# bdaiinstitute/vlfm

Hardware: AMD Instinct MI355X
Metric: env-steps/s (VLM+value-map update), 640x480 RGB-D (higher is better)
Workload: dtype f16 ViT-g (f32 accumulate) + f32 Q-Former (split-f16, 22-bit); f32 confidence + f64 value maps; 1 GPU; configs[1] step x resident envs: BLIP-2 ITC + ValueMap+ObstacleMap+sort_waypoints; envs_per_gpu=256, global_envs=256, map=1000x1000 @ 20 px/m, parallelism=env-sharded x1, tuned_gemms=True, vit_gemm=hip:fc1, attention=hip

## Files before the change

### include/vlfm_amd.h

```cpp
#ifndef VLFM_AMD_H
#define VLFM_AMD_H

#include <stddef.h>
#include <stdint.h>

#ifdef __cplusplus
extern "C" {
#endif

typedef enum {
    VLFM_OK = 0,
    VLFM_ERR_INVALID = -1,
    VLFM_ERR_OUTSIDE_MAP = -2,
    VLFM_ERR_INDEX = -3,
    VLFM_ERR_HIP = -4,
    VLFM_ERR_CAPACITY = -5
} vlfm_status;

enum { VLFM_FUSE_DEFAULT = 0, VLFM_FUSE_REPLACE = 1, VLFM_FUSE_EQUAL_WEIGHTING = 2 };

const char* vlfm_last_error(void);
int vlfm_abi_version(void);

int vlfm_profile_enable(int on);
int vlfm_profile_read(const char* kernel_name, double* mean_ms, int* launches);

int vlfm_host_wait_mode(int blocking);

typedef struct {
    double inv_affine[6];
    int32_t row0, col0;
    int32_t env;
    int32_t reserved;
} vlfm_vm_pose;

int vlfm_value_map_pose_params(const double* h_tf, const double* h_yaw, const int32_t* h_env, int n, int map_size,
                               int pixels_per_meter, int template_size, vlfm_vm_pose* h_out, int* bad_index);

int vlfm_cone_template_host(double fov, double max_depth, int pixels_per_meter, double min_confidence,
                            float* h_conf, int conf_capacity, int64_t* h_poly_xy, int poly_capacity,
                            int* n_poly);

int vlfm_tan_table_host(double fov, int width, double* h_out);

int vlfm_cone_template_build(const float* d_conf, const int64_t* d_poly_xy, int n_poly, int template_size,
                             float* d_template, uint32_t* d_template_bits, void* stream);

typedef struct {
    double tf[12];
    float depth_scale;
    float depth_offset;
    float depth_max;
    float reserved0;
    double fx, fy;
    double min_height, max_height;
    int32_t env;
    int32_t scatter;
} vlfm_ingest_params;

typedef struct {
    uint32_t* d_cells;
    int32_t* d_count;
    int32_t capacity;
    int32_t reserved;
} vlfm_scatter_journal;

int vlfm_depth_ingest_batched(const float* d_depth, int n, int height, int width,
                              const vlfm_ingest_params* d_params,
                              uint32_t* d_colmax_keys ,
                              uint32_t* d_obstacle , int map_size, int pixels_per_meter,
                              int32_t* d_status ,
                              uint32_t* d_hole_bits ,
                              const uint32_t* d_filled_bits ,
                              const vlfm_scatter_journal* journal ,
                              void* stream);

int vlfm_selftest_div_exact(const double* d_numerators, int n, double divisor, int32_t* d_mismatches, void* stream);

size_t vlfm_hole_scratch_bytes(int n, int height, int width, int cap_pts, int cap_contours);
int vlfm_fill_small_holes_batched(const uint32_t* d_hole_bits, const int32_t* d_status, int n, int height, int width,
                                  double area_thresh, void* d_scratch, size_t scratch_bytes, int cap_pts,
                                  int cap_contours, uint32_t* d_filled_bits, int32_t* d_counts,
                                  const vlfm_ingest_params* d_params, uint32_t* d_obstacle, int map_size,
                                  const vlfm_scatter_journal* journal, void* stream);
int vlfm_depth_scatter_holes_batched(const vlfm_ingest_params* d_params, int n, int height, int width,
                                     const uint32_t* d_hole_bits, const uint32_t* d_filled_bits,
                                     const int32_t* d_hole_counts ,
                                     uint32_t* d_obstacle, int map_size, int pixels_per_meter, int32_t* d_status,
                                     const float* d_depth ,
                                     void* stream);

int vlfm_fill_small_holes_rig_batched(const uint32_t* d_hole_bits, const int32_t* d_status, int n, int height, int width,
                                      double area_thresh, void* d_scratch, size_t scratch_bytes, int cap_pts,
                                      int cap_contours, uint32_t* d_filled_bits, int32_t* d_counts,
                                      const vlfm_ingest_params* d_params, uint32_t* d_obstacle, int map_size,
                                      const vlfm_scatter_journal* journal, int32_t* d_slot_undone, int n_envs, void* stream);
int vlfm_depth_scatter_holes_rig_batched(const vlfm_ingest_params* d_params, int n, int height, int width,
                                         const uint32_t* d_hole_bits, const uint32_t* d_filled_bits,
                                         const int32_t* d_hole_counts, uint32_t* d_obstacle, int map_size,
                                         int pixels_per_meter, int32_t* d_status, const float* d_depth,
                                         const int32_t* d_slot_undone, void* stream);

int vlfm_value_map_update_fused_batched(uint32_t* d_colmax_keys, int width, const double* d_tan,
                                        const float* d_template, const uint32_t* d_template_bits, int template_size,
                                        const vlfm_vm_pose* d_pose, const double* d_values, int n,
                                        float* d_conf, double* d_value, int map_size, int channels, int pixels_per_meter,
                                        double min_depth, double max_depth, int use_max_confidence, int fusion_type,
                                        const uint32_t* d_explored_bits, uint32_t* d_written_bits, int32_t* d_counters,
                                        const float* d_conf_quadrant, void* stream);

typedef struct {
    const float* d_template;
    const uint32_t* d_template_bits;
    const float* d_conf_quadrant;
    const double* d_tan;
    float depth_scale;
    float depth_offset;
    int32_t template_size;
    int32_t reserved;
} vlfm_vm_optics;

int vlfm_value_map_update_rig_batched(uint32_t* d_colmax_keys, int width, const vlfm_vm_pose* d_pose,
                                      const vlfm_vm_optics* d_optics, const int32_t* d_slots, int n_slots, int n,
                                      int max_template_size, const double* d_values, float* d_conf, double* d_value,
                                      int map_size, int channels, int pixels_per_meter, int use_max_confidence,
                                      int fusion_type, const uint32_t* d_explored_bits, uint32_t* d_written_bits,
                                      int32_t* d_counters, void* stream);

int vlfm_disc_rows_host(int radius, int32_t* h_halfwidth );
int vlfm_value_map_sort_waypoints_batched(const double* d_value, int map_size, int channels,
                                          const int32_t* d_cells, int m, int radius, const int32_t* d_disc,
                                          int value_is_f32, double* d_out, void* stream);



int vlfm_resample_coeffs_host(int in_size, int out_size, int32_t* h_bounds, int32_t* h_kk, int kk_capacity,
                              int* ksize_out);

int vlfm_resample_coeffs_filter_host(int in_size, int out_size, int filter, int32_t* h_bounds, int32_t* h_kk,
                                     int kk_capacity, int* ksize_out);

int vlfm_preprocess_sam_batched(const uint8_t* d_rgb, int n, int height, int width, int out_h, int out_w,
                                const int32_t* d_hbounds, const int32_t* d_hk, int hksize,
                                const int32_t* d_vbounds, const int32_t* d_vk, int vksize,
                                const float* h_mean3, const float* h_std3, int pad_size, uint8_t* d_tmp, float* d_out,
                                void* stream);

int vlfm_preprocess_rgb_batched(const uint8_t* d_rgb, int n, int height, int width, int out_size,
                                const int32_t* d_hbounds, const int32_t* d_hk, int hksize,
                                const int32_t* d_vbounds, const int32_t* d_vk, int vksize,
                                const float* h_mean3, const float* h_std3, uint8_t* d_tmp, void* d_out,
                                int out_dtype, int patch_size, void* stream);

int vlfm_itc_head_batched(const float* d_proj, int batch, int n_query, int proj_dim,
                          const float* d_text, float* d_out, void* stream);

#define VLFM_ITC_MAX_PROMPTS 8
int vlfm_itc_head_multi(const float* d_proj, int batch, int n_query, int proj_dim, const float* d_text_table, int n_text,
                        const int32_t* d_text_index, int n_prompts, float* d_out, void* stream);

int vlfm_layernorm_bias_f16(const void* d_x, const float* d_channel_bias, const void* d_gamma, const void* d_beta,
                            void* d_y, int rows, int dim, float eps, void* stream);

int vlfm_vit_attention_f16(const void* d_qkv, void* d_out, int batch, int tokens, int heads, int head_dim, float scale,
                           void* stream);

int vlfm_gemm_f16_nt(const void* d_x, const void* d_w, const void* d_bias, void* d_c, int m, int n, int k, int epilogue,
                     void* stream);

int vlfm_gemm_f16_pair_f32_nt(const void* d_x, const void* d_w_pair, const void* d_bias_f32, void* d_out, int m, int n_out, int k,
                              void* stream);

int vlfm_qformer_cross_attention_f32(const void* d_q, const void* d_kv_blocks, void* d_out, int batch, int tokens, int queries,
                                     int heads, int k_block0, int v_block0, int m_total, float scale, void* stream);

int vlfm_gemm_f16_tile_order(int m, int n, int group_m, int* out, int capacity_pairs);
int vlfm_gemm_f16_work_items(int m, int n, int grid, int* out, int capacity_pairs);

int vlfm_split_f32_to_f16_pair(const float* d_src, void* d_hi, void* d_lo, long long count, int* d_overflow, void* stream);
int vlfm_gemm_f32_nt(const float* d_x, const float* d_w, const float* d_bias, const float* d_residual, float* d_c, int m, int n,
                     int k, int activation, int precision, const void* d_w_hi, const void* d_w_lo, int* d_overflow, void* stream);


int vlfm_layernorm_rows_f32(const float* d_x, const float* d_gamma, const float* d_beta, float* d_out, int batch, int height,
                            int width, int channels, int window, float eps, void* stream);
int vlfm_window_reverse_add_f32(float* d_x, const float* d_windows, int batch, int height, int width, int channels, int window,
                                void* stream);
int vlfm_dwconv3x3_nhwc_f32(const float* d_x, const float* d_w9c, const float* d_bias, float* d_out, int batch, int height, int width,
                            int channels, void* stream);
int vlfm_window_attention_f32(const float* d_qkv, const float* d_bias_t, float* d_out, long long windows, int tokens, int heads,
                              float scale, void* stream);
int vlfm_layernorm_rows_shifted_f32(const float* d_x, const float* d_gamma, const float* d_beta, float* d_out, int batch, int height,
                                    int width, int channels, int window, float eps, int shift, int pad_zero, void* stream);
int vlfm_window_reverse_add_shifted_f32(float* d_x, const float* d_windows, int batch, int height, int width, int channels, int window,
                                        int shift, void* stream);
int vlfm_window_attention_masked_f32(const float* d_qkv, const float* d_bias_t, const float* d_mask_t, int windows_per_image, float* d_out,
                                     long long windows, int tokens, int heads, float scale, void* stream);

int vlfm_maxpool2x2_nhwc_f16(const void* d_x, void* d_out, int batch, int height, int width, int channels, void* stream);
int vlfm_conv_nhwc_tile(int pixels, int cin, int cout, int ksize, int* tile_pixels, int* tile_channels);
int vlfm_conv_nhwc_f16(const void* d_x, const void* d_w, const void* d_bias, void* d_out, const void* d_zero, int batch,
                       int height, int width, int cin, int cout, int ksize, int stride, int x_pix_stride,
                       int out_pix_stride, int act, void* stream);

int vlfm_resize_area_tab_host(int ssize, int dsize, int32_t* h_first, int32_t* h_count, float* h_w, int ktaps_capacity);

int vlfm_resize_area_batched(const uint8_t* d_rgb, int n, int height, int width, int out_h, int out_w,
                             const int32_t* d_xfirst, const int32_t* d_xcount, const float* d_xw, int xktaps,
                             const int32_t* d_yfirst, const int32_t* d_ycount, const float* d_yw, int yktaps,
                             void* d_out, int out_dtype, void* stream);

int vlfm_to_tensor_normalize_batched(const uint8_t* d_rgb, int n, int height, int width, const float* h_mean3,
                                     const float* h_std3, float* d_out, void* stream);

size_t vlfm_nms_scratch_bytes(int n);
int vlfm_nms(const float* d_boxes_xyxy, const int32_t* d_order, int n, float iou_threshold, void* d_scratch,
             size_t scratch_bytes, int32_t* d_keep, int32_t* d_num_keep, int max_keep, void* stream);

int vlfm_ms_deform_attn(const float* d_value, const int32_t* d_spatial_shapes, const int32_t* d_level_start,
                        const float* d_sampling_loc, const float* d_attn_weight, int batch, int n_query, int n_heads,
                        int head_dim, int n_levels, int n_points, int total_len, float* d_out, void* stream);
int vlfm_ms_deform_attn_fused(const float* d_value, const int32_t* d_spatial_shapes, const int32_t* d_level_start,
                              const float* d_offsets_logits, const float* d_reference, int batch, int n_query, int n_heads,
                              int head_dim, int n_levels, int n_points, int ref_coords, int total_len, float* d_out, void* stream);

int vlfm_dwconv3x3_f32(const float* d_x, const float* d_w, const float* d_bias, float* d_y, int n, int channels, int height,
                       int width, int stride, int gelu, void* stream);

int vlfm_bias_act_nchw(void* d_y, const void* d_bias, int n, int channels, long long hw, int dtype, int act, void* stream);


size_t vlfm_object_cloud_scratch_bytes(int height, int width);
int vlfm_object_cloud_extract(const float* d_depth, const uint8_t* d_mask, int height, int width, int erosion_iterations,
                              double min_depth, double max_depth, double fx, double fy, void* d_scratch, double* d_cloud,
                              int capacity, int32_t* d_count, void* stream);

size_t vlfm_dbscan_scratch_bytes(int n);
int vlfm_dbscan_largest_cluster(const double* d_points, int n, double eps, int min_points, void* d_scratch,
                                size_t scratch_bytes, int32_t* d_labels, int32_t* d_keep, int32_t* d_num_keep, void* stream);

int vlfm_bits_pack(const uint8_t* d_src, uint32_t* d_dst, int planes, int rows, int cols, void* stream);
int vlfm_bits_unpack(const uint32_t* d_src, uint8_t* d_dst, int planes, int rows, int cols, void* stream);

int vlfm_bits_dilate(const uint32_t* d_src, uint32_t* d_dst, int planes, int rows, int cols, int kernel_w,
                     int kernel_h, void* stream);

int vlfm_find_contours_external(const uint32_t* d_img, int planes, int rows, int cols, int method,
                                uint32_t* d_scratch , int32_t* d_pts, int cap_pts,
                                int32_t* d_starts, int32_t* d_lens, int cap_contours, int32_t* d_counts, void* stream);

size_t vlfm_find_contours_wg_scratch_bytes(int planes, int rows, int cols, int cap_pts);
int vlfm_walk_path_counters(long long* h_out4, int reset);
int vlfm_find_contours_external_wg(const uint32_t* d_img, int planes, int rows, int cols, int method, void* d_scratch,
                                   size_t scratch_bytes, int32_t* d_pts, int cap_pts, int32_t* d_starts, int32_t* d_lens,
                                   int cap_contours, int32_t* d_counts, void* stream);

#define VLFM_FOG_MAX_POLY 80
typedef struct {
    int32_t env;
    int32_t ax, ay;
    int32_t radius;
    int32_t n_poly;
    int32_t reserved;
    double rot_c, rot_s;
    double line_len;
    long long poly[2 * VLFM_FOG_MAX_POLY];
} vlfm_fog_params;

int vlfm_fog_params_host(const int32_t* h_agent_px, const double* h_angle_cv2_deg, const double* h_rot_cs,
                         double fov_deg, double max_line_len, const int32_t* h_env, const int32_t* h_explore, int n,
                         vlfm_fog_params* h_out);

size_t vlfm_obstacle_scratch_bytes(int n_envs, int map_size, int cap_pts, int cap_contours);

int vlfm_obstacle_map_update_batched(const vlfm_fog_params* d_prm, int n, const uint32_t* d_obstacle,
                                     uint32_t* d_navigable, uint32_t* d_explored, int32_t* d_bbox, int n_envs,
                                     int map_size, int kernel_size, int fog_radius, double area_thresh_px,
                                     void* d_scratch, size_t scratch_bytes, int cap_pts, int cap_contours,
                                     double* d_frontiers, int cap_frontiers, int32_t* d_counts, int update_obstacles,
                                     int explore, const int32_t* d_windows, int window_blocks_navigable,
                                     int window_blocks_prepare, void* stream);

int vlfm_obstacle_status(const void* d_scratch, int n_envs, int map_size, int cap_pts, int cap_contours,
                         int32_t* h_out);

enum { VLFM_REDUCE_MAX = 0,
       VLFM_REDUCE_EXPLORE = 1,
       VLFM_REDUCE_PLANE = 2 };
enum { VLFM_PRIM_CIRCLE_FILL = 0,
       VLFM_PRIM_CIRCLE = 1,
       VLFM_PRIM_LINE = 2,
       VLFM_PRIM_POLYLINE = 3 };
#define VLFM_RENDER_FLIP_ROWS 1
#define VLFM_RENDER_UNDER_PATH 2
typedef struct {
    int32_t frame;
    int32_t kind;
    int32_t flags;
    int32_t thickness;
    int32_t x0, y0, x1, y1;
    int32_t vtx_off, n_vtx;
    uint8_t bgr[4];
    int32_t reserved;
} vlfm_render_prim;

size_t vlfm_value_render_scratch_bytes(int n, int map_size);

int vlfm_value_map_render(const double* d_value, int n_envs, int map_size, int channels, const int32_t* d_frames, int n,
                          int reduce_mode, double explore_thresh, const double* d_plane, const uint32_t* d_explored,
                          const uint32_t* d_path, const int32_t* d_prim_off, const vlfm_render_prim* d_prims,
                          const int64_t* d_vtx, int rgb, void* d_scratch, size_t scratch_bytes, uint8_t* d_out,
                          void* stream);

int vlfm_obstacle_map_render(const uint32_t* d_obstacle, const uint32_t* d_navigable, const uint32_t* d_explored,
                             int n_envs, int map_size, const int32_t* d_frames, int n, uint32_t pad_bgr,
                             const uint32_t* d_path, const int32_t* d_prim_off, const vlfm_render_prim* d_prims,
                             const int64_t* d_vtx, int rgb, uint8_t* d_out, void* stream);

int vlfm_traj_append(uint32_t* d_path, int n_envs, int map_size, const int32_t* d_segs, int m, int thickness,
                     void* stream);

int vlfm_circle_polygon_host(const int32_t* h_circles, int n, int64_t* h_xy, int32_t* h_off, int capacity);

int vlfm_jpeg_quant_tables_host(int quality, uint16_t* h_tables);
size_t vlfm_jpeg_scratch_bytes(int n, int H, int W);
int vlfm_jpeg_roundtrip_batched(const uint8_t* d_in, uint8_t* d_out, int n, int H, int W, const uint16_t* h_tables,
                                void* d_scratch, size_t scratch_bytes, void* stream);

int vlfm_jpeg_header_host(int quality, int H, int W, uint8_t* h_out, size_t cap, size_t* len);
size_t vlfm_jpeg_encode_bound(int H, int W);
size_t vlfm_jpeg_encode_scratch_bytes(int n, int H, int W);
int vlfm_jpeg_encode_batched(const uint8_t* d_in, int n, int H, int W, int rgb_order, const uint16_t* h_tables,
                             uint8_t* d_out, size_t capacity, uint32_t* d_lengths, void* d_scratch, size_t scratch_bytes,
                             void* stream);
// ... 46 lines not shown
```

### vlfm_amd/_lib.py

```python
from __future__ import annotations

import ctypes
import os
import subprocess
from typing import Optional

_HERE = os.path.dirname(os.path.abspath(__file__))
LIB_PATH = os.path.join(_HERE, "libvlfm_amd.so")
SOURCES = ["value_map.hip", "depth_ingest.hip", "depth_holes.hip", "obstacle_map.hip", "vlm_ops.hip", "vit_attention.hip", "qformer_attention.hip", "detect_ops.hip", "object_cloud.hip", "gemm_f16.hip", "gemm_f32.hip", "conv_nhwc.hip", "sam_ops.hip", "map_render.hip", "jpeg_codec.hip", "jpeg_entropy.hip", "jpeg_decode.hip", "world_render.hip", "host.cpp"]

VLFM_OK = 0
VLFM_ERR_INVALID = -1
VLFM_ERR_OUTSIDE_MAP = -2
VLFM_ERR_INDEX = -3
VLFM_ERR_HIP = -4
VLFM_ERR_CAPACITY = -5

FUSION_TYPES = {"default": 0, "replace": 1, "equal_weighting": 2}


class VmPose(ctypes.Structure):
    _fields_ = [("inv_affine", ctypes.c_double * 6), ("row0", ctypes.c_int32), ("col0", ctypes.c_int32),
                ("env", ctypes.c_int32), ("reserved", ctypes.c_int32)]


class IngestParams(ctypes.Structure):
    _fields_ = [("tf", ctypes.c_double * 12), ("depth_scale", ctypes.c_float), ("depth_offset", ctypes.c_float),
                ("depth_max", ctypes.c_float), ("reserved0", ctypes.c_float), ("fx", ctypes.c_double),
                ("fy", ctypes.c_double), ("min_height", ctypes.c_double), ("max_height", ctypes.c_double),
                ("env", ctypes.c_int32), ("scatter", ctypes.c_int32)]


FOG_MAX_POLY = 80


class FogParams(ctypes.Structure):
    _fields_ = [("env", ctypes.c_int32), ("ax", ctypes.c_int32), ("ay", ctypes.c_int32), ("radius", ctypes.c_int32),
                ("n_poly", ctypes.c_int32), ("reserved", ctypes.c_int32), ("rot_c", ctypes.c_double),
                ("rot_s", ctypes.c_double), ("line_len", ctypes.c_double), ("poly", ctypes.c_longlong * (2 * FOG_MAX_POLY))]


class ScatterJournal(ctypes.Structure):
    _fields_ = [("d_cells", ctypes.c_void_p), ("d_count", ctypes.c_void_p), ("capacity", ctypes.c_int32),
                ("reserved", ctypes.c_int32)]


class VmOptics(ctypes.Structure):
    _fields_ = [("d_template", ctypes.c_void_p), ("d_template_bits", ctypes.c_void_p), ("d_conf_quadrant", ctypes.c_void_p),
                ("d_tan", ctypes.c_void_p), ("depth_scale", ctypes.c_float), ("depth_offset", ctypes.c_float),
                ("template_size", ctypes.c_int32), ("reserved", ctypes.c_int32)]


assert ctypes.sizeof(ScatterJournal) == 24 and ctypes.sizeof(VmOptics) == 48
assert ctypes.sizeof(VmPose) == 64 and ctypes.sizeof(IngestParams) == 152 and ctypes.sizeof(FogParams) == 48 + 16 * FOG_MAX_POLY


def build(verbose: bool = False) -> str:
    from concurrent.futures import ThreadPoolExecutor

    csrc = os.path.join(_HERE, "csrc")
    srcs = [os.path.join(csrc, s) for s in SOURCES if os.path.exists(os.path.join(csrc, s))]
    hdrs = [os.path.join(csrc, h) for h in os.listdir(csrc) if h.endswith(".h")] + [
        os.path.join(_HERE, "..", "include", "vlfm_amd.h")]
    hdr_time = max(os.path.getmtime(h) for h in hdrs)
    objdir = os.path.join(csrc, "build")
    os.makedirs(objdir, exist_ok=True)
    flags = ["--offload-arch=gfx950", "-O3", "-std=c++17", "-fPIC", "-ffp-contract=off"]

    def compile_one(src: str) -> str:
        obj = os.path.join(objdir, os.path.basename(src) + ".o")
        if not os.path.exists(obj) or os.path.getmtime(obj) < max(os.path.getmtime(src), hdr_time):
            cmd = ["hipcc"] + flags + ["-c", src, "-o", obj]
            if verbose:
                print(" ".join(cmd), flush=True)
            subprocess.check_call(cmd)
        return obj

    with ThreadPoolExecutor(max_workers=min(8, len(srcs))) as pool:
        objs = list(pool.map(compile_one, srcs))
    if os.path.exists(LIB_PATH) and all(os.path.getmtime(LIB_PATH) >= os.path.getmtime(o) for o in objs):
        return LIB_PATH
    cmd = ["hipcc", "--offload-arch=gfx950", "-shared", "-fPIC", "-o", LIB_PATH] + objs
    if verbose:
        print(" ".join(cmd), flush=True)
    subprocess.check_call(cmd)
    return LIB_PATH


_lib: Optional[ctypes.CDLL] = None


def lib() -> ctypes.CDLL:
    global _lib
    if _lib is None:
        if not os.path.exists(LIB_PATH):
            raise ImportError(
                f"{LIB_PATH} is missing: build it with `python -c 'import __graft_entry__ as g; g.build()'` "
                "(hipcc --offload-arch=gfx950).  vlfm_amd has no CPU fallback.")
        L = ctypes.CDLL(LIB_PATH)
        vp, ci, cd = ctypes.c_void_p, ctypes.c_int, ctypes.c_double
        L.vlfm_last_error.restype = ctypes.c_char_p
        L.vlfm_abi_version.restype = ci
        L.vlfm_profile_enable.argtypes = [ci]
        L.vlfm_host_wait_mode.argtypes = [ci]
        L.vlfm_profile_read.argtypes = [ctypes.c_char_p, ctypes.POINTER(cd), ctypes.POINTER(ci)]
        L.vlfm_value_map_pose_params.argtypes = [vp, vp, vp, ci, ci, ci, ci, vp, ctypes.POINTER(ci)]
        L.vlfm_cone_template_host.argtypes = [cd, cd, ci, cd, vp, ci, vp, ci, ctypes.POINTER(ci)]
        L.vlfm_tan_table_host.argtypes = [cd, ci, vp]
        L.vlfm_disc_rows_host.argtypes = [ci, vp]
        L.vlfm_cone_template_build.argtypes = [vp, vp, ci, ci, vp, vp, vp]
        L.vlfm_depth_ingest_batched.argtypes = [vp, ci, ci, ci, vp, vp, vp, ci, ci, vp, vp, vp, vp, vp]
        L.vlfm_selftest_div_exact.argtypes = [vp, ci, cd, vp, vp]
        L.vlfm_hole_scratch_bytes.argtypes = [ci, ci, ci, ci, ci]
        L.vlfm_hole_scratch_bytes.restype = ctypes.c_size_t
        L.vlfm_fill_small_holes_batched.argtypes = [vp, vp, ci, ci, ci, cd, vp, ctypes.c_size_t, ci, ci, vp, vp, vp, vp,
                                                    ci, vp, vp]
        L.vlfm_depth_scatter_holes_batched.argtypes = [vp, ci, ci, ci, vp, vp, vp, vp, ci, ci, vp, vp, vp]
        L.vlfm_fill_small_holes_rig_batched.argtypes = [vp, vp, ci, ci, ci, cd, vp, ctypes.c_size_t, ci, ci, vp, vp, vp, vp,
                                                        ci, vp, vp, ci, vp]
        L.vlfm_depth_scatter_holes_rig_batched.argtypes = [vp, ci, ci, ci, vp, vp, vp, vp, ci, ci, vp, vp, vp, vp]
        L.vlfm_layernorm_bias_f16.argtypes = [vp, vp, vp, vp, vp, ci, ci, ctypes.c_float, vp]
        L.vlfm_vit_attention_f16.argtypes = [vp, vp, ci, ci, ci, ci, ctypes.c_float, vp]
        L.vlfm_gemm_f16_nt.argtypes = [vp, vp, vp, vp, ci, ci, ci, ci, vp]
        L.vlfm_gemm_f16_pair_f32_nt.argtypes = [vp, vp, vp, vp, ci, ci, ci, vp]
        L.vlfm_qformer_cross_attention_f32.argtypes = [vp, vp, vp, ci, ci, ci, ci, ci, ci, ci, ctypes.c_float, vp]
        L.vlfm_gemm_f32_nt.argtypes = [vp, vp, vp, vp, vp, ci, ci, ci, ci, ci, vp, vp, vp, vp]
        L.vlfm_split_f32_to_f16_pair.argtypes = [vp, vp, vp, ctypes.c_longlong, vp, vp]
        L.vlfm_layernorm_rows_f32.argtypes = [vp, vp, vp, vp, ci, ci, ci, ci, ci, ctypes.c_float, vp]
        L.vlfm_window_reverse_add_f32.argtypes = [vp, vp, ci, ci, ci, ci, ci, vp]
        L.vlfm_dwconv3x3_nhwc_f32.argtypes = [vp, vp, vp, vp, ci, ci, ci, ci, vp]
        L.vlfm_window_attention_f32.argtypes = [vp, vp, vp, ctypes.c_longlong, ci, ci, ctypes.c_float, vp]
        L.vlfm_layernorm_rows_shifted_f32.argtypes = [vp, vp, vp, vp, ci, ci, ci, ci, ci, ctypes.c_float, ci, ci, vp]
        L.vlfm_window_reverse_add_shifted_f32.argtypes = [vp, vp, ci, ci, ci, ci, ci, ci, vp]
        L.vlfm_window_attention_masked_f32.argtypes = [vp, vp, vp, ci, vp, ctypes.c_longlong, ci, ci, ctypes.c_float, vp]
        L.vlfm_maxpool2x2_nhwc_f16.argtypes = [vp, vp, ci, ci, ci, ci, vp]
        L.vlfm_conv_nhwc_tile.argtypes = [ci, ci, ci, ci, ctypes.POINTER(ci), ctypes.POINTER(ci)]
        L.vlfm_conv_nhwc_f16.argtypes = [vp, vp, vp, vp, vp, ci, ci, ci, ci, ci, ci, ci, ci, ci, ci, vp]
        L.vlfm_value_map_update_fused_batched.argtypes = [vp, ci, vp, vp, vp, ci, vp, vp, ci, vp, vp, ci, ci, ci, cd, cd,
                                                          ci, ci, vp, vp, vp, vp, vp]
        L.vlfm_value_map_update_rig_batched.argtypes = [vp, ci, vp, vp, vp, ci, ci, ci, vp, vp, vp, ci, ci, ci, ci, ci, vp, vp,
                                                        vp, vp]
        L.vlfm_value_map_sort_waypoints_batched.argtypes = [vp, ci, ci, vp, ci, ci, vp, ci, vp, vp]
        L.vlfm_resample_coeffs_host.argtypes = [ci, ci, vp, vp, ci, ctypes.POINTER(ci)]
        L.vlfm_resample_coeffs_filter_host.argtypes = [ci, ci, ci, vp, vp, ci, ctypes.POINTER(ci)]
        L.vlfm_preprocess_sam_batched.argtypes = [vp, ci, ci, ci, ci, ci, vp, vp, ci, vp, vp, ci, vp, vp, ci, vp, vp, vp]
        L.vlfm_preprocess_rgb_batched.argtypes = [vp, ci, ci, ci, ci, vp, vp, ci, vp, vp, ci, vp, vp, vp, vp, ci, ci, vp]
        L.vlfm_itc_head_batched.argtypes = [vp, ci, ci, ci, vp, vp, vp]
        L.vlfm_itc_head_multi.argtypes = [vp, ci, ci, ci, vp, ci, vp, ci, vp, vp]
        cf = ctypes.c_float
        L.vlfm_resize_area_tab_host.argtypes = [ci, ci, vp, vp, vp, ci]
        L.vlfm_resize_area_batched.argtypes = [vp, ci, ci, ci, ci, ci, vp, vp, vp, ci, vp, vp, vp, ci, vp, ci, vp]
        L.vlfm_to_tensor_normalize_batched.argtypes = [vp, ci, ci, ci, vp, vp, vp, vp]
        L.vlfm_nms_scratch_bytes.argtypes = [ci]
        L.vlfm_nms_scratch_bytes.restype = ctypes.c_size_t
        L.vlfm_nms.argtypes = [vp, vp, ci, cf, vp, ctypes.c_size_t, vp, vp, ci, vp]
        L.vlfm_ms_deform_attn.argtypes = [vp, vp, vp, vp, vp, ci, ci, ci, ci, ci, ci, ci, vp, vp]
        L.vlfm_ms_deform_attn_fused.argtypes = [vp, vp, vp, vp, vp, ci, ci, ci, ci, ci, ci, ci, ci, vp, vp]
        L.vlfm_object_cloud_scratch_bytes.argtypes = [ci, ci]
        L.vlfm_object_cloud_scratch_bytes.restype = ctypes.c_size_t
        L.vlfm_object_cloud_extract.argtypes = [vp, vp, ci, ci, ci, cd, cd, cd, cd, vp, vp, ci, vp, vp]
        L.vlfm_dbscan_scratch_bytes.argtypes = [ci]
        L.vlfm_dbscan_scratch_bytes.restype = ctypes.c_size_t
        L.vlfm_dbscan_largest_cluster.argtypes = [vp, ci, cd, ci, vp, ctypes.c_size_t, vp, vp, vp, vp]
        L.vlfm_bits_pack.argtypes = [vp, vp, ci, ci, ci, vp]
        L.vlfm_bits_unpack.argtypes = [vp, vp, ci, ci, ci, vp]
        L.vlfm_bits_dilate.argtypes = [vp, vp, ci, ci, ci, ci, ci, vp]
        L.vlfm_find_contours_external.argtypes = [vp, ci, ci, ci, ci, vp, vp, ci, vp, vp, ci, vp, vp]
        L.vlfm_dwconv3x3_f32.argtypes = [vp, vp, vp, vp, ci, ci, ci, ci, ci, ci, vp]
        L.vlfm_bias_act_nchw.argtypes = [vp, vp, ci, ci, ctypes.c_longlong, ci, ci, vp]
        L.vlfm_find_contours_wg_scratch_bytes.argtypes = [ci, ci, ci, ci]
        L.vlfm_find_contours_wg_scratch_bytes.restype = ctypes.c_size_t
        L.vlfm_find_contours_external_wg.argtypes = [vp, ci, ci, ci, ci, vp, ctypes.c_size_t, vp, ci, vp, vp, ci, vp, vp]
        L.vlfm_walk_path_counters.argtypes = [vp, ci]
        L.vlfm_fog_params_host.argtypes = [vp, vp, vp, cd, cd, vp, vp, ci, vp]
        L.vlfm_obstacle_scratch_bytes.argtypes = [ci, ci, ci, ci]
        L.vlfm_obstacle_scratch_bytes.restype = ctypes.c_size_t
        L.vlfm_obstacle_map_update_batched.argtypes = [vp, ci, vp, vp, vp, vp, ci, ci, ci, ci, cd, vp, ctypes.c_size_t,
                                                       ci, ci, vp, ci, vp, ci, ci, vp, ci, ci, vp]
        L.vlfm_obstacle_status.argtypes = [vp, ci, ci, ci, ci, vp]
        L.vlfm_value_render_scratch_bytes.argtypes = [ci, ci]
        L.vlfm_value_render_scratch_bytes.restype = ctypes.c_size_t
        L.vlfm_value_map_render.argtypes = [vp, ci, ci, ci, vp, ci, ci, cd, vp, vp, vp, vp, vp, vp, ci, vp,
                                            ctypes.c_size_t, vp, vp]
        L.vlfm_obstacle_map_render.argtypes = [vp, vp, vp, ci, ci, vp, ci, ctypes.c_uint32, vp, vp, vp, vp, ci, vp, vp]
        L.vlfm_traj_append.argtypes = [vp, ci, ci, vp, ci, ci, vp]
        L.vlfm_circle_polygon_host.argtypes = [vp, ci, vp, vp, ci]
        L.vlfm_jpeg_quant_tables_host.argtypes = [ci, vp]
        L.vlfm_jpeg_scratch_bytes.argtypes = [ci, ci, ci]
        L.vlfm_jpeg_scratch_bytes.restype = ctypes.c_size_t
        L.vlfm_jpeg_roundtrip_batched.argtypes = [vp, vp, ci, ci, ci, vp, vp, ctypes.c_size_t, vp]
        L.vlfm_jpeg_header_host.argtypes = [ci, ci, ci, vp, ctypes.c_size_t, ctypes.POINTER(ctypes.c_size_t)]
        L.vlfm_jpeg_encode_bound.argtypes = [ci, ci]
        L.vlfm_jpeg_encode_bound.restype = ctypes.c_size_t
        L.vlfm_jpeg_encode_scratch_bytes.argtypes = [ci, ci, ci]
        L.vlfm_jpeg_encode_scratch_bytes.restype = ctypes.c_size_t
        L.vlfm_jpeg_encode_batched.argtypes = [vp, ci, ci, ci, ci, vp, vp, ctypes.c_size_t, vp, vp, ctypes.c_size_t, vp]
        L.vlfm_jpeg_parse_host.argtypes = [vp, ctypes.c_size_t, vp, vp]
        L.vlfm_jpeg_parse_reason.argtypes = [ci]
        L.vlfm_jpeg_parse_reason.restype = ctypes.c_char_p
        L.vlfm_jpeg_decode_chunk_bytes.restype = ctypes.c_size_t
        L.vlfm_jpeg_decode_scratch_bytes.argtypes = [ci, ci, ci, ctypes.c_size_t]
        L.vlfm_jpeg_decode_scratch_bytes.restype = ctypes.c_size_t
        L.vlfm_jpeg_decode_batched.argtypes = [vp, ctypes.c_size_t, vp, ctypes.c_size_t, vp, ci, ci, ci, vp, vp, ci, vp, ci, ci,
                                               ctypes.c_size_t, ci, vp, vp, vp, ctypes.c_size_t, vp]
        L.vlfm_rooms_raycast.argtypes = [vp, ci, vp, ci, ci, ci, vp, vp]
        L.vlfm_rooms_raycast_objects.argtypes = [vp, ci, vp, ci, vp, vp, ci, ci, ci, vp, vp, vp, vp]
        _lib = L
    return _lib


def profile_read(kernel: str):
    ms, n = ctypes.c_double(0.0), ctypes.c_int(0)
    lib().vlfm_profile_read(kernel.encode(), ctypes.byref(ms), ctypes.byref(n))
    return ms.value, n.value


def last_error() -> str:
    return lib().vlfm_last_error().decode()


def host_wait_blocking(device=None, blocking: bool = True) -> None:
    import torch

    with torch.cuda.device(device if device is not None else torch.cuda.current_device()):
        check(lib().vlfm_host_wait_mode(int(bool(blocking))), "host_wait_mode")


def try_host_wait_blocking(device=None) -> bool:
    import os
    import warnings

    if os.environ.get("VLFM_HOST_WAIT", "blocking") == "spin":
        return False
    try:
        host_wait_blocking(device)
        return True
    except Exception as exc:
        warnings.warn(f"blocking host waits not enabled on {device}: {exc} (call vlfm_amd._lib.host_wait_blocking before the "
                      f"device's first allocation; waits will spin on a host core)")
        return False


def check(rc: int, what: str = "") -> int:
    if rc >= 0:
        return rc
    msg = last_error()
    if rc == VLFM_ERR_OUTSIDE_MAP:
        raise AssertionError(msg or "Pixel location is outside the image.")
    if rc == VLFM_ERR_INDEX:
        raise IndexError(msg or "index out of bounds for obstacle map")
    raise RuntimeError(f"libvlfm_amd {what} failed ({rc}): {msg}")
```

### vlfm_amd/csrc/gemm_f32.hip

```cpp
#include <hip/hip_runtime.h>
#include <stdint.h>
#include <stdlib.h>

#include "../../include/vlfm_amd.h"
#include "profile.h"
#include "status.h"

namespace vlfm {
namespace g32 {

typedef float floatx4 __attribute__((ext_vector_type(4)));
typedef float floatx16 __attribute__((ext_vector_type(16)));
typedef _Float16 half8 __attribute__((ext_vector_type(8)));
typedef _Float16 half4 __attribute__((ext_vector_type(4)));

constexpr int TB = 128;
constexpr int TK = 32;
constexpr int ROWB = TK * 4;
constexpr int OPER = TB * ROWB;
constexpr int BUF = 2 * OPER;
constexpr int EPI_ROW = 272;
constexpr int EPI_WAVE = 64 * EPI_ROW;
constexpr int LDS_EXACT = 4 * EPI_WAVE > 2 * BUF ? 4 * EPI_WAVE : 2 * BUF;

enum { ACT_NONE = 0, ACT_RELU = 1, ACT_GELU = 2 };

struct Args {
    const float* x;
    const float* w;
    const float* bias;
    const float* residual;
    float* c;
    int M, N, K;
    int tiles_m, tiles_n;
    int* overflow;
    const _Float16* w_hi;
    const _Float16* w_lo;
};

__device__ inline float gelu_erf(float v) {
    const float u = fabsf(v);
    float q = 2.834908400e-06f;
    q = fmaf(q, u, -3.937762449e-05f);
    q = fmaf(q, u, 1.861798810e-04f);
    q = fmaf(q, u, 1.369373058e-04f);
    q = fmaf(q, u, -7.063421421e-03f);
    q = fmaf(q, u, 5.249617994e-02f);
    q = fmaf(q, u, 4.592081904e-01f);
    q = fmaf(q, u, 1.151105165e+00f);
    const float e = __builtin_amdgcn_exp2f(-(q * u));
    return fmaf(-0.5f * u, e, fmaxf(v, 0.0f));
}

using lds_ptr = __attribute__((address_space(3))) unsigned char*;
using gbl_ptr = const __attribute__((address_space(1))) unsigned char*;

__device__ inline void tile_of_block(const Args& a, int& tm, int& tn) {
    const int nwg = a.tiles_m * a.tiles_n;
    int bid = blockIdx.x;
    const int q = nwg >> 3, r = nwg & 7, xcd = bid & 7, idx = bid >> 3;
    bid = (xcd < r ? xcd * (q + 1) : r * (q + 1) + (xcd - r) * q) + idx;
    tm = bid / a.tiles_n;
    tn = bid - tm * a.tiles_n;
}

__device__ inline void stage_tile(const Args& a, lds_ptr lds, int buf, int n0, int m0, int k0, int wave, int lane) {
    const int sub = lane >> 3, p = lane & 7;
#pragma unroll
    for (int j = 0; j < 4; j++) {
        const int chunk = wave * 4 + j;
        const int r = chunk * 8 + sub;
        const int s = p ^ ((r >> 1) & 7);
        const int rn = min(n0 + r, a.N - 1), rm = min(m0 + r, a.M - 1);
        const float* gw = a.w + (size_t)rn * a.K + k0 + s * 4;
        const float* gx = a.x + (size_t)rm * a.K + k0 + s * 4;
        const int dst = __builtin_amdgcn_readfirstlane(buf + chunk * 1024);
        __builtin_amdgcn_global_load_lds((gbl_ptr)gw, lds + dst, 16, 0, 0);
        __builtin_amdgcn_global_load_lds((gbl_ptr)gx, lds + dst + OPER, 16, 0, 0);
    }
}

template <bool SPLIT>
__device__ inline void store_tile(const Args& a, unsigned char* smem, const floatx16 (&acc)[2][2], const floatx16 (&cross)[2][2],
                                  int act, int wave, int wn, int wm, int lane, int m0, int n0) {
    unsigned char* stg = smem + wave * EPI_WAVE;
    const int c32 = lane & 31, h4 = (lane >> 5) * 4;
    floatx4 bias4[2][4];
#pragma unroll
    for (int i = 0; i < 2; i++)
#pragma unroll
        for (int g = 0; g < 4; g++) {
            floatx4 b = {0.f, 0.f, 0.f, 0.f};
            if (a.bias) {
                const int n = n0 + wn * 64 + i * 32 + g * 8 + h4;
                if (n + 4 <= a.N && ((uintptr_t)a.bias & 15) == 0) b = *reinterpret_cast<const floatx4*>(a.bias + n);
                else
                    for (int e = 0; e < 4; e++) b[e] = n + e < a.N ? a.bias[n + e] : 0.f;
            }
            bias4[i][g] = b;
        }
#pragma unroll
    for (int i = 0; i < 2; i++)
#pragma unroll
        for (int g = 0; g < 4; g++) {
            const int nl = i * 32 + g * 8 + h4;
            const floatx4 b = bias4[i][g];
#pragma unroll
            for (int j = 0; j < 2; j++) {
                floatx4 v;
#pragma unroll
                for (int e = 0; e < 4; e++) {
                    float t = acc[i][j][g * 4 + e];
                    if (SPLIT) t = fmaf(cross[i][j][g * 4 + e], 0x1p-11f, t);
                    t += b[e];
                    if (act == ACT_RELU) t = fmaxf(t, 0.f);
                    else if (act == ACT_GELU) t = gelu_erf(t);
                    v[e] = t;
                }
                *reinterpret_cast<floatx4*>(stg + (j * 32 + c32) * EPI_ROW + nl * 4) = v;
            }
        }
    __builtin_amdgcn_s_waitcnt(0xC07F);
    const int rsub = lane >> 4, chunk = lane & 15;
    const bool vec = (a.N & 3) == 0;
    const int n = n0 + wn * 64 + chunk * 4;
    const bool fast = vec && n + 4 <= a.N;
    floatx4 r[16], v[16];
#pragma unroll
    for (int it = 0; it < 16; it++) {
        const int m = m0 + wm * 64 + it * 4 + rsub;
        r[it] = floatx4{0.f, 0.f, 0.f, 0.f};
        if (a.residual && fast && m < a.M) r[it] = *reinterpret_cast<const floatx4*>(a.residual + (size_t)m * a.N + n);
    }
#pragma unroll
    for (int it = 0; it < 16; it++) v[it] = *reinterpret_cast<const floatx4*>(stg + (it * 4 + rsub) * EPI_ROW + chunk * 16);
#pragma unroll
    for (int it = 0; it < 16; it++) {
        const int m = m0 + wm * 64 + it * 4 + rsub;
        if (m >= a.M || n >= a.N) continue;
        const size_t at = (size_t)m * a.N + n;
        if (fast) {
            *reinterpret_cast<floatx4*>(a.c + at) = v[it] + r[it];
        } else {
            for (int e = 0; e < 4 && n + e < a.N; e++) a.c[at + e] = v[it][e] + (a.residual ? a.residual[at + e] : 0.f);
        }
    }
}

__global__ __launch_bounds__(256, 2) void gemm_f32_exact_kernel(Args a, int act) {
    extern __shared__ __attribute__((aligned(16))) unsigned char smem[];
    lds_ptr lds = (lds_ptr)smem;
    const int tid = threadIdx.x, lane = tid & 63;
    const int wave = __builtin_amdgcn_readfirstlane(tid >> 6);
    const int wn = wave >> 1, wm = wave & 1;
    int tm, tn;
    tile_of_block(a, tm, tn);
    const int m0 = tm * TB, n0 = tn * TB;
    const int NT = a.K / TK;

    floatx16 acc[2][2];
#pragma unroll
    for (int i = 0; i < 2; i++)
#pragma unroll
        for (int j = 0; j < 2; j++)
#pragma unroll
            for (int e = 0; e < 16; e++) acc[i][j][e] = 0.f;

    stage_tile(a, lds, 0, n0, m0, 0, wave, lane);
    __builtin_amdgcn_s_waitcnt(0x0F70);
    __builtin_amdgcn_s_barrier();
    asm volatile("" ::: "memory");

    const int r32 = lane & 31, h = lane >> 5;
    for (int t = 0; t < NT; t++) {
        const int cur = (t & 1) * BUF;
        if (t + 1 < NT) stage_tile(a, lds, cur ^ BUF, n0, m0, (t + 1) * TK, wave, lane);
#pragma unroll
        for (int kk = 0; kk < 4; kk++) {
            const int s = kk * 2 + h;
            floatx4 fa[2], fb[2];
#pragma unroll
            for (int i = 0; i < 2; i++) {
                const int R = wn * 64 + i * 32 + r32;
                fa[i] = *reinterpret_cast<const floatx4*>(smem + cur + R * ROWB + ((s ^ ((R >> 1) & 7)) << 4));
            }
#pragma unroll
            for (int j = 0; j < 2; j++) {
                const int R = wm * 64 + j * 32 + r32;
                fb[j] = *reinterpret_cast<const floatx4*>(smem + cur + OPER + R * ROWB + ((s ^ ((R >> 1) & 7)) << 4));
            }
#pragma unroll
            for (int q = 0; q < 4; q++)
#pragma unroll
                for (int i = 0; i < 2; i++)
#pragma unroll
                    for (int j = 0; j < 2; j++)
                        acc[i][j] = __builtin_amdgcn_mfma_f32_32x32x2f32(fa[i][q], fb[j][q], acc[i][j], 0, 0, 0);
        }
        __builtin_amdgcn_s_waitcnt(0x0F70);
        __builtin_amdgcn_s_barrier();
        asm volatile("" ::: "memory");
    }
    store_tile<false>(a, smem, acc, acc, act, wave, wn, wm, lane, m0, n0);
}

constexpr int SROWB = TK * 2;
constexpr int SOPER = TB * SROWB;
constexpr int SBUF = 4 * SOPER;

__device__ inline int sslot(int row, int slot) { return (slot ^ ((row >> 2) & 3)) << 4; }

__device__ inline void split4(const floatx4 v, half4& hi, half4& lo, bool& over) {
#pragma unroll
    for (int e = 0; e < 4; e++) {
        const float a = v[e];
        over |= !(fabsf(a) < 65504.0f);
        const _Float16 hh = (_Float16)a;
        hi[e] = hh;
        lo[e] = (_Float16)((a - (float)hh) * 2048.0f);
    }
}

template <int NI>
struct SplitGeom {
    static constexpr int TN = 64 * NI;
    static constexpr int WOPER = TN * SROWB;
    static constexpr int XO = 0, WO = 2 * SOPER;
    static constexpr int BUF = 2 * SOPER + 2 * WOPER;
    static constexpr int LDS = 4 * EPI_WAVE > 2 * BUF ? 4 * EPI_WAVE : 2 * BUF;
};

template <int NI>
__device__ __forceinline__ void gemm_f32_split_body(const Args& a, int act) {
    using G = SplitGeom<NI>;
    extern __shared__ __attribute__((aligned(16))) unsigned char smem[];
    lds_ptr lds = (lds_ptr)smem;
    const int tid = threadIdx.x, lane = tid & 63;
    const int wave = __builtin_amdgcn_readfirstlane(tid >> 6);
    const int wn = wave >> 1, wm = wave & 1;
    int tm, tn;
    tile_of_block(a, tm, tn);
    const int m0 = tm * TB, n0 = tn * G::TN;
    const int NT = a.K / TK;

    floatx16 acc[NI][2], crs[NI][2];
#pragma unroll
    for (int i = 0; i < NI; i++)
#pragma unroll
        for (int j = 0; j < 2; j++)
#pragma unroll
            for (int e = 0; e < 16; e++) { acc[i][j][e] = 0.f; crs[i][j][e] = 0.f; }

    floatx4 xr[4];
    bool over = false;
    auto load_x = [&](int k0) {
#pragma unroll
        for (int u = 0; u < 4; u++) {
            const int idx = tid + 256 * u, r = idx >> 3, pc = idx & 7;
            const int rm = min(m0 + r, a.M - 1);
            xr[u] = *reinterpret_cast<const floatx4*>(a.x + (size_t)rm * a.K + k0 + pc * 4);
        }
    };
    auto put_x = [&](int buf) {
#pragma unroll
        for (int u = 0; u < 4; u++) {
            const int idx = tid + 256 * u, r = idx >> 3, pc = idx & 7;
            half4 hi, lo;
            split4(xr[u], hi, lo, over);
            const int off = r * SROWB + sslot(r, pc >> 1) + (pc & 1) * 8;
            *reinterpret_cast<half4*>(smem + buf + G::XO + off) = hi;
            *reinterpret_cast<half4*>(smem + buf + G::XO + SOPER + off) = lo;
        }
    };
    auto stage_w = [&](int buf, int k0) {
        const int sub = lane >> 2, p = lane & 3;
#pragma unroll
        for (int j = 0; j < NI; j++) {
            const int chunk = wave * NI + j;
            const int r = chunk * 16 + sub;
            const int s = p ^ ((r >> 2) & 3);
            const int rn = min(n0 + r, a.N - 1);
            const size_t g = (size_t)rn * a.K + k0 + s * 8;
            const int dst = __builtin_amdgcn_readfirstlane(buf + G::WO + chunk * 1024);
            __builtin_amdgcn_global_load_lds((gbl_ptr)(a.w_hi + g), lds + dst, 16, 0, 0);
            __builtin_amdgcn_global_load_lds((gbl_ptr)(a.w_lo + g), lds + dst + G::WOPER, 16, 0, 0);
        }
    };

    load_x(0);
    stage_w(0, 0);
    put_x(0);
    __builtin_amdgcn_s_waitcnt(0x0F70);
    __builtin_amdgcn_s_waitcnt(0xC07F);
    __builtin_amdgcn_s_barrier();
    asm volatile("" ::: "memory");

    const int r32 = lane & 31, h = lane >> 5;
    for (int t = 0; t < NT; t++) {
        const int cur = (t & 1) * G::BUF;
        if (t + 1 < NT) {
            load_x((t + 1) * TK);
            stage_w(cur ^ G::BUF, (t + 1) * TK);
        }
#pragma unroll
        for (int kk = 0; kk < 2; kk++) {
            const int s = kk * 2 + h;
            half8 whi[NI], wlo[NI], xhi[2], xlo[2];
#pragma unroll
            for (int i = 0; i < NI; i++) {
                const int R = wn * 32 * NI + i * 32 + r32, o = cur + G::WO + R * SROWB + sslot(R, s);
                whi[i] = *reinterpret_cast<const half8*>(smem + o);
                wlo[i] = *reinterpret_cast<const half8*>(smem + o + G::WOPER);
            }
#pragma unroll
            for (int j = 0; j < 2; j++) {
                const int R = wm * 64 + j * 32 + r32, o = cur + G::XO + R * SROWB + sslot(R, s);
                xhi[j] = *reinterpret_cast<const half8*>(smem + o);
                xlo[j] = *reinterpret_cast<const half8*>(smem + o + SOPER);
            }
#pragma unroll
            for (int i = 0; i < NI; i++)
#pragma unroll
                for (int j = 0; j < 2; j++) {
                    acc[i][j] = __builtin_amdgcn_mfma_f32_32x32x16_f16(whi[i], xhi[j], acc[i][j], 0, 0, 0);
                    crs[i][j] = __builtin_amdgcn_mfma_f32_32x32x16_f16(whi[i], xlo[j], crs[i][j], 0, 0, 0);
                    crs[i][j] = __builtin_amdgcn_mfma_f32_32x32x16_f16(wlo[i], xhi[j], crs[i][j], 0, 0, 0);
                }
        }
        if (t + 1 < NT) put_x(cur ^ G::BUF);
        __builtin_amdgcn_s_waitcnt(0x0F70);
        __builtin_amdgcn_s_waitcnt(0xC07F);
        __builtin_amdgcn_s_barrier();
        asm volatile("" ::: "memory");
    }
    if (over && a.overflow) atomicOr(a.overflow, 1);
#pragma unroll
    for (int half = 0; half < NI / 2; half++)
        store_tile<true>(a, smem, reinterpret_cast<const floatx16(&)[2][2]>(acc[2 * half]),
                         reinterpret_cast<const floatx16(&)[2][2]>(crs[2 * half]), act, wave, 0, wm, lane, m0,
                         n0 + wn * 32 * NI + half * 64);
}

__global__ __launch_bounds__(256, 2) void gemm_f32_split_kernel(Args a, int act) { gemm_f32_split_body<2>(a, act); }

__global__ void split_f32_kernel(const float* __restrict__ src, _Float16* __restrict__ hi, _Float16* __restrict__ lo, long long n,
                                 int* overflow) {
    const long long i = (long long)blockIdx.x * blockDim.x + threadIdx.x;
    if (i >= n) return;
    const float a = src[i];
    if (!(fabsf(a) < 65504.0f) && overflow) atomicOr(overflow, 1);
    const _Float16 hh = (_Float16)a;
    hi[i] = hh;
    lo[i] = (_Float16)((a - (float)hh) * 2048.0f);
}

}
}

using namespace vlfm;
using namespace vlfm::g32;

extern "C" int vlfm_split_f32_to_f16_pair(const float* d_src, void* d_hi, void* d_lo, long long count, int* d_overflow, void* stream) {
    if (count == 0) return VLFM_OK;
    if (!d_src || !d_hi || !d_lo || count < 0) return fail(VLFM_ERR_INVALID, "split_f32_to_f16_pair: bad argument");
    const long long blocks = (count + 255) / 256;
    VLFM_KLAUNCH(split_f32_kernel, dim3((unsigned)blocks), dim3(256), 0, (hipStream_t)stream, d_src, (_Float16*)d_hi, (_Float16*)d_lo,
                 count, d_overflow);
    return check_launch("split_f32_kernel");
}

extern "C" int vlfm_gemm_f32_nt(const float* d_x, const float* d_w, const float* d_bias, const float* d_residual, float* d_c, int m,
                                int n, int k, int activation, int precision, const void* d_w_hi, const void* d_w_lo,
                                int* d_overflow, void* stream) {
    if (m == 0 || n == 0) return VLFM_OK;
    if (!d_x || !d_w || !d_c || m < 0 || n < 0 || k <= 0 || (k % TK) != 0 || activation < 0 || activation > 2 || precision < 0 ||
        precision > 1)
        return fail(VLFM_ERR_INVALID, "gemm_f32_nt: K must be a multiple of 32, activation 0..2, precision 0..1");
    if (((uintptr_t)d_x | (uintptr_t)d_w | (uintptr_t)d_c | (uintptr_t)d_residual | (uintptr_t)d_w_hi | (uintptr_t)d_w_lo) & 15)
        return fail(VLFM_ERR_INVALID, "gemm_f32_nt: X, W, C, residual and the split weights must be 16-byte aligned");
    if (precision == 1 && (!d_w_hi || !d_w_lo || !d_overflow))
        return fail(VLFM_ERR_INVALID, "gemm_f32_nt: the split form needs the pre-split weights and the overflow flag");
    Args a;
    a.x = d_x; a.w = d_w; a.bias = d_bias; a.residual = d_residual; a.c = d_c;
    a.M = m; a.N = n; a.K = k;
    a.tiles_m = (m + TB - 1) / TB; a.tiles_n = (n + TB - 1) / TB;
    a.overflow = d_overflow; a.w_hi = (const _Float16*)d_w_hi; a.w_lo = (const _Float16*)d_w_lo;
    if ((long long)a.tiles_m * a.tiles_n > 0x7fffffffLL) return fail(VLFM_ERR_CAPACITY, "gemm_f32_nt: too many tiles");
    const dim3 grid(a.tiles_m * a.tiles_n), block(256);
    static LdsOptIn opt_exact, opt_split;
    if (precision == 0) {
        if (LDS_EXACT > 64 * 1024 && !opt_exact.ensure(reinterpret_cast<const void*>(gemm_f32_exact_kernel), LDS_EXACT))
            return fail(VLFM_ERR_HIP, "gemm_f32_nt: cannot opt in to the LDS size");
        VLFM_TIMED("gemm_f32_exact_kernel", stream);
        VLFM_KLAUNCH(gemm_f32_exact_kernel, grid, block, LDS_EXACT, (hipStream_t)stream, a, activation);
        return check_launch("gemm_f32_exact_kernel");
    }
    if (SplitGeom<2>::LDS > 64 * 1024 && !opt_split.ensure(reinterpret_cast<const void*>(gemm_f32_split_kernel), SplitGeom<2>::LDS))
        return fail(VLFM_ERR_HIP, "gemm_f32_nt: cannot opt in to the LDS size");
    VLFM_TIMED("gemm_f32_split_kernel", stream);
    VLFM_KLAUNCH(gemm_f32_split_kernel, grid, block, SplitGeom<2>::LDS, (hipStream_t)stream, a, activation);
    return check_launch("gemm_f32_split_kernel");
}
```

### vlfm_amd/csrc/host.cpp

```cpp
#include <cmath>
#include <cstdint>
#include <cstring>
#include <mutex>
#include <string>

#include "../../include/vlfm_amd.h"
#include "status.h"

namespace vlfm {
static thread_local std::string g_last_error;
void set_last_error(const char* msg) { g_last_error = msg ? msg : ""; }
}

extern "C" const char* vlfm_last_error(void) { return vlfm::g_last_error.c_str(); }
extern "C" int vlfm_abi_version(void) { return 16; }

namespace {

const double kPi = 3.141592653589793238462643383279502884;

inline long round_half_even(double v) { return std::lrint(v); }

float sin_deg_table(int deg) {
    static float tab[451];
    static std::once_flag once;
    std::call_once(once, [] {
        for (int i = 0; i <= 450; i++) tab[i] = (float)(std::round(std::sin(i * kPi / 180.0) * 1e7) / 1e7);
    });
    return tab[deg];
}

}

extern "C" int vlfm_value_map_pose_params(const double* h_tf, const double* h_yaw, const int32_t* h_env, int n,
                                          int map_size, int pixels_per_meter, int template_size,
                                          vlfm_vm_pose* h_out, int* bad_index) {
    if (!h_tf || !h_out || n < 0 || map_size <= 0 || template_size <= 0)
        return vlfm::fail(VLFM_ERR_INVALID, "value_map_pose_params: bad argument");
    const double ppm = (double)pixels_per_meter;
    const int half = template_size / 2;
    for (int k = 0; k < n; k++) {
        const double* tf = h_tf + 16 * k;
        const double yaw = h_yaw ? h_yaw[k] : std::atan2(tf[4], tf[0]);
        const double degrees = (-yaw) * (180.0 / kPi);
        const double ang = degrees * (kPi / 180);
        const double alpha = std::cos(ang), beta = std::sin(ang);
        const double cx = (double)(float)half, cy = (double)(float)half;
        double M[6] = {alpha, beta, (1 - alpha) * cx - beta * cy, -beta, alpha, beta * cx + (1 - alpha) * cy};
        double D = M[0] * M[4] - M[1] * M[3];
        D = D != 0 ? 1. / D : 0;
        const double A11 = M[4] * D, A22 = M[0] * D;
        M[0] = A11; M[1] *= -D;
        M[3] *= -D; M[4] = A22;
        const double b1 = -M[0] * M[2] - M[1] * M[5];
        const double b2 = -M[3] * M[2] - M[4] * M[5];
        M[2] = b1; M[5] = b2;
        vlfm_vm_pose& p = h_out[k];
        std::memcpy(p.inv_affine, M, sizeof(M));
        const double cam_x = tf[3] / tf[15], cam_y = tf[7] / tf[15];
        const long px = (long)(cam_x * ppm) + map_size / 2;
        const long py = (long)(-cam_y * ppm) + map_size / 2;
        if (px < 0 || px >= map_size || py < 0 || py >= map_size) {
            if (bad_index) *bad_index = k;
            return vlfm::fail(VLFM_ERR_OUTSIDE_MAP, "Pixel location is outside the image.");
        }
        p.row0 = (int32_t)(px - half);
        p.col0 = (int32_t)(py - half);
        p.env = h_env ? h_env[k] : k;
        p.reserved = 0;
    }
    return VLFM_OK;
}

static int ellipse_sector_polygon(int cx, int cy, int radius, double start_angle, double end_angle, int64_t* out_xy,
                                  int capacity) {
    int a0 = (int)round_half_even(start_angle), a1 = (int)round_half_even(end_angle);
    const bool full = (a1 - a0) >= 360;
    if (a0 > a1) { int t = a0; a0 = a1; a1 = t; }
    while (a0 < 0) { a0 += 360; a1 += 360; }
    while (a1 > 360) { a1 -= 360; a0 -= 360; }
    if (a1 - a0 > 360) { a0 = 0; a1 = 360; }
    const int step = radius < 3 ? 90 : radius < 10 ? 30 : radius < 15 ? 18 : 5;
    const double ccx = (double)((int64_t)cx << 16), ccy = (double)((int64_t)cy << 16);
    const double axis = (double)((int64_t)radius << 16);
    int m = 0;
    int64_t last_x = -1, last_y = -1;
    for (int a = a0; a < a1 + step; a += step) {
        int t = a > a1 ? a1 : a;
        if (t < 0) t += 360;
        const double ex = axis * sin_deg_table(450 - t), ey = axis * sin_deg_table(t);
        const double vx = ccx + ex * sin_deg_table(90) - ey * sin_deg_table(0);
        const double vy = ccy + ex * sin_deg_table(0) + ey * sin_deg_table(90);
        int64_t qx = (int64_t)round_half_even(vx / 65536.0) << 16, qy = (int64_t)round_half_even(vy / 65536.0) << 16;
        qx += round_half_even(vx - (double)qx);
        qy += round_half_even(vy - (double)qy);
        if (qx == last_x && qy == last_y) continue;
        if (m >= capacity) return VLFM_ERR_CAPACITY;
        out_xy[2 * m] = qx; out_xy[2 * m + 1] = qy; m++;
        last_x = qx; last_y = qy;
    }
    if (!full) {
        if (m >= capacity) return VLFM_ERR_CAPACITY;
        out_xy[2 * m] = (int64_t)cx << 16; out_xy[2 * m + 1] = (int64_t)cy << 16; m++;
    }
    return m;
}

extern "C" int vlfm_fog_params_host(const int32_t* h_agent_px, const double* h_angle_cv2_deg, const double* h_rot_cs,
                                    double fov_deg, double max_line_len, const int32_t* h_env,
                                    const int32_t* h_explore, int n, vlfm_fog_params* h_out) {
    if (!h_agent_px || !h_angle_cv2_deg || !h_rot_cs || !h_out || n < 0)
        return vlfm::fail(VLFM_ERR_INVALID, "fog_params_host: bad argument");
    for (int k = 0; k < n; k++) {
        vlfm_fog_params& p = h_out[k];
        std::memset(&p, 0, sizeof(p));
        p.env = h_env ? h_env[k] : k;
        p.ax = h_agent_px[2 * k]; p.ay = h_agent_px[2 * k + 1];
        p.radius = (int)max_line_len;
        p.rot_c = h_rot_cs[2 * k]; p.rot_s = h_rot_cs[2 * k + 1];
        p.line_len = max_line_len * 1.05;
        if (h_explore && !h_explore[k]) { p.n_poly = 0; continue; }
        const int m = ellipse_sector_polygon(p.ax, p.ay, p.radius, h_angle_cv2_deg[k] - fov_deg / 2,
                                             h_angle_cv2_deg[k] + fov_deg / 2, (int64_t*)p.poly, VLFM_FOG_MAX_POLY);
        if (m < 0) return vlfm::fail(m, "fog_params_host: sector polygon does not fit VLFM_FOG_MAX_POLY");
        p.n_poly = m;
    }
    return VLFM_OK;
}

extern "C" int vlfm_circle_polygon_host(const int32_t* h_circles, int n, int64_t* h_xy, int32_t* h_off, int capacity) {
    if (!h_circles || !h_xy || !h_off || n < 0 || capacity < 0)
        return vlfm::fail(VLFM_ERR_INVALID, "circle_polygon_host: bad argument");
    int total = 0;
    h_off[0] = 0;
    for (int k = 0; k < n; k++) {
        const int cx = h_circles[3 * k], cy = h_circles[3 * k + 1], r = h_circles[3 * k + 2];
        if (r < 0) return vlfm::fail(VLFM_ERR_INVALID, "circle_polygon_host: negative radius");
        const int m = ellipse_sector_polygon(cx, cy, r, 0.0, 360.0, h_xy + 2 * (size_t)total, capacity - total);
        if (m < 0) return vlfm::fail(m, "circle_polygon_host: vertex capacity");
        if (m == 1) {
            if (total + 2 > capacity) return vlfm::fail(VLFM_ERR_CAPACITY, "circle_polygon_host: vertex capacity");
            for (int i = 0; i < 2; i++) {
                h_xy[2 * (size_t)(total + i)] = (int64_t)cx << 16;
                h_xy[2 * (size_t)(total + i) + 1] = (int64_t)cy << 16;
            }
            total += 2;
        } else {
            total += m;
        }
        h_off[k + 1] = total;
    }
    return total;
}

extern "C" int vlfm_cone_template_host(double fov, double max_depth, int pixels_per_meter, double min_confidence,
                                       float* h_conf, int conf_capacity, int64_t* h_poly_xy, int poly_capacity,
                                       int* n_poly) {
    if (!h_conf || !h_poly_xy || !n_poly || pixels_per_meter <= 0)
        return vlfm::fail(VLFM_ERR_INVALID, "cone_template_host: bad argument");
    const int size = (int)(max_depth * pixels_per_meter);
    const int T = 2 * size + 1;
    if (size <= 0) return vlfm::fail(VLFM_ERR_INVALID, "cone_template_host: empty template");
    if ((long)T * T > conf_capacity) return vlfm::fail(VLFM_ERR_CAPACITY, "cone_template_host: conf capacity");
    const int mid = T / 2;
    for (int r = 0; r < T; r++) {
        const double fwd = std::abs(r - mid);
        for (int c = 0; c < T; c++) {
            const double lat = std::abs(c - mid);
// ... 125 lines not shown
```

### vlfm_amd/csrc/qformer_attention.hip

```cpp
#include <hip/hip_runtime.h>
#include <stdint.h>

#include "../../include/vlfm_amd.h"
#include "profile.h"
#include "status.h"

namespace vlfm {

typedef float qa_f32x16 __attribute__((ext_vector_type(16)));
typedef float qa_f32x4 __attribute__((ext_vector_type(4)));
using qa_lds_ptr = __attribute__((address_space(3))) unsigned char*;
using qa_gbl_ptr = const __attribute__((address_space(1))) unsigned char*;

constexpr int QA_ROWB = 256;
constexpr int QA_MERGE_REGS = 34;
constexpr int QA_MERGE = 3 * QA_MERGE_REGS * 64 * 4;
constexpr int QA_MAX_T = 257, QA_MAX_Q = 32;

struct QaArgs {
    const float* q;
    const float* kv;
    float* out;
    int B, T, Q, heads, k_block0, v_block0, M_total;
    int rows_pad;
    float scale_log2e;
};

struct QaKernel {
    const QaArgs& a;
    unsigned char* smem;
    qa_lds_ptr lds;
    int lane, wave, col, g, voff;

    __device__ QaKernel(const QaArgs& a_, unsigned char* smem_) : a(a_), smem(smem_), lds((qa_lds_ptr)smem_) {
        lane = threadIdx.x & 63;
        wave = __builtin_amdgcn_readfirstlane(threadIdx.x >> 6);
        col = lane & 31;
        g = lane >> 5;
        voff = a.rows_pad * QA_ROWB;
    }
    __device__ inline const unsigned char* block(int block0, int b, int h) const {
        return reinterpret_cast<const unsigned char*>(a.kv + ((size_t)(block0 + h) * (size_t)a.M_total + (size_t)b * (size_t)a.T) * 64);
    }
    __device__ inline void issue_k(const unsigned char* kg, int row0, int n_ins) const {
        const int r4 = lane >> 4, p = lane & 15;
        for (int ins = 0; ins < n_ins; ins++) {
            const int row = row0 + 4 * ins + r4, src_row = min(row, a.T - 1);
            const int dst = __builtin_amdgcn_readfirstlane((row0 + 4 * ins) * QA_ROWB);
            __builtin_amdgcn_global_load_lds((qa_gbl_ptr)(kg + (size_t)src_row * QA_ROWB + ((p ^ (row & 15)) << 4)), lds + dst, 16, 0, 0);
        }
    }
    __device__ inline void issue_v(const unsigned char* vg, int row0, int n_ins) const {
        const int r4 = lane >> 4, p = lane & 15;
        for (int ins = 0; ins < n_ins; ins++) {
            const int row = row0 + 4 * ins + r4, src_row = min(row, a.T - 1);
            const int dst = __builtin_amdgcn_readfirstlane(voff + (row0 + 4 * ins) * QA_ROWB);
            __builtin_amdgcn_global_load_lds((qa_gbl_ptr)(vg + (size_t)src_row * QA_ROWB + ((p ^ (((row >> 2) & 1) << 3)) << 4)),
                                             lds + dst, 16, 0, 0);
        }
    }
    __device__ inline void issue_rows(const unsigned char* kg, const unsigned char* vg, int row0, int n_ins) const {
        issue_k(kg, row0, n_ins);
        issue_v(vg, row0, n_ins);
    }
    __device__ inline void load_q(int b, int h, float (&qn)[32]) const {
        const float* src = a.q + ((size_t)b * a.Q + min(col, a.Q - 1)) * ((size_t)a.heads * 64) + (size_t)h * 64 + 32 * g;
#pragma unroll
        for (int c = 0; c < 8; c++) {
            const qa_f32x4 v = *reinterpret_cast<const qa_f32x4*>(src + 4 * c);
            qn[4 * c] = v[0]; qn[4 * c + 1] = v[1]; qn[4 * c + 2] = v[2]; qn[4 * c + 3] = v[3];
        }
    }
};

__device__ __forceinline__ void qa_item(int w, int heads, int& b, int& h) {
    const int xcd = w & 7, idx = w >> 3;
    b = (idx / heads) * 8 + xcd;
    h = idx % heads;
}

__global__ __launch_bounds__(256) void qformer_cross_attention_kernel(QaArgs a) {
    extern __shared__ __attribute__((aligned(16))) unsigned char smem[];
    QaKernel k(a, smem);
    const int lane = k.lane, wave = k.wave, col = k.col, g = k.g;
    const int n_full = a.T >> 5, n_left = a.T & 31, left_wave = n_full & 3, left_ins = (n_left + 3) >> 2;
    const int stride = gridDim.x;
    const int moff = 2 * k.voff;
    int w = blockIdx.x, b, h;
    qa_item(w, a.heads, b, h);
    if (b >= a.B) return;

    float qn[32];
    k.load_q(b, h, qn);
    {
        const unsigned char* kg = k.block(a.k_block0, b, h);
        const unsigned char* vg = k.block(a.v_block0, b, h);
        for (int t = wave; t < n_full; t += 4) k.issue_rows(kg, vg, 32 * t, 8);
        if (n_left != 0 && wave == left_wave) k.issue_rows(kg, vg, 32 * n_full, left_ins);
    }
    for (;;) {
        __builtin_amdgcn_s_waitcnt(0x0F70);
        asm volatile("" ::: "memory");
        float qf[32];
#pragma unroll
        for (int s = 0; s < 32; s++) qf[s] = qn[s];
        const int nw = w + stride;
        int nb, nh;
        qa_item(nw, a.heads, nb, nh);
        const bool more = nb < a.B;
        const unsigned char* kg = k.block(a.k_block0, more ? nb : b, more ? nh : h);
        const unsigned char* vg = k.block(a.v_block0, more ? nb : b, more ? nh : h);
        if (more) k.load_q(nb, nh, qn);

        float m = -INFINITY, l = 0.f;
        qa_f32x16 o0, o1;
#pragma unroll
        for (int r = 0; r < 16; r++) { o0[r] = 0.f; o1[r] = 0.f; }
        for (int t = wave; t < n_full; t += 4) {
            const unsigned char* kb = smem + (32 * t + col) * QA_ROWB;
            float kf[32];
#pragma unroll
            for (int c = 0; c < 8; c++) {
                const qa_f32x4 v = *reinterpret_cast<const qa_f32x4*>(kb + (((8 * g + c) ^ (col & 15)) << 4));
                kf[4 * c] = v[0]; kf[4 * c + 1] = v[1]; kf[4 * c + 2] = v[2]; kf[4 * c + 3] = v[3];
            }
            __builtin_amdgcn_s_waitcnt(0xC07F);
            __builtin_amdgcn_sched_barrier(0);
            asm volatile("" ::: "memory");
            if (more) k.issue_k(kg, 32 * t, 8);
            qa_f32x16 acc;
#pragma unroll
            for (int r = 0; r < 16; r++) acc[r] = 0.f;
#pragma unroll
            for (int s = 0; s < 32; s++) acc = __builtin_amdgcn_mfma_f32_32x32x2f32(kf[s], qf[s], acc, 0, 0, 0);
#pragma unroll
            for (int r = 0; r < 16; r++) acc[r] *= a.scale_log2e;
            float tm = acc[0];
#pragma unroll
            for (int r = 1; r < 16; r++) tm = fmaxf(tm, acc[r]);
            tm = fmaxf(tm, __shfl_xor(tm, 32, 64));
            const float mn = fmaxf(m, tm);
            const float alpha = __builtin_amdgcn_exp2f(m - mn);
            m = mn;
            l *= alpha;
#pragma unroll
            for (int r = 0; r < 16; r++) { o0[r] *= alpha; o1[r] *= alpha; }
#pragma unroll
            for (int r = 0; r < 16; r++) { const float pj = __builtin_amdgcn_exp2f(acc[r] - mn); l += pj; acc[r] = pj; }
            const float* vb = reinterpret_cast<const float*>(smem + k.voff + (32 * t + 4 * g) * QA_ROWB);
            const int c0 = (((col >> 2) ^ (8 * g)) << 2) + (col & 3), c1 = (((8 + (col >> 2)) ^ (8 * g)) << 2) + (col & 3);
#pragma unroll
            for (int r = 0; r < 16; r++) {
                const int ro = ((r & 3) + 8 * (r >> 2)) * 64;
                o0 = __builtin_amdgcn_mfma_f32_32x32x2f32(vb[ro + c0], acc[r], o0, 0, 0, 0);
                o1 = __builtin_amdgcn_mfma_f32_32x32x2f32(vb[ro + c1], acc[r], o1, 0, 0, 0);
            }
            __builtin_amdgcn_s_waitcnt(0xC07F);
            __builtin_amdgcn_sched_barrier(0);
            asm volatile("" ::: "memory");
            if (more) k.issue_v(vg, 32 * t, 8);
        }
        if (n_left != 0 && wave == left_wave) {
            for (int j = 32 * n_full; j < a.T; j++) {
                const unsigned char* kr = smem + j * QA_ROWB;
                float part = 0.f;
#pragma unroll
                for (int c = 0; c < 8; c++) {
                    const qa_f32x4 v = *reinterpret_cast<const qa_f32x4*>(kr + (((8 * g + c) ^ (j & 15)) << 4));
#pragma unroll
                    for (int e = 0; e < 4; e++) part = fmaf(v[e], qf[4 * c + e], part);
                }
                const float s = (part + __shfl_xor(part, 32, 64)) * a.scale_log2e;
                const float mn = fmaxf(m, s);
                const float alpha = __builtin_amdgcn_exp2f(m - mn), pj = __builtin_amdgcn_exp2f(s - mn);
                m = mn;
                l = l * alpha + (g == 0 ? pj : 0.f);
                const unsigned char* vr = smem + k.voff + j * QA_ROWB;
                const int sw = ((j >> 2) & 1) << 3;
#pragma unroll
                for (int q4 = 0; q4 < 4; q4++) {
                    const qa_f32x4 v0 = *reinterpret_cast<const qa_f32x4*>(vr + (((2 * q4 + g) ^ sw) << 4));
                    const qa_f32x4 v1 = *reinterpret_cast<const qa_f32x4*>(vr + (((8 + 2 * q4 + g) ^ sw) << 4));
#pragma unroll
                    for (int e = 0; e < 4; e++) {
                        o0[4 * q4 + e] = fmaf(pj, v0[e], o0[4 * q4 + e] * alpha);
                        o1[4 * q4 + e] = fmaf(pj, v1[e], o1[4 * q4 + e] * alpha);
                    }
                }
            }
            __builtin_amdgcn_s_waitcnt(0xC07F);
            __builtin_amdgcn_sched_barrier(0);
            asm volatile("" ::: "memory");
            if (more) k.issue_rows(kg, vg, 32 * n_full, left_ins);
        }
        l += __shfl_xor(l, 32, 64);

        float* sc = reinterpret_cast<float*>(smem + moff);
        if (wave != 0) {
            float* mine = sc + (wave - 1) * QA_MERGE_REGS * 64 + lane;
#pragma unroll
            for (int r = 0; r < 16; r++) { mine[r * 64] = o0[r]; mine[(16 + r) * 64] = o1[r]; }
            mine[32 * 64] = m;
            mine[33 * 64] = l;
            __builtin_amdgcn_s_waitcnt(0xC07F);
        }
        asm volatile("" ::: "memory");
        __builtin_amdgcn_s_barrier();
        asm volatile("" ::: "memory");
        if (wave == 0) {
#pragma unroll
            for (int v = 0; v < 3; v++) {
                const float* src = sc + v * QA_MERGE_REGS * 64 + lane;
                const float m2 = src[32 * 64], l2 = src[33 * 64];
                const float mn = fmaxf(m, m2);
                const float a1 = __builtin_amdgcn_exp2f(m - mn), a2 = __builtin_amdgcn_exp2f(m2 - mn);
                m = mn;
                l = l * a1 + l2 * a2;
#pragma unroll
                for (int r = 0; r < 16; r++) {
                    o0[r] = o0[r] * a1 + src[r * 64] * a2;
                    o1[r] = o1[r] * a1 + src[(16 + r) * 64] * a2;
                }
            }
            if (col < a.Q) {
                const float inv = 1.0f / l;
                float* orow = a.out + ((size_t)b * a.Q + col) * ((size_t)a.heads * 64) + (size_t)h * 64 + 4 * g;
#pragma unroll
                for (int q4 = 0; q4 < 4; q4++) {
                    const qa_f32x4 s0 = {o0[4 * q4] * inv, o0[4 * q4 + 1] * inv, o0[4 * q4 + 2] * inv, o0[4 * q4 + 3] * inv};
                    const qa_f32x4 s1 = {o1[4 * q4] * inv, o1[4 * q4 + 1] * inv, o1[4 * q4 + 2] * inv, o1[4 * q4 + 3] * inv};
                    *reinterpret_cast<qa_f32x4*>(orow + 8 * q4) = s0;
                    *reinterpret_cast<qa_f32x4*>(orow + 32 + 8 * q4) = s1;
                }
            }
            __builtin_amdgcn_s_waitcnt(0xC07F);
        }
        asm volatile("" ::: "memory");
        __builtin_amdgcn_s_barrier();
        asm volatile("" ::: "memory");
        if (!more) break;
        w = nw; b = nb; h = nh;
    }
}

}

using namespace vlfm;

extern "C" int vlfm_qformer_cross_attention_f32(const void* d_q, const void* d_kv_blocks, void* d_out, int batch, int tokens,
                                                int queries, int heads, int k_block0, int v_block0, int m_total, float scale,
                                                void* stream) {
    if (batch == 0) return VLFM_OK;
    if (!d_q || !d_kv_blocks || !d_out || batch < 0 || tokens < 1 || tokens > QA_MAX_T || queries < 1 || queries > QA_MAX_Q || heads < 1 ||
        k_block0 < 0 || v_block0 < 0 || (long long)batch * tokens > (long long)m_total)
        return fail(VLFM_ERR_INVALID, "qformer_cross_attention_f32: head width 64, 1-32 queries, 1-257 tokens, batch * tokens <= m_total");
    if ((((uintptr_t)d_q | (uintptr_t)d_kv_blocks | (uintptr_t)d_out) & 15) != 0)
        return fail(VLFM_ERR_INVALID, "qformer_cross_attention_f32: pointers must be 16-byte aligned");
    QaArgs a;
    a.q = (const float*)d_q; a.kv = (const float*)d_kv_blocks; a.out = (float*)d_out;
    a.B = batch; a.T = tokens; a.Q = queries; a.heads = heads; a.k_block0 = k_block0; a.v_block0 = v_block0; a.M_total = m_total;
    a.rows_pad = (tokens + 3) & ~3;
    a.scale_log2e = scale * 1.4426950408889634f;
    const size_t lds = 2 * (size_t)a.rows_pad * QA_ROWB + QA_MERGE;
    const void* fn = reinterpret_cast<const void*>(qformer_cross_attention_kernel);
    static LdsOptIn opt;
    if (!opt.ensure(fn, lds)) return fail(VLFM_ERR_HIP, "qformer_cross_attention_f32: cannot opt in to the LDS size");
    const long long items = (long long)((batch + 7) / 8) * 8 * heads;
    const int n_cu = device_cu_count() & ~7;
    const dim3 grid((unsigned)(items < n_cu ? items : n_cu)), block(256);
    VLFM_TIMED("qformer_cross_attention_kernel", stream);
    VLFM_KLAUNCH(qformer_cross_attention_kernel, grid, block, lds, stream, a);
    return check_launch("qformer_cross_attention_kernel");
}
```

### vlfm_amd/csrc/vlm_ops.hip

```cpp
#include <hip/hip_fp16.h>
#include <hip/hip_bf16.h>
#include <hip/hip_runtime.h>
#include <stdint.h>

#include <cmath>
#include <cstdlib>
#include <vector>

#include "../../include/vlfm_amd.h"
#include "profile.h"
#include "status.h"

namespace vlfm {

constexpr int PRECISION_BITS = 32 - 8 - 2;

__device__ inline unsigned char clip8(int v) {
    v >>= PRECISION_BITS;
    return (unsigned char)(v < 0 ? 0 : v > 255 ? 255 : v);
}

__global__ __launch_bounds__(256) void resample_h_kernel(const unsigned char* __restrict__ src, int H, int W, int O,
                                                         const int* __restrict__ bounds, const int* __restrict__ kk,
                                                         int ksize, unsigned char* __restrict__ dst) {
// ... 137 lines not shown
        const int x = x4 + i;
        coloff[i] = patch ? (x / patch) * cell + (x % patch) : x;
    }
    const int chan_off = c * (patch ? patch * patch : O * O);
    const unsigned* col0 = reinterpret_cast<const unsigned*>(tmp) + (size_t)c * TR * opd + dc;
    const float* lut_c = lut + c * 256;
    for (int yy = yy0 + vg; yy < yy1; yy += PF_THREADS / PF_VGROUP) {
        const int yu = __builtin_amdgcn_readfirstlane(yy);
        const int ymin = vbounds[2 * yu], cnt = vbounds[2 * yu + 1];
        const int* kv = vk + (size_t)yu * vksize;
        size_t row_off;
        if (patch == 0) {
            row_off = ((size_t)n * 3 * O + yu) * O;
        } else {
            const int py = yu / patch;
            row_off = ((size_t)n * gp * gp + (size_t)py * gp) * cell + (size_t)(yu - py * patch) * patch;
        }
        if (!vlive) continue;
        const unsigned* col = col0 + (size_t)(ymin - r0) * opd;
        int s[4];
#pragma unroll
        for (int i = 0; i < 4; i++) s[i] = 1 << (PRECISION_BITS - 1);
        for (int y = 0; y < cnt; y++) {
            const unsigned wv = col[(size_t)y * opd];
            const int kq = kv[y];
            s[0] = __mul24((int)(wv & 0xFFu), kq) + s[0];
            s[1] = __mul24((int)((wv >> 8) & 0xFFu), kq) + s[1];
            s[2] = __mul24((int)((wv >> 16) & 0xFFu), kq) + s[2];
            s[3] = __mul24((int)(wv >> 24), kq) + s[3];
        }
        OutT v[4];
#pragma unroll
        for (int i = 0; i < 4; i++) v[i] = cast_out<OutT>(lut_c[clip8(s[i])]);
        OutT* o = dst + row_off + chan_off;
        if (pair_ok && x4 + 3 < O) {
            *reinterpret_cast<Pair<OutT>*>(o + coloff[0]) = Pair<OutT>{v[0], v[1]};
            *reinterpret_cast<Pair<OutT>*>(o + coloff[2]) = Pair<OutT>{v[2], v[3]};
        } else {
#pragma unroll
            for (int i = 0; i < 4; i++)
                if (x4 + i < O) o[coloff[i]] = v[i];
        }
    }
}

__global__ __launch_bounds__(256) void resample_v_sam_kernel(const unsigned char* __restrict__ src, int H, int OH, int OW,
                                                             int P, const int* __restrict__ bounds,
                                                             const int* __restrict__ kk, int ksize, Norm3 nrm,
                                                             float* __restrict__ dst) {
    const int yy = blockIdx.x, n = blockIdx.y;
    const unsigned char* img = src + (size_t)n * H * OW * 3;
    const bool row_in = yy < OH;
    const int ymin = row_in ? bounds[2 * yy] : 0, cnt = row_in ? bounds[2 * yy + 1] : 0;
    const int* k = kk + (size_t)(row_in ? yy : 0) * ksize;
    for (int o = threadIdx.x; o < 3 * P; o += blockDim.x) {
        const int c = o / P, xx = o - c * P;
        float v = 0.0f;
        if (row_in && xx < OW) {
            int ss = 1 << (PRECISION_BITS - 1);
            for (int y = 0; y < cnt; y++) ss += (int)img[((size_t)(ymin + y) * OW + xx) * 3 + c] * k[y];
            v = __fdiv_rn(__fsub_rn((float)clip8(ss), nrm.mean[c]), nrm.std[c]);
        }
        dst[(((size_t)n * 3 + c) * P + yy) * P + xx] = v;
    }
}

constexpr int LN_MAXV = 4;
constexpr int LN_ROWS = 8;

struct alignas(16) Half8 { __half2 h[4]; };

template <int NV>
__global__ __launch_bounds__(256) void layernorm_bias_f16_kernel(const __half* __restrict__ x, const float* __restrict__ cb,
                                                                 const __half* __restrict__ gamma,
                                                                 const __half* __restrict__ beta, __half* __restrict__ y,
                                                                 int rows, int D, float eps, int rows_per_wave) {
    const int lane = threadIdx.x & 63, wave = (blockIdx.x * blockDim.x + threadIdx.x) >> 6;
    const int nvec = D >> 3;
    const int r0 = wave * rows_per_wave;
    if (r0 >= rows) return;
    Half8 gm[NV], bt[NV];
    float4 c0[NV], c1[NV];
#pragma unroll
    for (int i = 0; i < NV; i++) {
        const int v = lane + 64 * i;
        if (v < nvec) {
            gm[i] = reinterpret_cast<const Half8*>(gamma)[v];
            bt[i] = reinterpret_cast<const Half8*>(beta)[v];
            c0[i] = cb ? reinterpret_cast<const float4*>(cb)[2 * v] : make_float4(0.f, 0.f, 0.f, 0.f);
            c1[i] = cb ? reinterpret_cast<const float4*>(cb)[2 * v + 1] : make_float4(0.f, 0.f, 0.f, 0.f);
        }
    }
    Half8 cur[NV], nxt[NV], nx2[NV];
    auto load_row = [&](int r, Half8* dst) {
#pragma unroll
        for (int i = 0; i < NV; i++) {
            const int v = lane + 64 * i;
            if (v < nvec) dst[i] = reinterpret_cast<const Half8*>(x + (size_t)r * D)[v];
        }
    };
    auto val = [&](const Half8* row, int i, int j) -> float {
        const float2 t = __half22float2(row[i].h[j >> 1]);
        const float cc = j < 4 ? (&c0[i].x)[j] : (&c1[i].x)[j - 4];
        return ((j & 1) ? t.y : t.x) + cc;
    };
    const int r_end = min(rows, r0 + rows_per_wave);
    load_row(r0, cur);
    if (r0 + 1 < r_end) load_row(r0 + 1, nxt);
    const float inv_d = 1.0f / (float)D;
    for (int r = r0; r < r_end; r++) {
        if (r + 2 < r_end) load_row(r + 2, nx2);
        float sum = 0.0f;
#pragma unroll
        for (int i = 0; i < NV; i++) {
            if (lane + 64 * i < nvec) {
#pragma unroll
                for (int j = 0; j < 8; j++) sum += val(cur, i, j);
            }
        }
#pragma unroll
        for (int off = 32; off > 0; off >>= 1) sum += __shfl_xor(sum, off, 64);
        const float mean = sum * inv_d;
        float sq = 0.0f;
#pragma unroll
        for (int i = 0; i < NV; i++) {
            if (lane + 64 * i < nvec) {
#pragma unroll
                for (int j = 0; j < 8; j++) {
                    const float dlt = val(cur, i, j) - mean;
                    sq = fmaf(dlt, dlt, sq);
                }
            }
        }
#pragma unroll
        for (int off = 32; off > 0; off >>= 1) sq += __shfl_xor(sq, off, 64);
        const float rstd = rsqrtf(sq * inv_d + eps);
#pragma unroll
        for (int i = 0; i < NV; i++) {
            const int v = lane + 64 * i;
            if (v < nvec) {
                Half8 o;
#pragma unroll
                for (int j = 0; j < 4; j++) {
                    const float2 g2 = __half22float2(gm[i].h[j]), b2 = __half22float2(bt[i].h[j]);
                    o.h[j] = __floats2half2_rn((val(cur, i, 2 * j) - mean) * rstd * g2.x + b2.x,
                                               (val(cur, i, 2 * j + 1) - mean) * rstd * g2.y + b2.y);
                }
                reinterpret_cast<Half8*>(y + (size_t)r * D)[v] = o;
            }
        }
#pragma unroll
        for (int i = 0; i < NV; i++) { cur[i] = nxt[i]; nxt[i] = nx2[i]; }
    }
}

__global__ __launch_bounds__(512) void itc_head_kernel(const float* __restrict__ proj, int NQ, int P,
                                                       const float* __restrict__ text, float* __restrict__ out) {
    __shared__ float cos_q[64];
    const int b = blockIdx.x, lane = threadIdx.x & 63, wave = threadIdx.x >> 6, n_waves = blockDim.x >> 6;
    const float* t = text + (size_t)b * P;
    for (int q = wave; q < NQ; q += n_waves) {
        const float* p = proj + ((size_t)b * NQ + q) * P;
        float n2 = 0.0f, dt = 0.0f;
        for (int j = lane; j < P; j += 64) {
            const float v = p[j];
            n2 = fmaf(v, v, n2);
            dt = fmaf(v, t[j], dt);
        }
        for (int off = 32; off > 0; off >>= 1) {
            n2 += __shfl_down(n2, off, 64);
            dt += __shfl_down(dt, off, 64);
        }
        if (lane == 0) cos_q[q] = dt / fmaxf(sqrtf(n2), 1e-12f);
    }
    __syncthreads();
    if (wave == 0) {
        float c = lane < NQ ? cos_q[lane] : -__builtin_huge_valf();
        for (int off = 32; off > 0; off >>= 1) c = fmaxf(c, __shfl_down(c, off, 64));
        if (lane == 0) out[b] = c;
    }
}

template <int T>
__global__ __launch_bounds__(512) void itc_head_multi_kernel(const float* __restrict__ proj, int NQ, int P,
                                                             const float* __restrict__ text, int U,
                                                             const int* __restrict__ idx, float* __restrict__ out) {
    __shared__ float cos_q[T][64];
    const int b = blockIdx.x, lane = threadIdx.x & 63, wave = threadIdx.x >> 6, n_waves = blockDim.x >> 6;
    const float* tp[T];
    unsigned ok = 0;
#pragma unroll
    for (int t = 0; t < T; t++) {
        const int u = idx[(size_t)b * T + t];
        const bool in = u >= 0 && u < U;
        ok |= (unsigned)in << t;
        tp[t] = text + (size_t)(in ? u : 0) * P;
    }
    for (int q = wave; q < NQ; q += n_waves) {
        const float* p = proj + ((size_t)b * NQ + q) * P;
        float n2 = 0.0f, dt[T];
#pragma unroll
        for (int t = 0; t < T; t++) dt[t] = 0.0f;
        for (int j = lane; j < P; j += 64) {
            const float v = p[j];
            n2 = fmaf(v, v, n2);
#pragma unroll
            for (int t = 0; t < T; t++) dt[t] = fmaf(v, tp[t][j], dt[t]);
        }
        for (int off = 32; off > 0; off >>= 1) {
            n2 += __shfl_down(n2, off, 64);
#pragma unroll
            for (int t = 0; t < T; t++) dt[t] += __shfl_down(dt[t], off, 64);
        }
        if (lane == 0) {
            const float nrm = fmaxf(sqrtf(n2), 1e-12f);
#pragma unroll
            for (int t = 0; t < T; t++) cos_q[t][q] = dt[t] / nrm;
        }
    }
    __syncthreads();
    if (wave < T) {
        float c = lane < NQ ? cos_q[wave][lane] : -__builtin_huge_valf();
        for (int off = 32; off > 0; off >>= 1) c = fmaxf(c, __shfl_down(c, off, 64));
        if (lane == 0) out[(size_t)b * T + wave] = (ok >> wave) & 1u ? c : __builtin_nanf("");
    }
}

}

using namespace vlfm;

extern "C" int vlfm_resample_coeffs_filter_host(int in_size, int out_size, int filter, int32_t* h_bounds, int32_t* h_kk,
                                                int kk_capacity, int* ksize_out) {
    if (in_size <= 0 || out_size <= 0 || !h_bounds || !h_kk || !ksize_out || (filter != 0 && filter != 1))
        return fail(VLFM_ERR_INVALID, "resample_coeffs_host: bad argument (filter 0 = bicubic, 1 = bilinear)");
    auto bicubic = [filter](double x) {
        if (x < 0.0) x = -x;
        if (filter == 1) return x < 1.0 ? 1.0 - x : 0.0;
        const double a = -0.5;
        if (x < 1.0) return ((a + 2.0) * x - (a + 3.0)) * x * x + 1;
        if (x < 2.0) return (((x - 5) * x + 8) * x - 4) * a;
        return 0.0;
    };
    const float in0 = 0.0f, in1 = (float)in_size;
    double scale = (double)(in1 - in0) / out_size, filterscale = scale;
    if (filterscale < 1.0) filterscale = 1.0;
    const double support = (filter == 1 ? 1.0 : 2.0) * filterscale;
    const int ksize = (int)std::ceil(support) * 2 + 1;
    *ksize_out = ksize;
    if ((long)out_size * ksize > kk_capacity) return fail(VLFM_ERR_CAPACITY, "resample_coeffs_host: kk capacity");
    std::vector<double> k(ksize);
    for (int xx = 0; xx < out_size; xx++) {
        const double center = in0 + (xx + 0.5) * scale;
        double ww = 0.0;
        const double ss = 1.0 / filterscale;
        int xmin = (int)(center - support + 0.5);
        if (xmin < 0) xmin = 0;
        int xmax = (int)(center + support + 0.5);
        if (xmax > in_size) xmax = in_size;
        xmax -= xmin;
        for (int x = 0; x < xmax; x++) {
            const double w = bicubic((x + xmin - center + 0.5) * ss);
            k[x] = w;
            ww += w;
        }
        for (int x = 0; x < xmax; x++)
            if (ww != 0.0) k[x] /= ww;
        for (int x = xmax; x < ksize; x++) k[x] = 0;
        h_bounds[2 * xx] = xmin;
        h_bounds[2 * xx + 1] = xmax;
        for (int x = 0; x < ksize; x++) {
            const double v = k[x];
            h_kk[(size_t)xx * ksize + x] = v < 0 ? (int)(-0.5 + v * (1 << PRECISION_BITS)) : (int)(0.5 + v * (1 << PRECISION_BITS));
        }
    }
    return VLFM_OK;
}

extern "C" int vlfm_resample_coeffs_host(int in_size, int out_size, int32_t* h_bounds, int32_t* h_kk, int kk_capacity,
                                         int* ksize_out) {
    return vlfm_resample_coeffs_filter_host(in_size, out_size, 0, h_bounds, h_kk, kk_capacity, ksize_out);
}

extern "C" int vlfm_preprocess_sam_batched(const uint8_t* d_rgb, int n, int height, int width, int out_h, int out_w,
                                           const int32_t* d_hbounds, const int32_t* d_hk, int hksize,
                                           const int32_t* d_vbounds, const int32_t* d_vk, int vksize,
                                           const float* h_mean3, const float* h_std3, int pad_size, uint8_t* d_tmp,
                                           float* d_out, void* stream) {
    if (n == 0) return VLFM_OK;
    if (!d_rgb || !d_hbounds || !d_hk || !d_vbounds || !d_vk || !h_mean3 || !h_std3 || !d_tmp || !d_out || n < 0 ||
        height <= 0 || width <= 0 || out_h <= 0 || out_w <= 0 || pad_size < out_h || pad_size < out_w)
        return fail(VLFM_ERR_INVALID, "preprocess_sam_batched: bad argument");
    hipStream_t s = (hipStream_t)stream;
    const size_t lds = ((size_t)width * 3 + 15) / 16 * 16;
    {
        VLFM_TIMED("resample_h_kernel", s);
        VLFM_KLAUNCH(resample_h_kernel, dim3(height, n), dim3(256), lds, s, d_rgb, height, width, out_w, d_hbounds, d_hk,
                     hksize, d_tmp);
    }
    int rc = check_launch("resample_h_kernel");
    if (rc != VLFM_OK) return rc;
    Norm3 nrm;
    for (int c = 0; c < 3; c++) { nrm.mean[c] = h_mean3[c]; nrm.std[c] = h_std3[c]; }
    VLFM_TIMED("resample_v_sam_kernel", s);
    VLFM_KLAUNCH(resample_v_sam_kernel, dim3(pad_size, n), dim3(256), 0, s, d_tmp, height, out_h, out_w, pad_size,
                 d_vbounds, d_vk, vksize, nrm, d_out);
    return check_launch("resample_v_sam_kernel");
}

extern "C" int vlfm_preprocess_rgb_batched(const uint8_t* d_rgb, int n, int height, int width, int out_size,
                                           const int32_t* d_hbounds, const int32_t* d_hk, int hksize,
                                           const int32_t* d_vbounds, const int32_t* d_vk, int vksize,
                                           const float* h_mean3, const float* h_std3, uint8_t* d_tmp, void* d_out,
                                           int out_dtype, int patch_size, void* stream) {
    if (n == 0) return VLFM_OK;
    if (!d_rgb || !d_hbounds || !d_hk || !d_vbounds || !d_vk || !h_mean3 || !h_std3 || !d_tmp || !d_out || n < 0 ||
        height <= 0 || width <= 0 || out_size <= 0 || patch_size < 0 || (patch_size > 0 && out_size % patch_size != 0))
        return fail(VLFM_ERR_INVALID, "preprocess_rgb_batched: bad argument");
    hipStream_t s = (hipStream_t)stream;
    Norm3 nrm;
    for (int c = 0; c < 3; c++) { nrm.mean[c] = h_mean3[c]; nrm.std[c] = h_std3[c]; }
    if (out_dtype < 0 || out_dtype > 2)
        return fail(VLFM_ERR_INVALID, "preprocess_rgb_batched: out_dtype must be 0 (f32), 1 (f16) or 2 (bf16)");
    const int row_bytes = width * 3;
    if (row_bytes % 16 == 0 && row_bytes <= 4096 && ((uintptr_t)d_rgb & 15) == 0 && hksize <= 32 && out_size <= 256 &&
        !getenv("VLFM_PREPROCESS_TWO_PASS")) {
        const int OP = (out_size + 3) & ~3;
        auto span = [&](int R) { return (int)(((long)(R - 1) * height + out_size - 1) / out_size) + vksize + 2; };
        auto lds_of = [&](int R) { return (size_t)3 * 256 * 4 + (size_t)2 * PF_GROUPS * PF_ROW_BYTES + (size_t)3 * span(R) * OP; };
        int R = out_size < 32 ? out_size : 32;
        while (R > 1 && lds_of(R) > 80 * 1024) R--;
        while (R > 8 && (long)((out_size + R - 1) / R) * n < 512) R = (R + 1) / 2;
        const int bands = (out_size + R - 1) / R;
        R = (out_size + bands - 1) / bands;
        const size_t lds = lds_of(R);
        const int TR = span(R);
        const dim3 grid(bands, n), block(PF_THREADS);
        VLFM_TIMED("preprocess_fused_kernel", s);
#define VLFM_PF_LAUNCH(KS, T)                                                                                          \
    do {                                                                                                               \
        static LdsOptIn opt;                                                                                           \
        if (!opt.ensure(reinterpret_cast<const void*>(preprocess_fused_kernel<KS, T>), 80 * 1024))                     \
            return fail(VLFM_ERR_HIP, "preprocess_rgb_batched: cannot opt in to 80 KB of LDS");                        \
        VLFM_KLAUNCH((preprocess_fused_kernel<KS, T>), grid, block, lds, s, d_rgb, height, width, out_size, R, TR,     \
                     d_hbounds, d_hk, hksize, d_vbounds, d_vk, vksize, nrm, (T*)d_out, patch_size);                    \
    } while (0)
#define VLFM_PF_DTYPE(KS)                                                                                              \
    do {                                                                                                               \
        if (out_dtype == 0) VLFM_PF_LAUNCH(KS, float);                                                                 \
        else if (out_dtype == 1) VLFM_PF_LAUNCH(KS, __half);                                                           \
        else VLFM_PF_LAUNCH(KS, __hip_bfloat16);                                                                       \
    } while (0)
        if (hksize <= 8) VLFM_PF_DTYPE(8);
        else if (hksize <= 13) VLFM_PF_DTYPE(13);
        else if (hksize <= 16) VLFM_PF_DTYPE(16);
        else if (hksize <= 25) VLFM_PF_DTYPE(25);
        else VLFM_PF_DTYPE(32);
#undef VLFM_PF_DTYPE
#undef VLFM_PF_LAUNCH
        return check_launch("preprocess_fused_kernel");
    }
    const size_t lds = ((size_t)width * 3 + 15) / 16 * 16;
    {
        VLFM_TIMED("resample_h_kernel", s);
    VLFM_KLAUNCH(resample_h_kernel, dim3(height, n), dim3(256), lds, s, d_rgb, height, width, out_size,
                       d_hbounds, d_hk, hksize, d_tmp);
    }
    int rc = check_launch("resample_h_kernel");
    if (rc != VLFM_OK) return rc;
    VLFM_TIMED("resample_v_norm_kernel", s);
    if (out_dtype == 0)
        VLFM_KLAUNCH(resample_v_norm_kernel<float>, dim3(out_size, n), dim3(256), 0, s, d_tmp, height, out_size,
                           d_vbounds, d_vk, vksize, nrm, (float*)d_out, patch_size);
    else if (out_dtype == 1)
        VLFM_KLAUNCH(resample_v_norm_kernel<__half>, dim3(out_size, n), dim3(256), 0, s, d_tmp, height,
                           out_size, d_vbounds, d_vk, vksize, nrm, (__half*)d_out, patch_size);
    else
        VLFM_KLAUNCH(resample_v_norm_kernel<__hip_bfloat16>, dim3(out_size, n), dim3(256), 0, s, d_tmp, height,
                           out_size, d_vbounds, d_vk, vksize, nrm, (__hip_bfloat16*)d_out, patch_size);
    return check_launch("resample_v_norm_kernel");
}

extern "C" int vlfm_itc_head_batched(const float* d_proj, int batch, int n_query, int proj_dim, const float* d_text,
                                     float* d_out, void* stream) {
    if (batch == 0) return VLFM_OK;
    if (!d_proj || !d_text || !d_out || batch < 0 || n_query <= 0 || n_query > 64 || proj_dim <= 0)
        return fail(VLFM_ERR_INVALID, "itc_head_batched: bad argument (n_query <= 64)");
    VLFM_TIMED("itc_head_kernel", stream);
    VLFM_KLAUNCH(itc_head_kernel, dim3(batch), dim3(512), 0, (hipStream_t)stream, d_proj, n_query, proj_dim,
                       d_text, d_out);
    return check_launch("itc_head_kernel");
}

extern "C" int vlfm_itc_head_multi(const float* d_proj, int batch, int n_query, int proj_dim, const float* d_text_table,
                                   int n_text, const int32_t* d_text_index, int n_prompts, float* d_out, void* stream) {
    if (!d_proj || !d_text_table || !d_text_index || !d_out || batch < 0 || n_query <= 0 || n_query > 64 || proj_dim <= 0 ||
        n_text < 1 || n_prompts < 1 || n_prompts > VLFM_ITC_MAX_PROMPTS)
        return fail(VLFM_ERR_INVALID, "itc_head_multi: bad argument (n_query <= 64, 1 <= n_prompts <= 8, n_text >= 1)");
    if (batch == 0) return VLFM_OK;
    VLFM_TIMED("itc_head_multi_kernel", stream);
#define VLFM_ITC_MULTI(T)                                                                                              \
    case T:                                                                                                            \
        VLFM_KLAUNCH(itc_head_multi_kernel<T>, dim3(batch), dim3(512), 0, (hipStream_t)stream, d_proj, n_query,        \
                     proj_dim, d_text_table, n_text, d_text_index, d_out);                                             \
        break
    switch (n_prompts) {
        VLFM_ITC_MULTI(1); VLFM_ITC_MULTI(2); VLFM_ITC_MULTI(3); VLFM_ITC_MULTI(4);
        VLFM_ITC_MULTI(5); VLFM_ITC_MULTI(6); VLFM_ITC_MULTI(7); VLFM_ITC_MULTI(8);
    }
#undef VLFM_ITC_MULTI
    return check_launch("itc_head_multi_kernel");
}

extern "C" int vlfm_layernorm_bias_f16(const void* d_x, const float* d_channel_bias, const void* d_gamma, const void* d_beta,
                                       void* d_y, int rows, int dim, float eps, void* stream) {
    if (rows == 0) return VLFM_OK;
    if (!d_x || !d_gamma || !d_beta || !d_y || rows < 0 || dim <= 0 || dim % 8 != 0 || dim > 64 * 8 * LN_MAXV)
        return fail(VLFM_ERR_INVALID, "layernorm_bias_f16: dim must be a multiple of 8 and <= 2048");
    const int nvec = dim / 8, nv = (nvec + 63) / 64;
    int rpw = rows / 8192;
    rpw = rpw < 1 ? 1 : rpw > LN_ROWS ? LN_ROWS : rpw;
    const int waves = (rows + rpw - 1) / rpw;
    const dim3 grid((waves + 3) / 4), block(256);
    const __half* x = (const __half*)d_x; const __half* g = (const __half*)d_gamma; const __half* b = (const __half*)d_beta;
    __half* y = (__half*)d_y;
    VLFM_TIMED("layernorm_bias_f16_kernel", stream);
    switch (nv) {
        case 1: VLFM_KLAUNCH(layernorm_bias_f16_kernel<1>, grid, block, 0, (hipStream_t)stream, x, d_channel_bias, g, b, y, rows, dim, eps, rpw); break;
        case 2: VLFM_KLAUNCH(layernorm_bias_f16_kernel<2>, grid, block, 0, (hipStream_t)stream, x, d_channel_bias, g, b, y, rows, dim, eps, rpw); break;
        case 3: VLFM_KLAUNCH(layernorm_bias_f16_kernel<3>, grid, block, 0, (hipStream_t)stream, x, d_channel_bias, g, b, y, rows, dim, eps, rpw); break;
        default: VLFM_KLAUNCH(layernorm_bias_f16_kernel<4>, grid, block, 0, (hipStream_t)stream, x, d_channel_bias, g, b, y, rows, dim, eps, rpw); break;
    }
    return check_launch("layernorm_bias_f16_kernel");
}
```

### vlfm_amd/vlm/blip2itm.py

```python
from __future__ import annotations

import hashlib
import math
import os
import re
from dataclasses import dataclass
from typing import Dict, List, Optional, Sequence, Tuple

import numpy as np
import torch
import torch.nn as nn
import torch.nn.functional as F


@dataclass
class Blip2ITCConfig:
    image_size: int = 224
    patch_size: int = 14
    v_hidden: int = 1408
    v_layers: int = 39
    v_heads: int = 16
    v_mlp: int = 6144
    v_ln_eps: float = 1e-6
    q_hidden: int = 768
# ... 14 lines not shown
                              q_hidden=24, q_layers=4, q_heads=4, q_mlp=48, vocab_size=97,
                              max_position_embeddings=40, num_query_tokens=5, proj_dim=8)


DEFAULT_HIP_GEMMS = ("fc1",)


def x_is_contiguous_f16(t: torch.Tensor) -> bool:
    return t.dtype == torch.float16 and t.is_contiguous()


class _VitBlock(nn.Module):
    def __init__(self, c: Blip2ITCConfig):
        super().__init__()
        self.heads = c.v_heads
        self.layer_norm1 = nn.LayerNorm(c.v_hidden, eps=c.v_ln_eps)
        self.qkv = nn.Linear(c.v_hidden, 3 * c.v_hidden, bias=True)
        self.projection = nn.Linear(c.v_hidden, c.v_hidden)
        self.layer_norm2 = nn.LayerNorm(c.v_hidden, eps=c.v_ln_eps)
        self.fc1 = nn.Linear(c.v_hidden, c.v_mlp)
        self.fc2 = nn.Linear(c.v_mlp, c.v_hidden)

        self._packed = None
        self.hip_attention = True
        self.strict_hip_attention = True
        self.hip_mlp_min_rows = 32 * 257
        self.hip_gemms = frozenset(DEFAULT_HIP_GEMMS)

    def pack_heads(self, multiple: int = 32) -> None:
        h, d = self.heads, self.qkv.in_features
        hd = d // h
        hp = (hd + multiple - 1) // multiple * multiple
        if hp == hd:
            self._packed = None
            return
        w = self.qkv.weight.detach().view(3, h, hd, d)
        bq = self.qkv.bias.detach().view(3, h, hd)
        wq = torch.zeros((3, h, hp, d), dtype=w.dtype, device=w.device)
        bb = torch.zeros((3, h, hp), dtype=w.dtype, device=w.device)
        wq[:, :, :hd] = w
        bb[:, :, :hd] = bq
        pw = self.projection.weight.detach().view(d, h, hd)
        wp = torch.zeros((d, h, hp), dtype=pw.dtype, device=pw.device)
        wp[:, :, :hd] = pw
        self._packed = (wq.view(3 * h * hp, d).contiguous(), bb.view(-1).contiguous(), wp.view(d, h * hp).contiguous(),
                        hp, float(hd) ** -0.5)

    def hip_gemms_at(self, rows: int) -> frozenset:
        from . import ops

        if not (self.hip_mlp_min_rows and rows >= self.hip_mlp_min_rows):
            return frozenset()
        layers = {"qkv": self.qkv, "proj": self.projection, "fc1": self.fc1, "fc2": self.fc2}

        def ok(lin: nn.Linear) -> bool:
            w, b = lin.weight, lin.bias
            return (x_is_contiguous_f16(w) and w.shape[1] % 64 == 0 and w.shape[0] % 8 == 0 and w.numel() * 2 < (1 << 32)
                    and rows * max(w.shape) * 2 < (1 << 32) and (b is None or x_is_contiguous_f16(b)))

        return frozenset(n for n in self.hip_gemms if ok(layers[n]))

    def forward_deferred(self, x: torch.Tensor, c_in: torch.Tensor, c_mid: torch.Tensor) -> torch.Tensor:
        from . import ops

        b, n, d = x.shape
        hd = d // self.heads
        hip = self.hip_gemms_at(b * n)
        h = ops.layernorm_bias(x, c_in, self.layer_norm1.weight, self.layer_norm1.bias, self.layer_norm1.eps)
        x2 = x.view(b * n, d)
        a = None
        if self.hip_attention and n == ops.VIT_ATTENTION_TOKENS and hd in ops.VIT_ATTENTION_HEADS:
            if "qkv" in hip:
                qkv = ops.linear_f16(h.view(b * n, d), self.qkv.weight, self.qkv.bias, "bias")
            else:
                qkv = F.linear(h.view(b * n, d), self.qkv.weight, self.qkv.bias)
            try:
                a = ops.vit_attention(qkv, b, n, self.heads, hd, float(hd) ** -0.5)
            except (RuntimeError, AssertionError, IndexError) as exc:
                if self.strict_hip_attention:
                    raise
                import warnings

                warnings.warn(f"vlfm_vit_attention_f16 unavailable ({exc}); using the library attention kernel instead")
                self.hip_attention = False
        if a is not None:
            if "proj" in hip and x2.is_contiguous():
                ops.linear_f16(a, self.projection.weight, None, "accumulate", out=x2)
            else:
                x2.addmm_(a, self.projection.weight.t())
        elif self._packed is not None:
            wq, bq, wp, hp, scale = self._packed
            q = F.linear(h.view(b * n, d), wq, bq).view(b, n, 3, self.heads, hp).permute(2, 0, 3, 1, 4)
            a = F.scaled_dot_product_attention(q[0], q[1], q[2], scale=scale).transpose(1, 2).reshape(b * n, self.heads * hp)
            x2.addmm_(a, wp.t())
        else:
            q = self.qkv(h).view(b, n, 3, self.heads, hd).permute(2, 0, 3, 1, 4)
            a = F.scaled_dot_product_attention(q[0], q[1], q[2]).transpose(1, 2).reshape(b * n, d)
            x2.addmm_(a, self.projection.weight.t())
        h = ops.layernorm_bias(x, c_mid, self.layer_norm2.weight, self.layer_norm2.bias, self.layer_norm2.eps)
        if "fc1" in hip:
            act = ops.linear_gelu(h.view(b * n, d), self.fc1.weight, self.fc1.bias)
        else:
            act = F.gelu(F.linear(h, self.fc1.weight, self.fc1.bias)).view(b * n, -1)
        if "fc2" in hip and x2.is_contiguous():
            ops.linear_f16(act, self.fc2.weight, None, "accumulate", out=x2)
        else:
            x2.addmm_(act, self.fc2.weight.t())
        return x

    def forward(self, x: torch.Tensor) -> torch.Tensor:
        b, n, d = x.shape
        if self._packed is not None and self._packed[0].dtype == x.dtype:
            wq, bq, wp, hp, scale = self._packed
            qkv = F.linear(self.layer_norm1(x), wq, bq).view(b, n, 3, self.heads, hp).permute(2, 0, 3, 1, 4)
            a = F.scaled_dot_product_attention(qkv[0], qkv[1], qkv[2], scale=scale)
            x = x + F.linear(a.transpose(1, 2).reshape(b, n, self.heads * hp), wp, self.projection.bias)
        else:
            qkv = self.qkv(self.layer_norm1(x)).view(b, n, 3, self.heads, d // self.heads).permute(2, 0, 3, 1, 4)
            a = F.scaled_dot_product_attention(qkv[0], qkv[1], qkv[2])
            x = x + self.projection(a.transpose(1, 2).reshape(b, n, d))
        return x + self.fc2(F.gelu(self.fc1(self.layer_norm2(x))))


def _exact_split3(w: torch.Tensor) -> Tuple[torch.Tensor, torch.Tensor, torch.Tensor]:
    w = w.detach().float()
    w1 = w.half()
    r = (w - w1.float()) * 2048.0
    w2 = r.half()
    return w1, w2, ((r - w2.float()) * 2048.0).half()


KV_SPLIT_PIECES = 2


def _split_gemm(x16: torch.Tensor, pieces, bias: torch.Tensor, n_pieces: Optional[int] = None) -> torch.Tensor:
    w1t, w2t, w3t = pieces
    if (KV_SPLIT_PIECES if n_pieces is None else n_pieces) >= 3:
        o = torch.addmm(bias, x16, w3t, alpha=2.0 ** -22, out_dtype=torch.float32)
        torch.addmm(o, x16, w2t, alpha=2.0 ** -11, out_dtype=torch.float32, out=o)
    else:
        o = torch.addmm(bias, x16, w2t, alpha=2.0 ** -11, out_dtype=torch.float32)
    torch.addmm(o, x16, w1t, out_dtype=torch.float32, out=o)
    return o


QFORMER_SPLIT_MIN_ROWS = 2048


def _qlinear(x: torch.Tensor, lin_w: torch.Tensor, lin_b, act=None, residual=None) -> torch.Tensor:
    from . import ops

    if (x.is_cuda and x.dtype == torch.float32 and lin_w.dtype == torch.float32 and not torch.is_grad_enabled()
            and x.numel() // x.shape[-1] >= QFORMER_SPLIT_MIN_ROWS and ops.linear_f32_supported(x, lin_w)):
        return ops.linear_f32(x, lin_w, lin_b, act=act, residual=residual, precision="split", owner="blip2")
    y = F.linear(x, lin_w, lin_b)
    if act == "gelu":
        y = F.gelu(y)
    return y if residual is None else y + residual


class _BertAttention(nn.Module):
    def __init__(self, hidden: int, kv_hidden: int, heads: int, eps: float):
        super().__init__()
        self.heads = heads
        self.query = nn.Linear(hidden, hidden)
        self.key = nn.Linear(kv_hidden, hidden)
        self.value = nn.Linear(kv_hidden, hidden)
        self.dense = nn.Linear(hidden, hidden)
        self.LayerNorm = nn.LayerNorm(hidden, eps=eps)
        self._kv_split = None
        self._qkv_fused = None

    def _project_kv_f16(self, kv16: torch.Tensor) -> Tuple[torch.Tensor, torch.Tensor]:
        if self._kv_split is None or self._kv_split[0].device != kv16.device:
            w1, w2, w3 = _exact_split3(torch.cat([self.key.weight, self.value.weight]))
            bias = torch.cat([self.key.bias, self.value.bias]).detach().float()
            self._kv_split = (w1.t(), w2.t(), w3.t(), bias)
        o = _split_gemm(kv16.reshape(-1, kv16.shape[-1]), self._kv_split[:3], self._kv_split[3])
        o = o.view(*kv16.shape[:-1], -1)
        hid = self.key.out_features
        return o[..., :hid], o[..., hid:]

    def forward(self, x: torch.Tensor, kv: Optional[torch.Tensor] = None, mask: Optional[torch.Tensor] = None,
                kv_proj: Optional[Tuple[torch.Tensor, torch.Tensor]] = None, kv_blocks=None) -> torch.Tensor:
        b, n, d = x.shape
        h = self.heads
        if kv_blocks is not None:
            from . import ops

            blocks, tokens, k_block0, v_block0 = kv_blocks
            q = _qlinear(x, self.query.weight, self.query.bias).contiguous()
            a = ops.qformer_cross_attention(q, blocks, tokens, h, k_block0, v_block0, (d // h) ** -0.5)
            return self.LayerNorm(_qlinear(a, self.dense.weight, self.dense.bias, residual=x))
        if kv_proj is not None:
            q = _qlinear(x, self.query.weight, self.query.bias).view(b, n, h, d // h).transpose(1, 2)
            k = kv_proj[0].reshape(b, -1, h, d // h).transpose(1, 2)
            v = kv_proj[1].reshape(b, -1, h, d // h).transpose(1, 2)
        elif kv is None and x.is_cuda and not self.training:
            if self._qkv_fused is None or self._qkv_fused[0].device != x.device or self._qkv_fused[0].dtype != x.dtype:
                self._qkv_fused = (torch.cat([self.query.weight, self.key.weight, self.value.weight]).detach(),
                                   torch.cat([self.query.bias, self.key.bias, self.value.bias]).detach())
            qkv = _qlinear(x, *self._qkv_fused).view(b, n, 3, h, d // h).permute(2, 0, 3, 1, 4)
            q, k, v = qkv[0], qkv[1], qkv[2]
        else:
            q = self.query(x).view(b, n, h, d // h).transpose(1, 2)
            if kv is not None and kv.dtype == torch.float16 and kv.is_cuda and self.key.weight.dtype == torch.float32:
                k, v = self._project_kv_f16(kv)
                src_len = kv.shape[1]
            else:
                src = x if kv is None else kv.to(x.dtype)
                k, v, src_len = self.key(src), self.value(src), src.shape[1]
            k = k.reshape(b, src_len, h, d // h).transpose(1, 2)
            v = v.reshape(b, src_len, h, d // h).transpose(1, 2)
        a = F.scaled_dot_product_attention(q, k, v, attn_mask=mask)
        return self.LayerNorm(_qlinear(a.transpose(1, 2).reshape(b, n, d), self.dense.weight, self.dense.bias,
                                       residual=x))


class _BertFFN(nn.Module):
    def __init__(self, hidden: int, inter: int, eps: float):
        super().__init__()
        self.up = nn.Linear(hidden, inter)
        self.down = nn.Linear(inter, hidden)
        self.LayerNorm = nn.LayerNorm(hidden, eps=eps)

    def forward(self, x: torch.Tensor) -> torch.Tensor:
        hid = _qlinear(x, self.up.weight, self.up.bias, act="gelu")
        return self.LayerNorm(_qlinear(hid, self.down.weight, self.down.bias, residual=x))


class _QFormerLayer(nn.Module):
    def __init__(self, c: Blip2ITCConfig, idx: int):
        super().__init__()
        self.attention = _BertAttention(c.q_hidden, c.q_hidden, c.q_heads, c.q_ln_eps)
        self.crossattention = (_BertAttention(c.q_hidden, c.v_hidden, c.q_heads, c.q_ln_eps)
                               if idx % c.cross_attention_frequency == 0 else None)
        self.ffn_text = _BertFFN(c.q_hidden, c.q_mlp, c.q_ln_eps)
        self.ffn_query = _BertFFN(c.q_hidden, c.q_mlp, c.q_ln_eps)


class Blip2ITCModel(nn.Module):

    def __init__(self, cfg: Blip2ITCConfig):
        super().__init__()
        c = self.cfg = cfg
        n_patches = (c.image_size // c.patch_size) ** 2
        self.class_embedding = nn.Parameter(torch.zeros(1, 1, c.v_hidden))
        self.position_embedding = nn.Parameter(torch.zeros(1, n_patches + 1, c.v_hidden))
        self.patch_embedding = nn.Conv2d(3, c.v_hidden, c.patch_size, c.patch_size)
        self.blocks = nn.ModuleList([_VitBlock(c) for _ in range(c.v_layers)])
        self.post_layernorm = nn.LayerNorm(c.v_hidden, eps=c.v_ln_eps)
        self.query_tokens = nn.Parameter(torch.zeros(1, c.num_query_tokens, c.q_hidden))
        self.word_embeddings = nn.Embedding(c.vocab_size, c.q_hidden)
        self.position_embeddings = nn.Embedding(c.max_position_embeddings, c.q_hidden)
        self.q_layernorm = nn.LayerNorm(c.q_hidden, eps=c.q_ln_eps)
        self.q_layers = nn.ModuleList([_QFormerLayer(c, i) for i in range(c.q_layers)])
        self.vision_projection = nn.Linear(c.q_hidden, c.proj_dim)
        self.text_projection = nn.Linear(c.q_hidden, c.proj_dim)
        self.deferred_bias = True
        self._deferred_c: Optional[torch.Tensor] = None
        self.split_kv = True
        self.split_kv_min_rows = 32 * 257
        self._kv_all = None
        self.fused_cross_kv = True
        self._kv_pair = None

    def init_random(self, seed: int = 0) -> "Blip2ITCModel":
        dev = self.query_tokens.device
        g = torch.Generator(device=dev).manual_seed(seed)
        with torch.no_grad():
            for p in self.parameters():
                if p.dim() > 1:
                    p.copy_(torch.randn(p.shape, generator=g, device=dev) * 0.02)
                else:
                    p.zero_()
            for m in self.modules():
                if isinstance(m, nn.LayerNorm):
                    m.weight.fill_(1.0)
        self.weights_changed()
        return self

    def weights_changed(self) -> None:
        self._deferred_c = None
        self._kv_all = None
        self._kv_pair = None
        for layer in self.q_layers:
            layer.attention._qkv_fused = None
            if layer.crossattention is not None:
                layer.crossattention._kv_split = None

    def vision_dtype(self) -> torch.dtype:
        return self.patch_embedding.weight.dtype

    def set_precision(self, vision_dtype: torch.dtype = torch.float16) -> "Blip2ITCModel":
        for m in (self.patch_embedding, self.blocks, self.post_layernorm):
            m.to(vision_dtype)
        self.class_embedding.data = self.class_embedding.data.to(vision_dtype)
        self.position_embedding.data = self.position_embedding.data.to(vision_dtype)
        self.weights_changed()
        return self

    def load_hf_state_dict(self, sd: Dict[str, torch.Tensor]) -> None:
        own = dict(self.named_parameters())

        def put(name: str, src: str) -> None:
            with torch.no_grad():
                own[name].copy_(sd[src].to(own[name].dtype).reshape(own[name].shape))

        put("class_embedding", "vision_model.embeddings.class_embedding")
        put("position_embedding", "vision_model.embeddings.position_embedding")
        put("patch_embedding.weight", "vision_model.embeddings.patch_embedding.weight")
        put("patch_embedding.bias", "vision_model.embeddings.patch_embedding.bias")
        for i in range(self.cfg.v_layers):
            s, d = f"vision_model.encoder.layers.{i}.", f"blocks.{i}."
            for a, b in [("layer_norm1", "layer_norm1"), ("layer_norm2", "layer_norm2"),
                         ("self_attn.qkv", "qkv"), ("self_attn.projection", "projection"),
                         ("mlp.fc1", "fc1"), ("mlp.fc2", "fc2")]:
                put(d + b + ".weight", s + a + ".weight")
                put(d + b + ".bias", s + a + ".bias")
        put("post_layernorm.weight", "vision_model.post_layernorm.weight")
        put("post_layernorm.bias", "vision_model.post_layernorm.bias")
        put("query_tokens", "query_tokens")
        put("word_embeddings.weight", "embeddings.word_embeddings.weight")
        put("position_embeddings.weight", "embeddings.position_embeddings.weight")
        put("q_layernorm.weight", "qformer.layernorm.weight")
        put("q_layernorm.bias", "qformer.layernorm.bias")
        for i, layer in enumerate(self.q_layers):
            s, d = f"qformer.encoder.layer.{i}.", f"q_layers.{i}."
            atts = [("attention", "attention")] + ([("crossattention", "crossattention")]
                                                   if layer.crossattention is not None else [])
            for a, b in atts:
                for hf, mine in [("attention.query", "query"), ("attention.key", "key"), ("attention.value", "value"),
                                 ("output.dense", "dense"), ("output.LayerNorm", "LayerNorm")]:
                    put(f"{d}{b}.{mine}.weight", f"{s}{a}.{hf}.weight")
                    put(f"{d}{b}.{mine}.bias", f"{s}{a}.{hf}.bias")
            for hf_i, hf_o, mine in [("intermediate", "output", "ffn_text"),
                                     ("intermediate_query", "output_query", "ffn_query")]:
                put(f"{d}{mine}.up.weight", f"{s}{hf_i}.dense.weight")
                put(f"{d}{mine}.up.bias", f"{s}{hf_i}.dense.bias")
                put(f"{d}{mine}.down.weight", f"{s}{hf_o}.dense.weight")
                put(f"{d}{mine}.down.bias", f"{s}{hf_o}.dense.bias")
                put(f"{d}{mine}.LayerNorm.weight", f"{s}{hf_o}.LayerNorm.weight")
                put(f"{d}{mine}.LayerNorm.bias", f"{s}{hf_o}.LayerNorm.bias")
        for n in ("vision_projection", "text_projection"):
            put(n + ".weight", n + ".weight")
            put(n + ".bias", n + ".bias")

    def load_lavis_state_dict(self, sd: Dict[str, torch.Tensor], vit_sd: Optional[Dict[str, torch.Tensor]] = None) -> None:
        c = self.cfg
        sd = {(k[len("module."):] if k.startswith("module.") else k): v for k, v in sd.items()}
        vit = {("visual_encoder." + k): v for k, v in (vit_sd or {}).items()}
        overlap = set(vit) & set(sd)
        if overlap:
            raise KeyError(f"the vision tower is given twice (e.g. {sorted(overlap)[:2]})")
        src = {**sd, **vit}
        own = dict(self.named_parameters())
        used, fed = set(), set()

        def take(key: str) -> torch.Tensor:
            if key not in src:
                raise KeyError(f"LAVIS state dict lacks {key}" + ("" if vit_sd is not None or not key.startswith("visual_encoder.")
                                                                 else " (blip2_pretrained.pth does not carry the frozen ViT: "
                                                                      "pass eva_vit_g.pth as the vision checkpoint)"))
            used.add(key)
            return src[key]

        def put(name: str, value: torch.Tensor) -> None:
            if tuple(value.shape) != tuple(own[name].shape) and value.numel() != own[name].numel():
                raise ValueError(f"{name}: {tuple(own[name].shape)} in the graph, {tuple(value.shape)} in the file")
            with torch.no_grad():
                own[name].copy_(value.to(own[name].dtype).reshape(own[name].shape))
            fed.add(name)

        put("class_embedding", take("visual_encoder.cls_token"))
        put("position_embedding", take("visual_encoder.pos_embed"))
        put("patch_embedding.weight", take("visual_encoder.patch_embed.proj.weight"))
        put("patch_embedding.bias", take("visual_encoder.patch_embed.proj.bias"))
        for i in range(c.v_layers):
            o, d = f"visual_encoder.blocks.{i}.", f"blocks.{i}."
            for a, b in (("norm1", "layer_norm1"), ("norm2", "layer_norm2"), ("attn.proj", "projection"),
                         ("mlp.fc1", "fc1"), ("mlp.fc2", "fc2")):
                put(d + b + ".weight", take(o + a + ".weight"))
                put(d + b + ".bias", take(o + a + ".bias"))
            put(d + "qkv.weight", take(o + "attn.qkv.weight"))
            qb, vb = take(o + "attn.q_bias"), take(o + "attn.v_bias")
            put(d + "qkv.bias", torch.cat([qb, torch.zeros_like(vb), vb]))
        put("post_layernorm.weight", take("ln_vision.weight"))
        put("post_layernorm.bias", take("ln_vision.bias"))
        put("query_tokens", take("query_tokens"))
        put("word_embeddings.weight", take("Qformer.bert.embeddings.word_embeddings.weight"))
        put("position_embeddings.weight", take("Qformer.bert.embeddings.position_embeddings.weight"))
        put("q_layernorm.weight", take("Qformer.bert.embeddings.LayerNorm.weight"))
        put("q_layernorm.bias", take("Qformer.bert.embeddings.LayerNorm.bias"))
        for i, layer in enumerate(self.q_layers):
            o, d = f"Qformer.bert.encoder.layer.{i}.", f"q_layers.{i}."
            for att in ["attention"] + (["crossattention"] if layer.crossattention is not None else []):
                for theirs, mine in (("self.query", "query"), ("self.key", "key"), ("self.value", "value"),
                                     ("output.dense", "dense"), ("output.LayerNorm", "LayerNorm")):
                    put(f"{d}{att}.{mine}.weight", take(f"{o}{att}.{theirs}.weight"))
                    put(f"{d}{att}.{mine}.bias", take(f"{o}{att}.{theirs}.bias"))
            for t_i, t_o, mine in (("intermediate", "output", "ffn_text"), ("intermediate_query", "output_query", "ffn_query")):
                put(f"{d}{mine}.up.weight", take(f"{o}{t_i}.dense.weight"))
                put(f"{d}{mine}.up.bias", take(f"{o}{t_i}.dense.bias"))
                put(f"{d}{mine}.down.weight", take(f"{o}{t_o}.dense.weight"))
                put(f"{d}{mine}.down.bias", take(f"{o}{t_o}.dense.bias"))
                put(f"{d}{mine}.LayerNorm.weight", take(f"{o}{t_o}.LayerNorm.weight"))
                put(f"{d}{mine}.LayerNorm.bias", take(f"{o}{t_o}.LayerNorm.bias"))
        put("vision_projection.weight", take("vision_proj.weight"))
        put("vision_projection.bias", take("vision_proj.bias"))
        put("text_projection.weight", take("text_proj.weight"))
        put("text_projection.bias", take("text_proj.bias"))
        unfed = sorted(set(own) - fed)
        if unfed:
            raise KeyError(f"{len(unfed)} parameters of the graph were not fed, e.g. {unfed[:4]}")

        def unused_ok(k: str) -> bool:
            return (k.startswith(("Qformer.cls.", "itm_head.")) or k in ("temp", "Qformer.bert.embeddings.position_ids")
                    or k.startswith(f"visual_encoder.blocks.{c.v_layers}.")
                    or k.startswith(("visual_encoder.norm.", "visual_encoder.fc_norm.", "visual_encoder.head.")))

        left = sorted(k for k in src if k not in used and not unused_ok(k))
        if left:
            raise KeyError(f"{len(left)} tensors of the file have no place in the ITC graph, e.g. {left[:4]}")
        self.weights_changed()

    def vision_tokens(self, pixel_values: torch.Tensor) -> torch.Tensor:
        c = self.cfg
        if pixel_values.dim() == 4:
            b, g = pixel_values.shape[0], c.image_size // c.patch_size
            pixel_values = pixel_values.reshape(b, 3, g, c.patch_size, g, c.patch_size).permute(0, 2, 4, 1, 3, 5) \
                .reshape(b, g * g, 3 * c.patch_size * c.patch_size)
        w = self.patch_embedding.weight
        x = F.linear(pixel_values.to(w.dtype), w.view(w.shape[0], -1), self.patch_embedding.bias)
        x = torch.cat([self.class_embedding.expand(x.shape[0], -1, -1), x], dim=1) + self.position_embedding
        if self.deferred_bias and x.is_cuda and x.dtype == torch.float16 and c.v_hidden % 8 == 0 and c.v_hidden <= 2048:
            from . import ops

            c = self._deferred_constants()
            x = x.contiguous()
            for i, blk in enumerate(self.blocks):
                x = blk.forward_deferred(x, c[2 * i], c[2 * i + 1])
            return ops.layernorm_bias(x, c[2 * len(self.blocks)], self.post_layernorm.weight, self.post_layernorm.bias,
                                      self.post_layernorm.eps)
        for blk in self.blocks:
            x = blk(x)
        return self.post_layernorm(x)

    def _deferred_constants(self) -> torch.Tensor:
        if self._deferred_c is None or self._deferred_c.device != self.post_layernorm.weight.device:
            rows, run = [], torch.zeros(self.cfg.v_hidden, dtype=torch.float32, device=self.post_layernorm.weight.device)
            for blk in self.blocks:
                rows.append(run.clone())
                run = run + blk.projection.bias.detach().float()
                rows.append(run.clone())
                run = run + blk.fc2.bias.detach().float()
            rows.append(run.clone())
            self._deferred_c = torch.stack(rows).contiguous()
        return self._deferred_c

    def query_features(self, image_tokens: torch.Tensor) -> torch.Tensor:
        split_ok = (self.split_kv and image_tokens.dtype == torch.float16 and image_tokens.is_cuda
                    and image_tokens.shape[0] * image_tokens.shape[1] >= self.split_kv_min_rows)
        enc = image_tokens if split_ok else image_tokens.to(self.q_layernorm.weight.dtype)
        h = self.q_layernorm(self.query_tokens).expand(enc.shape[0], -1, -1)
        fused = split_ok and self._fused_cross_ok(enc)
        blocks = self._project_all_kv_blocks(enc) if fused else None
        proj = self._project_all_kv(enc) if split_ok and not fused else None
        hid, at = self.cfg.q_hidden, 0
        for layer in self.q_layers:
            h = layer.attention(h)
            if layer.crossattention is not None:
                if blocks is not None:
                    h = layer.crossattention(h, kv_blocks=(blocks, enc.shape[1], at // 64, (at + hid) // 64))
                    at += 2 * hid
                elif proj is not None:
                    h = layer.crossattention(h, kv_proj=(proj[..., at:at + hid], proj[..., at + hid:at + 2 * hid]))
                    at += 2 * hid
                else:
                    h = layer.crossattention(h, kv=enc)
            h = layer.ffn_query(h)
        return h

    def _fused_cross_ok(self, tokens16: torch.Tensor) -> bool:
        from . import ops

        c = self.cfg
        return (self.fused_cross_kv and KV_SPLIT_PIECES == 2 and not torch.is_grad_enabled()
                and self.q_layernorm.weight.dtype == torch.float32
                and c.q_hidden % c.q_heads == 0 and c.q_hidden // c.q_heads == ops.QFORMER_ATTENTION_HEAD
                and c.num_query_tokens <= ops.QFORMER_ATTENTION_MAX_QUERIES
                and 1 <= tokens16.shape[1] <= ops.QFORMER_ATTENTION_MAX_TOKENS and c.v_hidden % 64 == 0
                and tokens16.shape[0] * tokens16.shape[1] * c.v_hidden * 2 < (1 << 32))

    def _kv_all_pieces(self, device):
        if self._kv_all is None or self._kv_all[0].device != device:
            cross = [l.crossattention for l in self.q_layers if l.crossattention is not None]
            w = torch.cat([torch.cat([c.key.weight, c.value.weight]) for c in cross])
            bias = torch.cat([torch.cat([c.key.bias, c.value.bias]) for c in cross]).detach().float()
            w1, w2, w3 = _exact_split3(w)
            self._kv_all = (w1.t(), w2.t(), w3.t(), bias)
            self._kv_pair = None
        return self._kv_all

    def _project_all_kv_blocks(self, tokens16: torch.Tensor) -> torch.Tensor:
        from . import ops

        w1t, w2t, _, bias = self._kv_all_pieces(tokens16.device)
        if self._kv_pair is None:
            self._kv_pair = (ops.interleave_pair_weights(w1t.t(), w2t.t()), bias.contiguous())
        return ops.linear_pair_f32(tokens16.reshape(-1, tokens16.shape[-1]), *self._kv_pair)

    def _project_all_kv(self, tokens16: torch.Tensor) -> torch.Tensor:
        pieces = self._kv_all_pieces(tokens16.device)
        o = _split_gemm(tokens16.reshape(-1, tokens16.shape[-1]), pieces[:3], pieces[3])
        return o.view(*tokens16.shape[:-1], -1)

    def text_feature(self, input_ids: torch.Tensor, attention_mask: Optional[torch.Tensor] = None) -> torch.Tensor:
        pos = torch.arange(input_ids.shape[1], device=input_ids.device)[None]
        h = self.q_layernorm(self.word_embeddings(input_ids) + self.position_embeddings(pos))
        mask = None
        if attention_mask is not None:
            mask = (attention_mask[:, None, None, :] > 0)
        for layer in self.q_layers:
            h = layer.ffn_text(layer.attention(h, mask=mask))
        return F.normalize(self.text_projection(h[:, 0, :]), dim=-1)

    def itc_reference_head(self, query_feats: torch.Tensor, text_feat: torch.Tensor) -> torch.Tensor:
        img = F.normalize(self.vision_projection(query_feats.float()), dim=-1)
        return torch.einsum("bqd,bd->bq", img, text_feat.float().expand(img.shape[0], -1)).max(dim=1).values


_CAPTION_STRIP = re.compile(r"([.!\"()*#:;~])")


def blip_caption(text: str, max_words: int = 50) -> str:
    t = _CAPTION_STRIP.sub(" ", text.lower())
    t = re.sub(r"\s{2,}", " ", t).rstrip("\n").strip(" ")
    words = t.split(" ")
    return " ".join(words[:max_words]) if len(words) > max_words else t


class HashTokenizer:

    def __init__(self, vocab_size: int, max_len: int):
        self.vocab_size, self.max_len = vocab_size, max_len

    def __call__(self, text: str) -> List[int]:
        ids = [101 % self.vocab_size]
        for w in text.split():
            hv = int.from_bytes(hashlib.sha1(w.encode()).digest()[:4], "little")
            ids.append(1000 % self.vocab_size + hv % max(1, self.vocab_size - 1000))
        ids = ids[: self.max_len - 1] + [102 % self.vocab_size]
        return ids


class BLIP2ITM:

    def __init__(self, name: str = "blip2_image_text_matching", model_type: str = "pretrain", device=None,
                 model_dir: Optional[str] = None, config: Optional[Blip2ITCConfig] = None,
                 vision_dtype: torch.dtype = torch.float16, seed: int = 0, allow_random_init: bool = False,
                 strict_hip_attention: bool = True, checkpoint: Optional[str] = None, vit_checkpoint: Optional[str] = None,
                 tokenizer_dir: Optional[str] = None) -> None:
        from ..mapping.base_map import require_gpu
        from .. import _lib

        self.device = require_gpu(device)
        _lib.lib()
        from . import ops as _ops

        _ops.use_tuned_gemms()
        self.cfg = config or Blip2ITCConfig()
        self.tokenizer = None
        model_dir = model_dir or os.environ.get("BLIP2ITM_MODEL_DIR")
        checkpoint = checkpoint or os.environ.get("BLIP2_LAVIS_CHECKPOINT")
        vit_checkpoint = vit_checkpoint or os.environ.get("EVA_VIT_G_CHECKPOINT")
        if checkpoint and not model_dir:
            for f in (checkpoint, vit_checkpoint):
                if f and not os.path.isfile(f):
                    raise FileNotFoundError(f"BLIP-2 checkpoint {f!r} not found")
            self.model = Blip2ITCModel(self.cfg)
            ck = torch.load(checkpoint, map_location="cpu", weights_only=True)
            vit = torch.load(vit_checkpoint, map_location="cpu", weights_only=True) if vit_checkpoint else None
            self.model.load_lavis_state_dict(ck["model"] if isinstance(ck, dict) and "model" in ck else ck,
                                             vit["model"] if isinstance(vit, dict) and "model" in vit else vit)
            self.tokenizer = self._lavis_tokenizer(tokenizer_dir)
            self.weights = f"lavis:{checkpoint}" + (f" + {vit_checkpoint}" if vit_checkpoint else "")
        elif model_dir:
            self.model = Blip2ITCModel(self.cfg)
            self._load_pretrained(model_dir)
            self.weights = f"pretrained:{model_dir}"
        elif not (allow_random_init or config is not None):
            raise ValueError("BLIP2ITM needs `checkpoint` (+ `vit_checkpoint`): LAVIS' blip2_pretrained.pth and eva_vit_g.pth, what "
                             "the reference loads -- or model_dir / BLIP2ITM_MODEL_DIR (a Salesforce/blip2-itm-vit-g directory); "
                             "pass allow_random_init=True for a randomly initialised network (benchmarks / geometry tests only)")
        else:
            with torch.device(self.device):
                self.model = Blip2ITCModel(self.cfg)
            self.model.init_random(seed)
            self.weights = "random-init"
        if self.tokenizer is None:
            self.tokenizer = HashTokenizer(self.cfg.vocab_size, self.cfg.max_txt_len)
        self.model.eval().to(self.device).set_precision(vision_dtype)
        for blk in self.model.blocks:
            blk.pack_heads()
            blk.strict_hip_attention = bool(strict_hip_attention)
        self._text_cache: Dict[str, torch.Tensor] = {}
        self._prompt_cache: Dict[tuple, tuple] = {}
        self._proj_t = None
        self._graphs, self._prompt_graphs = {}, {}
        self.two_stream_min = None
        self._side_stream = None

    def _lavis_tokenizer(self, tokenizer_dir: Optional[str]):
        from transformers import BertTokenizer

        path = tokenizer_dir or os.environ.get("BLIP2_TOKENIZER")
        try:
            if path:
                vocab = path if os.path.isfile(path) else os.path.join(path, "vocab.txt")
                tok = BertTokenizer(vocab_file=vocab, do_lower_case=True)
            else:
                tok = BertTokenizer.from_pretrained("bert-base-uncased", local_files_only=True)
                if len(tok) < 30522:
                    raise FileNotFoundError("no cached bert-base-uncased vocabulary")
        except Exception as exc:
            raise ValueError("BLIP-2 weights need the bert-base-uncased vocabulary: pass tokenizer_dir (or set BLIP2_TOKENIZER) "
                             "to a directory with its vocab.txt") from exc
        tok.add_special_tokens({"bos_token": "[DEC]"})
        return lambda t: tok(t, truncation=True, max_length=self.cfg.max_txt_len)["input_ids"]

    @property
    def strict_hip_attention(self) -> bool:
        return all(blk.strict_hip_attention for blk in self.model.blocks)

    @strict_hip_attention.setter
    def strict_hip_attention(self, on: bool) -> None:
        for blk in self.model.blocks:
            blk.strict_hip_attention = bool(on)

    @property
    def attention_path(self) -> str:
        flags = {bool(blk.hip_attention) for blk in self.model.blocks}
        return "hip" if flags == {True} else "library" if flags == {False} else "mixed"

    def mlp_path(self, n_images: int) -> str:
# ... 173 lines not shown
```

### vlfm_amd/vlm/ops.py

```python
from __future__ import annotations

import ctypes
from typing import Dict, Optional, Tuple

import numpy as np
import torch

from .. import _lib

CLIP_MEAN = (0.48145466, 0.4578275, 0.40821073)
CLIP_STD = (0.26862954, 0.26130258, 0.27577711)
_DTYPE_CODE = {torch.float32: 0, torch.float16: 1, torch.bfloat16: 2}
_coeff_cache: Dict[Tuple[str, int, int], Tuple[torch.Tensor, torch.Tensor, int]] = {}


def _stream() -> int:
    return torch._C._cuda_getCurrentRawStream(torch._C._cuda_getDevice())


def resample_coeffs(in_size: int, out_size: int, bilinear: bool = False) -> Tuple[np.ndarray, np.ndarray, int]:
    bounds = np.zeros((out_size, 2), np.int32)
    cap = out_size * (2 * int(np.ceil(2.0 * max(1.0, in_size / out_size))) + 1)
    kk = np.zeros(cap, np.int32)
    ks = ctypes.c_int(0)
# ... 128 lines not shown
    n, c, h, w = y.shape
    _lib.check(_lib.lib().vlfm_bias_act_nchw(y.data_ptr(), bias.data_ptr(), n, c, h * w, 0 if y.dtype == torch.float32 else 1,
                                             _ACT_CODE[act], _stream()), "bias_act_nchw")
    return y


_BIAS_ACT_MAX_PLANES = 65535 * 16


class BiasAct(torch.nn.Module):

    def __init__(self, bias: torch.Tensor, act=None, inplace: bool = False):
        super().__init__()
        self.bias = torch.nn.Parameter(bias.detach().clone(), requires_grad=False)
        self.act = act
        self.inplace = inplace

    def forward(self, x):
        return bias_act(x, self.bias, self.act, inplace=self.inplace)


def bias_act(x: torch.Tensor, bias: torch.Tensor, act=None, inplace: bool = False) -> torch.Tensor:
    if (inplace and x.is_cuda and x.dim() == 4 and x.dtype in (torch.float32, torch.float16) and x.is_contiguous()
            and not x.requires_grad and x.shape[0] * x.shape[1] <= _BIAS_ACT_MAX_PLANES):
        return bias_act_(x, bias if bias.dtype == x.dtype else bias.to(x.dtype), act)
    y = x + bias.to(x.dtype).view(1, -1, 1, 1)
    if act == "gelu":
        return torch.nn.functional.gelu(y)
    if act == "silu":
        return torch.nn.functional.silu(y)
    return y


def depthwise_conv3x3(x: torch.Tensor, weight: torch.Tensor, bias, stride: int = 1, gelu: bool = False) -> torch.Tensor:
    assert x.is_cuda and x.dtype == torch.float32 and x.dim() == 4 and x.is_contiguous()
    n, c, h, w = x.shape
    assert weight.shape == (c, 1, 3, 3) and weight.dtype == torch.float32 and weight.is_contiguous()
    ho, wo = (h - 1) // stride + 1, (w - 1) // stride + 1
    y = torch.empty((n, c, ho, wo), dtype=torch.float32, device=x.device)
    _lib.check(_lib.lib().vlfm_dwconv3x3_f32(x.data_ptr(), weight.data_ptr(), bias.data_ptr() if bias is not None else None,
                                             y.data_ptr(), n, c, h, w, int(stride), int(gelu), _stream()), "dwconv3x3_f32")
    return y


def layernorm_rows(x: torch.Tensor, weight: torch.Tensor, bias: torch.Tensor, eps: float, window: int = 0, shift: int = 0,
                   pad_zero: bool = False) -> torch.Tensor:
    assert x.is_cuda and x.dtype == torch.float32 and x.dim() == 4 and x.is_contiguous()
    B, H, W, C = x.shape
    assert weight.dtype == torch.float32 and bias.dtype == torch.float32 and weight.numel() == C == bias.numel()
    if window > 0:
        nwy, nwx = (H + window - 1) // window, (W + window - 1) // window
        out = torch.empty((B * nwy * nwx, window * window, C), dtype=torch.float32, device=x.device)
    else:
        out = torch.empty_like(x)
    _lib.check(_lib.lib().vlfm_layernorm_rows_shifted_f32(x.data_ptr(), weight.data_ptr(), bias.data_ptr(), out.data_ptr(), B, H, W, C,
                                                          int(window), float(eps), int(shift), int(pad_zero), _stream()),
               "layernorm_rows_f32")
    return out


def window_reverse_add_(x: torch.Tensor, windows: torch.Tensor, window: int, shift: int = 0) -> torch.Tensor:
    assert x.is_cuda and x.dtype == torch.float32 and x.dim() == 4 and x.is_contiguous()
    B, H, W, C = x.shape
    nwy, nwx = (H + window - 1) // window, (W + window - 1) // window
    assert windows.is_contiguous() and windows.dtype == torch.float32 and windows.numel() == B * nwy * nwx * window * window * C
    _lib.check(_lib.lib().vlfm_window_reverse_add_shifted_f32(x.data_ptr(), windows.data_ptr(), B, H, W, C, int(window), int(shift),
                                                              _stream()), "window_reverse_add_f32")
    return x


def depthwise_conv3x3_nhwc(x: torch.Tensor, w9c: torch.Tensor, bias) -> torch.Tensor:
    assert x.is_cuda and x.dtype == torch.float32 and x.dim() == 4 and x.is_contiguous()
    B, H, W, C = x.shape
    assert w9c.shape == (9, C) and w9c.is_contiguous() and w9c.dtype == torch.float32
    out = torch.empty_like(x)
    _lib.check(_lib.lib().vlfm_dwconv3x3_nhwc_f32(x.data_ptr(), w9c.data_ptr(), bias.data_ptr() if bias is not None else None,
                                                  out.data_ptr(), B, H, W, C, _stream()), "dwconv3x3_nhwc_f32")
    return out


def window_attention(qkv: torch.Tensor, bias_t: torch.Tensor, heads: int, scale: float, mask_t=None) -> torch.Tensor:
    assert qkv.is_cuda and qkv.dtype == torch.float32 and qkv.dim() == 3 and qkv.is_contiguous() and qkv.shape[2] == heads * 96
    nw, n, _ = qkv.shape
    assert bias_t.shape == (heads, n, n) and bias_t.is_contiguous() and bias_t.dtype == torch.float32 and n <= 256
    out = torch.empty((nw, n, heads * 32), dtype=torch.float32, device=qkv.device)
    per_image = 1
    if mask_t is not None:
        assert mask_t.dim() == 3 and mask_t.shape[1:] == (n, n) and mask_t.is_contiguous() and mask_t.dtype == torch.float32
        per_image = mask_t.shape[0]
        assert nw % per_image == 0
    _lib.check(_lib.lib().vlfm_window_attention_masked_f32(qkv.data_ptr(), bias_t.data_ptr(),
                                                           mask_t.data_ptr() if mask_t is not None else None, per_image,
                                                           out.data_ptr(), nw, n, heads, float(scale), _stream()),
               "window_attention_f32")
    return out


GEMM_F16_EPILOGUE = {"bias": 0, "bias_gelu": 1, "accumulate": 2}


def linear_f16_supported(x: torch.Tensor, weight: torch.Tensor) -> bool:
    k = weight.shape[1]
    return (x.is_cuda and x.dtype == torch.float16 and weight.dtype == torch.float16 and x.shape[-1] == k and k % 64 == 0
            and weight.shape[0] % 8 == 0 and x.numel() * 2 < (1 << 32) and weight.numel() * 2 < (1 << 32))


def linear_f16(x: torch.Tensor, weight: torch.Tensor, bias: Optional[torch.Tensor] = None, epilogue: str = "bias",
               out: Optional[torch.Tensor] = None) -> torch.Tensor:
    assert x.is_cuda and x.dtype == torch.float16 and x.is_contiguous() and x.dim() == 2
    assert weight.dtype == torch.float16 and weight.is_contiguous() and weight.shape[1] == x.shape[1]
    assert bias is None or (bias.dtype == torch.float16 and bias.is_contiguous())
    M, K = x.shape
    N = weight.shape[0]
    if out is None:
        assert epilogue != "accumulate", "accumulate needs the tensor to accumulate into"
        out = torch.empty((M, N), dtype=torch.float16, device=x.device)
    else:
        assert out.dtype == torch.float16 and out.is_contiguous() and out.shape == (M, N) and out.device == x.device
    _lib.check(_lib.lib().vlfm_gemm_f16_nt(x.data_ptr(), weight.data_ptr(), bias.data_ptr() if bias is not None else None,
                                           out.data_ptr(), M, N, K, GEMM_F16_EPILOGUE[epilogue], _stream()), "gemm_f16_nt")
    return out


def linear_gelu(x: torch.Tensor, weight: torch.Tensor, bias: torch.Tensor) -> torch.Tensor:
    return linear_f16(x, weight, bias, "bias_gelu")


def interleave_pair_weights(w1: torch.Tensor, w2: torch.Tensor) -> torch.Tensor:
    assert w1.shape == w2.shape and w1.dtype == w2.dtype == torch.float16 and w1.dim() == 2 and w1.shape[0] % 64 == 0
    n, k = w1.shape
    return torch.stack([w1.reshape(n // 64, 64, k), w2.reshape(n // 64, 64, k)], dim=1).reshape(2 * n, k).contiguous()


def linear_pair_f32(x: torch.Tensor, w_pair: torch.Tensor, bias: Optional[torch.Tensor] = None,
                    out: Optional[torch.Tensor] = None) -> torch.Tensor:
    assert x.is_cuda and x.dtype == torch.float16 and x.is_contiguous() and x.dim() == 2
    assert w_pair.dtype == torch.float16 and w_pair.is_contiguous() and w_pair.shape[1] == x.shape[1] and w_pair.shape[0] % 128 == 0
    M, K = x.shape
    N = w_pair.shape[0] // 2
    assert bias is None or (bias.dtype == torch.float32 and bias.is_contiguous() and bias.numel() == N)
    if out is None:
        out = torch.empty((N // 64, M, 64), dtype=torch.float32, device=x.device)
    else:
        assert out.dtype == torch.float32 and out.is_contiguous() and out.shape == (N // 64, M, 64) and out.device == x.device
    _lib.check(_lib.lib().vlfm_gemm_f16_pair_f32_nt(x.data_ptr(), w_pair.data_ptr(), bias.data_ptr() if bias is not None else None,
                                                    out.data_ptr(), M, N, K, _stream()), "gemm_f16_pair_f32_nt")
    return out


QFORMER_ATTENTION_MAX_TOKENS, QFORMER_ATTENTION_MAX_QUERIES, QFORMER_ATTENTION_HEAD = 257, 32, 64


def qformer_cross_attention(q: torch.Tensor, kv_blocks: torch.Tensor, tokens: int, heads: int, k_block0: int, v_block0: int,
                            scale: float, out: Optional[torch.Tensor] = None) -> torch.Tensor:
    assert q.is_cuda and q.dtype == torch.float32 and q.is_contiguous() and q.dim() == 3 and q.shape[2] == heads * 64
    assert kv_blocks.dtype == torch.float32 and kv_blocks.is_contiguous() and kv_blocks.dim() == 3 and kv_blocks.shape[2] == 64
    assert kv_blocks.device == q.device and max(k_block0, v_block0) + heads <= kv_blocks.shape[0] and min(k_block0, v_block0) >= 0
    B, Q, _ = q.shape
    if out is None:
        out = torch.empty_like(q)
    else:
        assert out.dtype == torch.float32 and out.is_contiguous() and out.shape[1:] == q.shape[1:] and out.shape[0] >= B
    _lib.check(_lib.lib().vlfm_qformer_cross_attention_f32(q.data_ptr(), kv_blocks.data_ptr(), out.data_ptr(), B, tokens, Q, heads,
                                                           k_block0, v_block0, kv_blocks.shape[1], float(scale), _stream()),
               "qformer_cross_attention_f32")
    return out


VIT_ATTENTION_TOKENS, VIT_ATTENTION_HEADS = 257, (88,)


def vit_attention(qkv: torch.Tensor, batch: int, tokens: int, heads: int, head_dim: int, scale: float) -> torch.Tensor:
    assert qkv.is_cuda and qkv.dtype == torch.float16 and qkv.is_contiguous()
    assert qkv.numel() == batch * tokens * 3 * heads * head_dim
    out = torch.empty((batch * tokens, heads * head_dim), dtype=torch.float16, device=qkv.device)
    _lib.check(_lib.lib().vlfm_vit_attention_f16(qkv.data_ptr(), out.data_ptr(), batch, tokens, heads, head_dim,
                                                 float(scale), _stream()), "vit_attention_f16")
    return out


_ACT32 = {None: 0, "none": 0, "relu": 1, "gelu": 2}
GEMM_F32_PRECISION = {"exact": 0, "split": 1}
_overflow_flags: Dict[tuple, torch.Tensor] = {}
_split_cache: Dict[int, tuple] = {}


def gemm_f32_overflow_flag(device, owner: str = "") -> torch.Tensor:
    d = torch.device(device)
    index = d.index if d.index is not None else (torch.cuda.current_device() if d.type == "cuda" else 0)
    key = (d.type, index, owner)
    if key not in _overflow_flags:
        _overflow_flags[key] = torch.zeros(1, dtype=torch.int32, device=torch.device(d.type, index))
    return _overflow_flags[key]


def tensor_version(t: torch.Tensor) -> int:
    try:
        return t._version
    except RuntimeError:
        return 0


def split_weight(weight: torch.Tensor, owner: str = "") -> Tuple[torch.Tensor, torch.Tensor]:
    import weakref

    key = id(weight)
    hit = _split_cache.get(key)
    if hit is not None and hit[0]() is weight and hit[1] == tensor_version(weight) and hit[2] == weight.data_ptr():
        if hit[6]:
            gemm_f32_overflow_flag(weight.device, owner).bitwise_or_(hit[5])
        return hit[3], hit[4]
    if len(_split_cache) > 2048:
        for k in [k for k, v in _split_cache.items() if v[0]() is None]:
            del _split_cache[k]
    w = weight.detach().contiguous()
    hi = torch.empty(w.shape, dtype=torch.float16, device=w.device)
    lo = torch.empty_like(hi)
    bad = torch.zeros(1, dtype=torch.int32, device=w.device)
    _lib.check(_lib.lib().vlfm_split_f32_to_f16_pair(w.data_ptr(), hi.data_ptr(), lo.data_ptr(), w.numel(), bad.data_ptr(),
                                                     _stream()), "split_f32")
    gemm_f32_overflow_flag(w.device, owner).bitwise_or_(bad)
    _split_cache[key] = [weakref.ref(weight), tensor_version(weight), weight.data_ptr(), hi, lo, bad, False, owner]
    return hi, lo


def split_weights_bad(device, owner: str = "") -> bool:
    d = torch.device(device)
    entries = [v for v in _split_cache.values() if v[7] == owner and v[0]() is not None and v[5].device.type == d.type
               and (d.index is None or v[5].device.index == d.index)]
    if not entries:
        return False
    verdict = torch.cat([v[5] for v in entries]).cpu().tolist()
    for v, b in zip(entries, verdict):
        v[6] = bool(b)
    return any(verdict)


def linear_f32_supported(x: torch.Tensor, weight: torch.Tensor) -> bool:
    k = weight.shape[1]
    return (x.is_cuda and x.dtype == torch.float32 and weight.dtype == torch.float32 and k % 32 == 0 and x.shape[-1] == k
            and weight.shape[0] >= 32 and x.numel() // k >= 64 and not torch.is_grad_enabled())


def linear_f32(x: torch.Tensor, weight: torch.Tensor, bias=None, act=None, residual=None, precision: str = "exact",
               out=None, owner: str = "") -> torch.Tensor:
    K = weight.shape[1]
    N = weight.shape[0]
    lead = x.shape[:-1]
    x2 = x.reshape(-1, K)
    if not x2.is_contiguous() or x2.data_ptr() % 16:
        x2 = x2.contiguous()
    w = weight if weight.is_contiguous() else weight.contiguous()
    M = x2.shape[0]
    if out is None:
        out = torch.empty((M, N), dtype=torch.float32, device=x.device)
    res = None
    if residual is not None:
        res = residual.reshape(M, N)
        if not res.is_contiguous() or res.data_ptr() % 16:
            res = res.contiguous()
    b = None
    if bias is not None:
        b = bias if bias.is_contiguous() else bias.contiguous()
    prec = GEMM_F32_PRECISION[precision]
    hi = lo = None
    if prec == 1:
        hi, lo = split_weight(w, owner)
    _lib.check(_lib.lib().vlfm_gemm_f32_nt(x2.data_ptr(), w.data_ptr(), b.data_ptr() if b is not None else None,
                                           res.data_ptr() if res is not None else None, out.data_ptr(), M, N, K, _ACT32[act], prec,
                                           hi.data_ptr() if hi is not None else None, lo.data_ptr() if lo is not None else None,
                                           gemm_f32_overflow_flag(x.device, owner).data_ptr(), _stream()), "gemm_f32_nt")
    return out.view(*lead, N)


_tuned_gemms_state = None


def use_tuned_gemms() -> bool:
    global _tuned_gemms_state
    if _tuned_gemms_state is None:
        import os

        path = os.path.join(os.path.dirname(os.path.dirname(os.path.abspath(__file__))), "tunableop_results.csv")
        ok = False
        if os.environ.get("VLFM_TUNED_GEMMS", "1") != "0" and os.path.exists(path) and torch.cuda.is_available():
            try:
                import torch.cuda.tunable as tunable

                import tempfile

                tunable.enable(True)
                tunable.tuning_enable(False)
                tunable.set_filename(os.path.join(tempfile.gettempdir(), f"vlfm_amd_tunableop_{os.getpid()}.csv"))
                ok = bool(tunable.read_file(path))
            except Exception as exc:
                import warnings

                warnings.warn(f"tuned GEMM solutions not loaded ({type(exc).__name__}: {exc})")
                ok = False
        _tuned_gemms_state = ok
    return _tuned_gemms_state
```

Baseline: 1740 env-steps/s.

## Restructure Q-Former split-f16 GEMMs with pre-split planes, M64 geometry, and layer-0 folding

Measured after the change: 1749 env-steps/s (median of 6 runs). No clear change (+0.5%).

```diff
diff --git a/include/vlfm_amd.h b/include/vlfm_amd.h
--- a/include/vlfm_amd.h
+++ b/include/vlfm_amd.h
@@ -173,6 +173,9 @@
 
 int vlfm_qformer_cross_attention_f32(const void* d_q, const void* d_kv_blocks, void* d_out, int batch, int tokens, int queries,
                                      int heads, int k_block0, int v_block0, int m_total, float scale, void* stream);
+int vlfm_qformer_cross_attention_f32_strided(const void* d_q, long long q_batch_stride, const void* d_kv_blocks, void* d_out, int batch,
+                                             int tokens, int queries, int heads, int k_block0, int v_block0, int m_total, float scale,
+                                             void* stream);
 
 int vlfm_gemm_f16_tile_order(int m, int n, int group_m, int* out, int capacity_pairs);
 int vlfm_gemm_f16_work_items(int m, int n, int grid, int* out, int capacity_pairs);
@@ -180,6 +183,15 @@
 int vlfm_split_f32_to_f16_pair(const float* d_src, void* d_hi, void* d_lo, long long count, int* d_overflow, void* stream);
 int vlfm_gemm_f32_nt(const float* d_x, const float* d_w, const float* d_bias, const float* d_residual, float* d_c, int m, int n,
                      int k, int activation, int precision, const void* d_w_hi, const void* d_w_lo, int* d_overflow, void* stream);
+
+#define VLFM_GEMM_F32_GEOM_128 1
+#define VLFM_GEMM_F32_GEOM_M64 2
+int vlfm_gemm_f32_split_nt(const float* d_x, const void* d_x_hi, const void* d_x_lo, const float* d_bias, const float* d_residual,
+                           float* d_c, void* d_c_hi, void* d_c_lo, int m, int n, int k, int activation, const void* d_w_hi,
+                           const void* d_w_lo, int* d_overflow, int residual_period, int geometry, void* stream);
+int vlfm_layernorm768_f32_planes(const float* d_x, const float* d_gamma, const float* d_beta, float* d_y, void* d_hi, void* d_lo, int rows,
+                                 int dim, float eps, int* d_overflow, void* stream);
+int vlfm_gemm_f32_split_geometry(int m, int n, int k, int cu_count, int x_planes, long long* out);
 
 
 int vlfm_layernorm_rows_f32(const float* d_x, const float* d_gamma, const float* d_beta, float* d_out, int batch, int height,
diff --git a/vlfm_amd/_lib.py b/vlfm_amd/_lib.py
--- a/vlfm_amd/_lib.py
+++ b/vlfm_amd/_lib.py
@@ -125,6 +125,11 @@
         L.vlfm_gemm_f16_pair_f32_nt.argtypes = [vp, vp, vp, vp, ci, ci, ci, vp]
         L.vlfm_qformer_cross_attention_f32.argtypes = [vp, vp, vp, ci, ci, ci, ci, ci, ci, ci, ctypes.c_float, vp]
         L.vlfm_gemm_f32_nt.argtypes = [vp, vp, vp, vp, vp, ci, ci, ci, ci, ci, vp, vp, vp, vp]
+        L.vlfm_qformer_cross_attention_f32_strided.argtypes = [vp, ctypes.c_longlong, vp, vp, ci, ci, ci, ci, ci, ci, ci, ctypes.c_float,
+                                                               vp]
+        L.vlfm_gemm_f32_split_nt.argtypes = [vp, vp, vp, vp, vp, vp, vp, vp, ci, ci, ci, ci, vp, vp, vp, ci, ci, vp]
+        L.vlfm_layernorm768_f32_planes.argtypes = [vp, vp, vp, vp, vp, vp, ci, ci, ctypes.c_float, vp, vp]
+        L.vlfm_gemm_f32_split_geometry.argtypes = [ci, ci, ci, ci, ci, ctypes.POINTER(ctypes.c_longlong)]
         L.vlfm_split_f32_to_f16_pair.argtypes = [vp, vp, vp, ctypes.c_longlong, vp, vp]
         L.vlfm_layernorm_rows_f32.argtypes = [vp, vp, vp, vp, ci, ci, ci, ci, ci, ctypes.c_float, vp]
         L.vlfm_window_reverse_add_f32.argtypes = [vp, vp, ci, ci, ci, ci, ci, vp]
diff --git a/vlfm_amd/csrc/gemm_f32.hip b/vlfm_amd/csrc/gemm_f32.hip
--- a/vlfm_amd/csrc/gemm_f32.hip
+++ b/vlfm_amd/csrc/gemm_f32.hip
@@ -36,6 +36,11 @@
     int* overflow;
     const _Float16* w_hi;
     const _Float16* w_lo;
+    int res_mask;
+    const _Float16* x_hi;
+    const _Float16* x_lo;
+    _Float16* c_hi;
+    _Float16* c_lo;
 };
 
 __device__ inline float gelu_erf(float v) {
@@ -52,6 +57,17 @@
     return fmaf(-0.5f * u, e, fmaxf(v, 0.0f));
 }
 
+__device__ inline void split4(const floatx4 v, half4& hi, half4& lo, bool& over) {
+#pragma unroll
+    for (int e = 0; e < 4; e++) {
+        const float a = v[e];
+        over |= !(fabsf(a) < 65504.0f);
+        const _Float16 hh = (_Float16)a;
+        hi[e] = hh;
+        lo[e] = (_Float16)((a - (float)hh) * 2048.0f);
+    }
+}
+
 using lds_ptr = __attribute__((address_space(3))) unsigned char*;
 using gbl_ptr = const __attribute__((address_space(1))) unsigned char*;
 
@@ -80,10 +96,10 @@
     }
 }
 
-template <bool SPLIT>
-__device__ inline void store_tile(const Args& a, unsigned char* smem, const floatx16 (&acc)[2][2], const floatx16 (&cross)[2][2],
+template <bool SPLIT, int NJ = 2>
+__device__ inline void store_tile(const Args& a, unsigned char* smem, const floatx16 (&acc)[2][NJ], const floatx16 (&cross)[2][NJ],
                                   int act, int wave, int wn, int wm, int lane, int m0, int n0) {
-    unsigned char* stg = smem + wave * EPI_WAVE;
+    unsigned char* stg = smem + wave * (EPI_WAVE / 2 * NJ);
     const int c32 = lane & 31, h4 = (lane >> 5) * 4;
     floatx4 bias4[2][4];
 #pragma unroll
@@ -106,7 +122,7 @@
             const int nl = i * 32 + g * 8 + h4;
             const floatx4 b = bias4[i][g];
 #pragma unroll
-            for (int j = 0; j < 2; j++) {
+            for (int j = 0; j < NJ; j++) {
                 floatx4 v;
 #pragma unroll
                 for (int e = 0; e < 4; e++) {
@@ -125,26 +141,47 @@
     const bool vec = (a.N & 3) == 0;
     const int n = n0 + wn * 64 + chunk * 4;
     const bool fast = vec && n + 4 <= a.N;
-    floatx4 r[16], v[16];
-#pragma unroll
-    for (int it = 0; it < 16; it++) {
-        const int m = m0 + wm * 64 + it * 4 + rsub;
+    constexpr int NIT = 8 * NJ;
+    floatx4 r[NIT], v[NIT];
+    bool over = false;
+#pragma unroll
+    for (int it = 0; it < NIT; it++) {
+        const int m = m0 + wm * 32 * NJ + it * 4 + rsub;
         r[it] = floatx4{0.f, 0.f, 0.f, 0.f};
-        if (a.residual && fast && m < a.M) r[it] = *reinterpret_cast<const floatx4*>(a.residual + (size_t)m * a.N + n);
-    }
-#pragma unroll
-    for (int it = 0; it < 16; it++) v[it] = *reinterpret_cast<const floatx4*>(stg + (it * 4 + rsub) * EPI_ROW + chunk * 16);
-#pragma unroll
-    for (int it = 0; it < 16; it++) {
-        const int m = m0 + wm * 64 + it * 4 + rsub;
+        if (a.residual && fast && m < a.M)
+            r[it] = *reinterpret_cast<const floatx4*>(a.residual + (size_t)(m & a.res_mask) * a.N + n);
+    }
+#pragma unroll
+    for (int it = 0; it < NIT; it++) v[it] = *reinterpret_cast<const floatx4*>(stg + (it * 4 + rsub) * EPI_ROW + chunk * 16);
+#pragma unroll
+    for (int it = 0; it < NIT; it++) {
+        const int m = m0 + wm * 32 * NJ + it * 4 + rsub;
         if (m >= a.M || n >= a.N) continue;
         const size_t at = (size_t)m * a.N + n;
         if (fast) {
-            *reinterpret_cast<floatx4*>(a.c + at) = v[it] + r[it];
+            const floatx4 o = v[it] + r[it];
+            *reinterpret_cast<floatx4*>(a.c + at) = o;
+            if (SPLIT && a.c_hi) {
+                half4 hi, lo;
+                split4(o, hi, lo, over);
+                *reinterpret_cast<half4*>(a.c_hi + at) = hi;
+                *reinterpret_cast<half4*>(a.c_lo + at) = lo;
+            }
         } else {
-            for (int e = 0; e < 4 && n + e < a.N; e++) a.c[at + e] = v[it][e] + (a.residual ? a.residual[at + e] : 0.f);
-        }
-    }
+            const size_t rat = (size_t)(m & a.res_mask) * a.N + n;
+            for (int e = 0; e < 4 && n + e < a.N; e++) {
+                const float o = v[it][e] + (a.residual ? a.residual[rat + e] : 0.f);
+                a.c[at + e] = o;
+                if (SPLIT && a.c_hi) {
+                    over |= !(fabsf(o) < 65504.0f);
+                    const _Float16 hh = (_Float16)o;
+                    a.c_hi[at + e] = hh;
+                    a.c_lo[at + e] = (_Float16)((o - (float)hh) * 2048.0f);
+                }
+            }
+        }
+    }
+    if (SPLIT && over && a.overflow) atomicOr(a.overflow, 1);
 }
 
 __global__ __launch_bounds__(256, 2) void gemm_f32_exact_kernel(Args a, int act) {
@@ -210,29 +247,21 @@
 
 __device__ inline int sslot(int row, int slot) { return (slot ^ ((row >> 2) & 3)) << 4; }
 
-__device__ inline void split4(const floatx4 v, half4& hi, half4& lo, bool& over) {
-#pragma unroll
-    for (int e = 0; e < 4; e++) {
-        const float a = v[e];
-        over |= !(fabsf(a) < 65504.0f);
-        const _Float16 hh = (_Float16)a;
-        hi[e] = hh;
-        lo[e] = (_Float16)((a - (float)hh) * 2048.0f);
-    }
-}
-
-template <int NI>
+template <int NI, int NJ = 2>
 struct SplitGeom {
     static constexpr int TN = 64 * NI;
+    static constexpr int TM = 64 * NJ;
     static constexpr int WOPER = TN * SROWB;
-    static constexpr int XO = 0, WO = 2 * SOPER;
-    static constexpr int BUF = 2 * SOPER + 2 * WOPER;
-    static constexpr int LDS = 4 * EPI_WAVE > 2 * BUF ? 4 * EPI_WAVE : 2 * BUF;
+    static constexpr int XOPER = TM * SROWB;
+    static constexpr int XO = 0, WO = 2 * XOPER;
+    static constexpr int BUF = 2 * XOPER + 2 * WOPER;
+    static constexpr int EPI = 4 * (EPI_WAVE / 2 * NJ);
+    static constexpr int LDS = EPI > 2 * BUF ? EPI : 2 * BUF;
 };
 
-template <int NI>
+template <int NI, int NJ = 2, bool XP = false>
 __device__ __forceinline__ void gemm_f32_split_body(const Args& a, int act) {
-    using G = SplitGeom<NI>;
+    using G = SplitGeom<NI, NJ>;
     extern __shared__ __attribute__((aligned(16))) unsigned char smem[];
     lds_ptr lds = (lds_ptr)smem;
     const int tid = threadIdx.x, lane = tid & 63;
@@ -240,22 +269,22 @@
     const int wn = wave >> 1, wm = wave & 1;
     int tm, tn;
     tile_of_block(a, tm, tn);
-    const int m0 = tm * TB, n0 = tn * G::TN;
+    const int m0 = tm * G::TM, n0 = tn * G::TN;
     const int NT = a.K / TK;
 
-    floatx16 acc[NI][2], crs[NI][2];
+    floatx16 acc[NI][NJ], crs[NI][NJ];
 #pragma unroll
     for (int i = 0; i < NI; i++)
 #pragma unroll
-        for (int j = 0; j < 2; j++)
+        for (int j = 0; j < NJ; j++)
 #pragma unroll
             for (int e = 0; e < 16; e++) { acc[i][j][e] = 0.f; crs[i][j][e] = 0.f; }
 
-    floatx4 xr[4];
+    floatx4 xr[2 * NJ];
     bool over = false;
     auto load_x = [&](int k0) {
 #pragma unroll
-        for (int u = 0; u < 4; u++) {
+        for (int u = 0; u < 2 * NJ; u++) {
             const int idx = tid + 256 * u, r = idx >> 3, pc = idx & 7;
             const int rm = min(m0 + r, a.M - 1);
             xr[u] = *reinterpret_cast<const floatx4*>(a.x + (size_t)rm * a.K + k0 + pc * 4);
@@ -263,13 +292,27 @@
     };
     auto put_x = [&](int buf) {
 #pragma unroll
-        for (int u = 0; u < 4; u++) {
+        for (int u = 0; u < 2 * NJ; u++) {
             const int idx = tid + 256 * u, r = idx >> 3, pc = idx & 7;
             half4 hi, lo;
             split4(xr[u], hi, lo, over);
             const int off = r * SROWB + sslot(r, pc >> 1) + (pc & 1) * 8;
             *reinterpret_cast<half4*>(smem + buf + G::XO + off) = hi;
-            *reinterpret_cast<half4*>(smem + buf + G::XO + SOPER + off) = lo;
+            *reinterpret_cast<half4*>(smem + buf + G::XO + G::XOPER + off) = lo;
+        }
+    };
+    auto stage_x = [&](int buf, int k0) {
+        const int sub = lane >> 2, p = lane & 3;
+#pragma unroll
+        for (int j = 0; j < NJ; j++) {
+            const int chunk = wave * NJ + j;
+            const int r = chunk * 16 + sub;
+            const int s = p ^ ((r >> 2) & 3);
+            const int rm = min(m0 + r, a.M - 1);
+            const size_t g = (size_t)rm * a.K + k0 + s * 8;
+            const int dst = __builtin_amdgcn_readfirstlane(buf + G::XO + chunk * 1024);
+            __builtin_amdgcn_global_load_lds((gbl_ptr)(a.x_hi + g), lds + dst, 16, 0, 0);
+            __builtin_amdgcn_global_load_lds((gbl_ptr)(a.x_lo + g), lds + dst + G::XOPER, 16, 0, 0);
         }
     };
     auto stage_w = [&](int buf, int k0) {
@@ -287,9 +330,14 @@
         }
     };
 
-    load_x(0);
-    stage_w(0, 0);
-    put_x(0);
+    if constexpr (XP) {
+        stage_x(0, 0);
+        stage_w(0, 0);
+    } else {
+        load_x(0);
+        stage_w(0, 0);
+        put_x(0);
+    }
     __builtin_amdgcn_s_waitcnt(0x0F70);
     __builtin_amdgcn_s_waitcnt(0xC07F);
     __builtin_amdgcn_s_barrier();
@@ -299,13 +347,14 @@
     for (int t = 0; t < NT; t++) {
         const int cur = (t & 1) * G::BUF;
         if (t + 1 < NT) {
-            load_x((t + 1) * TK);
+            if constexpr (XP) stage_x(cur ^ G::BUF, (t + 1) * TK);
+            else load_x((t + 1) * TK);
             stage_w(cur ^ G::BUF, (t + 1) * TK);
         }
 #pragma unroll
         for (int kk = 0; kk < 2; kk++) {
             const int s = kk * 2 + h;
-            half8 whi[NI], wlo[NI], xhi[2], xlo[2];
+            half8 whi[NI], wlo[NI], xhi[NJ], xlo[NJ];
 #pragma unroll
             for (int i = 0; i < NI; i++) {
                 const int R = wn * 32 * NI + i * 32 + r32, o = cur + G::WO + R * SROWB + sslot(R, s);
@@ -313,21 +362,21 @@
                 wlo[i] = *reinterpret_cast<const half8*>(smem + o + G::WOPER);
             }
 #pragma unroll
-            for (int j = 0; j < 2; j++) {
-                const int R = wm * 64 + j * 32 + r32, o = cur + G::XO + R * SROWB + sslot(R, s);
+            for (int j = 0; j < NJ; j++) {
+                const int R = wm * 32 * NJ + j * 32 + r32, o = cur + G::XO + R * SROWB + sslot(R, s);
                 xhi[j] = *reinterpret_cast<const half8*>(smem + o);
-                xlo[j] = *reinterpret_cast<const half8*>(smem + o + SOPER);
+                xlo[j] = *reinterpret_cast<const half8*>(smem + o + G::XOPER);
             }
 #pragma unroll
             for (int i = 0; i < NI; i++)
 #pragma unroll
-                for (int j = 0; j < 2; j++) {
+                for (int j = 0; j < NJ; j++) {
                     acc[i][j] = __builtin_amdgcn_mfma_f32_32x32x16_f16(whi[i], xhi[j], acc[i][j], 0, 0, 0);
                     crs[i][j] = __builtin_amdgcn_mfma_f32_32x32x16_f16(whi[i], xlo[j], crs[i][j], 0, 0, 0);
                     crs[i][j] = __builtin_amdgcn_mfma_f32_32x32x16_f16(wlo[i], xhi[j], crs[i][j], 0, 0, 0);
                 }
         }
-        if (t + 1 < NT) put_x(cur ^ G::BUF);
+        if (!XP && t + 1 < NT) put_x(cur ^ G::BUF);
         __builtin_amdgcn_s_waitcnt(0x0F70);
         __builtin_amdgcn_s_waitcnt(0xC07F);
         __builtin_amdgcn_s_barrier();
@@ -336,12 +385,15 @@
     if (over && a.overflow) atomicOr(a.overflow, 1);
 #pragma unroll
     for (int half = 0; half < NI / 2; half++)
-        store_tile<true>(a, smem, reinterpret_cast<const floatx16(&)[2][2]>(acc[2 * half]),
-                         reinterpret_cast<const floatx16(&)[2][2]>(crs[2 * half]), act, wave, 0, wm, lane, m0,
-                         n0 + wn * 32 * NI + half * 64);
+        store_tile<true, NJ>(a, smem, reinterpret_cast<const floatx16(&)[2][NJ]>(acc[2 * half]),
+                             reinterpret_cast<const floatx16(&)[2][NJ]>(crs[2 * half]), act, wave, 0, wm, lane, m0,
+                             n0 + wn * 32 * NI + half * 64);
 }
 
 __global__ __launch_bounds__(256, 2) void gemm_f32_split_kernel(Args a, int act) { gemm_f32_split_body<2>(a, act); }
+__global__ __launch_bounds__(256, 3) void gemm_f32_split_kernel_m64(Args a, int act) { gemm_f32_split_body<2, 1>(a, act); }
+__global__ __launch_bounds__(256, 2) void gemm_f32_split_kernel_xp(Args a, int act) { gemm_f32_split_body<2, 2, true>(a, act); }
+__global__ __launch_bounds__(256, 3) void gemm_f32_split_kernel_m64_xp(Args a, int act) { gemm_f32_split_body<2, 1, true>(a, act); }
 
 __global__ void split_f32_kernel(const float* __restrict__ src, _Float16* __restrict__ hi, _Float16* __restrict__ lo, long long n,
                                  int* overflow) {
@@ -385,6 +437,8 @@
     a.M = m; a.N = n; a.K = k;
     a.tiles_m = (m + TB - 1) / TB; a.tiles_n = (n + TB - 1) / TB;
     a.overflow = d_overflow; a.w_hi = (const _Float16*)d_w_hi; a.w_lo = (const _Float16*)d_w_lo;
+    a.res_mask = 0x7fffffff;
+    a.x_hi = a.x_lo = nullptr; a.c_hi = a.c_lo = nullptr;
     if ((long long)a.tiles_m * a.tiles_n > 0x7fffffffLL) return fail(VLFM_ERR_CAPACITY, "gemm_f32_nt: too many tiles");
     const dim3 grid(a.tiles_m * a.tiles_n), block(256);
     static LdsOptIn opt_exact, opt_split;
@@ -401,3 +455,94 @@
     VLFM_KLAUNCH(gemm_f32_split_kernel, grid, block, SplitGeom<2>::LDS, (hipStream_t)stream, a, activation);
     return check_launch("gemm_f32_split_kernel");
 }
+
+namespace {
+struct GeomCount { int tile_m, wg_per_cu; long long tiles, slots, rounds, last; };
+
+GeomCount count_geometry(int geometry, int m, int n, int cus) {
+    GeomCount g;
+    g.tile_m = geometry == VLFM_GEMM_F32_GEOM_M64 ? 64 : 128;
+    g.wg_per_cu = geometry == VLFM_GEMM_F32_GEOM_M64 ? 3 : 2;
+    g.tiles = (long long)((m + g.tile_m - 1) / g.tile_m) * ((n + 127) / 128);
+    g.slots = (long long)cus * g.wg_per_cu;
+    g.rounds = (g.tiles + g.slots - 1) / g.slots;
+    g.last = g.tiles - (g.rounds - 1) * g.slots;
+    return g;
+}
+}
+
+extern "C" int vlfm_gemm_f32_split_geometry(int m, int n, int k, int cu_count, int x_planes, long long* out) {
+    if (m <= 0 || n <= 0 || k <= 0 || cu_count <= 0) return fail(VLFM_ERR_INVALID, "gemm_f32_split_geometry: bad argument");
+    const GeomCount a = count_geometry(VLFM_GEMM_F32_GEOM_128, m, n, cu_count), b = count_geometry(VLFM_GEMM_F32_GEOM_M64, m, n, cu_count);
+    if (out) {
+        const GeomCount* g[2] = {&a, &b};
+        for (int i = 0; i < 2; i++) {
+            out[4 * i] = g[i]->tiles; out[4 * i + 1] = g[i]->slots; out[4 * i + 2] = g[i]->rounds; out[4 * i + 3] = g[i]->last;
+        }
+    }
+    const long long cost_a = a.rounds * a.wg_per_cu * a.tile_m, cost_b = b.rounds * b.wg_per_cu * b.tile_m;
+    const bool fuller = b.last * a.slots >= a.last * b.slots;
+    const bool lds_bound = x_planes && (b.last == b.slots || b.rounds > 2);
+    return cost_b < cost_a && fuller && !lds_bound ? VLFM_GEMM_F32_GEOM_M64 : VLFM_GEMM_F32_GEOM_128;
+}
+
+extern "C" int vlfm_gemm_f32_split_nt(const float* d_x, const void* d_x_hi, const void* d_x_lo, const float* d_bias,
+                                      const float* d_residual, float* d_c, void* d_c_hi, void* d_c_lo, int m, int n, int k, int activation,
+                                      const void* d_w_hi, const void* d_w_lo, int* d_overflow, int residual_period, int geometry,
+                                      void* stream) {
+    if (m == 0 || n == 0) return VLFM_OK;
+    const bool xp = d_x_hi != nullptr;
+    if ((!d_x && !xp) || !d_c || !d_w_hi || !d_w_lo || !d_overflow || m < 0 || n < 0 || k <= 0 || (k % TK) != 0 || activation < 0 ||
+        activation > 2 || geometry < 0 || geometry > VLFM_GEMM_F32_GEOM_M64 || (d_x_hi == nullptr) != (d_x_lo == nullptr) ||
+        (d_c_hi == nullptr) != (d_c_lo == nullptr))
+        return fail(VLFM_ERR_INVALID, "gemm_f32_split_nt: K must be a multiple of 32, activation 0..2, geometry 0..2, planes in pairs, "
+                                      "weight planes and flag given");
+    if (residual_period < 0 || (residual_period & (residual_period - 1)) != 0)
+        return fail(VLFM_ERR_INVALID, "gemm_f32_split_nt: the residual's row period must be 0 or a power of two");
+    if (((uintptr_t)d_x | (uintptr_t)d_x_hi | (uintptr_t)d_x_lo | (uintptr_t)d_c | (uintptr_t)d_c_hi | (uintptr_t)d_c_lo |
+         (uintptr_t)d_residual | (uintptr_t)d_w_hi | (uintptr_t)d_w_lo) & 15)
+        return fail(VLFM_ERR_INVALID, "gemm_f32_split_nt: X, C, their planes, residual and the split weights must be 16-byte aligned");
+    if (geometry == 0) geometry = vlfm_gemm_f32_split_geometry(m, n, k, device_cu_count(), xp ? 1 : 0, nullptr);
+    if (geometry < 0) return geometry;
+    using GM64 = SplitGeom<2, 1>;
+    using G128 = SplitGeom<2>;
+    const bool m64 = geometry == VLFM_GEMM_F32_GEOM_M64;
+    const int tile_m = m64 ? GM64::TM : G128::TM;
+    Args a;
+    a.x = d_x; a.w = nullptr; a.bias = d_bias; a.residual = d_residual; a.c = d_c;
+    a.M = m; a.N = n; a.K = k;
+    a.tiles_m = (m + tile_m - 1) / tile_m; a.tiles_n = (n + TB - 1) / TB;
+    a.overflow = d_overflow; a.w_hi = (const _Float16*)d_w_hi; a.w_lo = (const _Float16*)d_w_lo;
+    a.res_mask = residual_period ? residual_period - 1 : 0x7fffffff;
+    a.x_hi = (const _Float16*)d_x_hi; a.x_lo = (const _Float16*)d_x_lo; a.c_hi = (_Float16*)d_c_hi; a.c_lo = (_Float16*)d_c_lo;
+    if ((long long)a.tiles_m * a.tiles_n > 0x7fffffffLL) return fail(VLFM_ERR_CAPACITY, "gemm_f32_split_nt: too many tiles");
+    const dim3 grid(a.tiles_m * a.tiles_n), block(256);
+    static LdsOptIn opt[4];
+    const void* fns[4] = {reinterpret_cast<const void*>(gemm_f32_split_kernel), reinterpret_cast<const void*>(gemm_f32_split_kernel_m64),
+                          reinterpret_cast<const void*>(gemm_f32_split_kernel_xp), reinterpret_cast<const void*>(gemm_f32_split_kernel_m64_xp)};
+    const int which = (m64 ? 1 : 0) + (xp ? 2 : 0);
+    const int lds = m64 ? GM64::LDS : G128::LDS;
+    if (lds > 64 * 1024 && !opt[which].ensure(fns[which], lds)) return fail(VLFM_ERR_HIP, "gemm_f32_split_nt: cannot opt in to the LDS size");
+    switch (which) {
+        case 0: {
+            VLFM_TIMED("gemm_f32_split_kernel", stream);
+            VLFM_KLAUNCH(gemm_f32_split_kernel, grid, block, lds, (hipStream_t)stream, a, activation);
+            return check_launch("gemm_f32_split_kernel");
+        }
+        case 1: {
+            VLFM_TIMED("gemm_f32_split_kernel_m64", stream);
+            VLFM_KLAUNCH(gemm_f32_split_kernel_m64, grid, block, lds, (hipStream_t)stream, a, activation);
+            return check_launch("gemm_f32_split_kernel_m64");
+        }
+        case 2: {
+            VLFM_TIMED("gemm_f32_split_kernel_xp", stream);
+            VLFM_KLAUNCH(gemm_f32_split_kernel_xp, grid, block, lds, (hipStream_t)stream, a, activation);
+            return check_launch("gemm_f32_split_kernel_xp");
+        }
+        default: {
+            VLFM_TIMED("gemm_f32_split_kernel_m64_xp", stream);
+            VLFM_KLAUNCH(gemm_f32_split_kernel_m64_xp, grid, block, lds, (hipStream_t)stream, a, activation);
+            return check_launch("gemm_f32_split_kernel_m64_xp");
+        }
+    }
+}
diff --git a/vlfm_amd/csrc/host.cpp b/vlfm_amd/csrc/host.cpp
--- a/vlfm_amd/csrc/host.cpp
+++ b/vlfm_amd/csrc/host.cpp
@@ -13,7 +13,7 @@
 }
 
 extern "C" const char* vlfm_last_error(void) { return vlfm::g_last_error.c_str(); }
-extern "C" int vlfm_abi_version(void) { return 16; }
+extern "C" int vlfm_abi_version(void) { return 17; }
 
 namespace {
 
diff --git a/vlfm_amd/csrc/qformer_attention.hip b/vlfm_amd/csrc/qformer_attention.hip
--- a/vlfm_amd/csrc/qformer_attention.hip
+++ b/vlfm_amd/csrc/qformer_attention.hip
@@ -24,6 +24,7 @@
     int B, T, Q, heads, k_block0, v_block0, M_total;
     int rows_pad;
     float scale_log2e;
+    long long q_stride;
 };
 
 struct QaKernel {
@@ -64,7 +65,7 @@
         issue_v(vg, row0, n_ins);
     }
     __device__ inline void load_q(int b, int h, float (&qn)[32]) const {
-        const float* src = a.q + ((size_t)b * a.Q + min(col, a.Q - 1)) * ((size_t)a.heads * 64) + (size_t)h * 64 + 32 * g;
+        const float* src = a.q + (size_t)b * (size_t)a.q_stride + (size_t)min(col, a.Q - 1) * ((size_t)a.heads * 64) + (size_t)h * 64 + 32 * g;
 #pragma unroll
         for (int c = 0; c < 8; c++) {
             const qa_f32x4 v = *reinterpret_cast<const qa_f32x4*>(src + 4 * c);
@@ -247,10 +248,12 @@
 
 using namespace vlfm;
 
-extern "C" int vlfm_qformer_cross_attention_f32(const void* d_q, const void* d_kv_blocks, void* d_out, int batch, int tokens,
-                                                int queries, int heads, int k_block0, int v_block0, int m_total, float scale,
-                                                void* stream) {
+extern "C" int vlfm_qformer_cross_attention_f32_strided(const void* d_q, long long q_batch_stride, const void* d_kv_blocks, void* d_out,
+                                                        int batch, int tokens, int queries, int heads, int k_block0, int v_block0,
+                                                        int m_total, float scale, void* stream) {
     if (batch == 0) return VLFM_OK;
+    if (q_batch_stride != 0 && (q_batch_stride < (long long)queries * heads * 64 || (q_batch_stride & 3) != 0))
+        return fail(VLFM_ERR_INVALID, "qformer_cross_attention_f32: the batch stride of Q is 0 or at least queries * heads * 64, a multiple of 4");
     if (!d_q || !d_kv_blocks || !d_out || batch < 0 || tokens < 1 || tokens > QA_MAX_T || queries < 1 || queries > QA_MAX_Q || heads < 1 ||
         k_block0 < 0 || v_block0 < 0 || (long long)batch * tokens > (long long)m_total)
         return fail(VLFM_ERR_INVALID, "qformer_cross_attention_f32: head width 64, 1-32 queries, 1-257 tokens, batch * tokens <= m_total");
@@ -261,6 +264,7 @@
     a.B = batch; a.T = tokens; a.Q = queries; a.heads = heads; a.k_block0 = k_block0; a.v_block0 = v_block0; a.M_total = m_total;
     a.rows_pad = (tokens + 3) & ~3;
     a.scale_log2e = scale * 1.4426950408889634f;
+    a.q_stride = q_batch_stride;
     const size_t lds = 2 * (size_t)a.rows_pad * QA_ROWB + QA_MERGE;
     const void* fn = reinterpret_cast<const void*>(qformer_cross_attention_kernel);
     static LdsOptIn opt;
@@ -272,3 +276,10 @@
     VLFM_KLAUNCH(qformer_cross_attention_kernel, grid, block, lds, stream, a);
     return check_launch("qformer_cross_attention_kernel");
 }
+
+extern "C" int vlfm_qformer_cross_attention_f32(const void* d_q, const void* d_kv_blocks, void* d_out, int batch, int tokens,
+                                                int queries, int heads, int k_block0, int v_block0, int m_total, float scale,
+                                                void* stream) {
+    return vlfm_qformer_cross_attention_f32_strided(d_q, (long long)queries * heads * 64, d_kv_blocks, d_out, batch, tokens, queries, heads,
+                                                    k_block0, v_block0, m_total, scale, stream);
+}
diff --git a/vlfm_amd/csrc/vlm_ops.hip b/vlfm_amd/csrc/vlm_ops.hip
--- a/vlfm_amd/csrc/vlm_ops.hip
+++ b/vlfm_amd/csrc/vlm_ops.hip
@@ -313,6 +313,64 @@
 #pragma unroll
         for (int i = 0; i < NV; i++) { cur[i] = nxt[i]; nxt[i] = nx2[i]; }
     }
+}
+
+constexpr int LNQ_D = 768;
+
+__global__ __launch_bounds__(256) void layernorm768_f32_planes_kernel(const float* __restrict__ x, const float* __restrict__ gamma,
+                                                                      const float* __restrict__ beta, float* __restrict__ y,
+                                                                      _Float16* __restrict__ hi, _Float16* __restrict__ lo, int rows,
+                                                                      float eps, int* overflow) {
+    typedef _Float16 h4 __attribute__((ext_vector_type(4)));
+    const int lane = threadIdx.x & 63, row = (blockIdx.x * blockDim.x + threadIdx.x) >> 6;
+    if (row >= rows) return;
+    float4 v[3], g[3], b[3];
+#pragma unroll
+    for (int i = 0; i < 3; i++) {
+        v[i] = reinterpret_cast<const float4*>(x + (size_t)row * LNQ_D)[lane + 64 * i];
+        g[i] = reinterpret_cast<const float4*>(gamma)[lane + 64 * i];
+        b[i] = reinterpret_cast<const float4*>(beta)[lane + 64 * i];
+    }
+    float sum = 0.0f;
+#pragma unroll
+    for (int i = 0; i < 3; i++) sum += (v[i].x + v[i].y) + (v[i].z + v[i].w);
+#pragma unroll
+    for (int off = 32; off > 0; off >>= 1) sum += __shfl_xor(sum, off, 64);
+    const float mean = sum * (1.0f / LNQ_D);
+    float sq = 0.0f;
+#pragma unroll
+    for (int i = 0; i < 3; i++) {
+        const float d0 = v[i].x - mean, d1 = v[i].y - mean, d2 = v[i].z - mean, d3 = v[i].w - mean;
+        sq += (d0 * d0 + d1 * d1) + (d2 * d2 + d3 * d3);
+    }
+#pragma unroll
+    for (int off = 32; off > 0; off >>= 1) sq += __shfl_xor(sq, off, 64);
+    const float rstd = 1.0f / sqrtf(sq * (1.0f / LNQ_D) + eps);
+    bool over = false;
+#pragma unroll
+    for (int i = 0; i < 3; i++) {
+        float4 o;
+        o.x = (v[i].x - mean) * rstd * g[i].x + b[i].x;
+        o.y = (v[i].y - mean) * rstd * g[i].y + b[i].y;
+        o.z = (v[i].z - mean) * rstd * g[i].z + b[i].z;
+        o.w = (v[i].w - mean) * rstd * g[i].w + b[i].w;
+        const size_t at = (size_t)row * LNQ_D + 4 * (lane + 64 * i);
+        *reinterpret_cast<float4*>(y + at) = o;
+        if (hi) {
+            const float e[4] = {o.x, o.y, o.z, o.w};
+            h4 ph, pl;
+#pragma unroll
+            for (int j = 0; j < 4; j++) {
+                over |= !(fabsf(e[j]) < 65504.0f);
+                const _Float16 hh = (_Float16)e[j];
+                ph[j] = hh;
+                pl[j] = (_Float16)((e[j] - (float)hh) * 2048.0f);
+            }
+            *reinterpret_cast<h4*>(hi + at) = ph;
+            *reinterpret_cast<h4*>(lo + at) = pl;
+        }
+    }
+    if (over && overflow) atomicOr(overflow, 1);
 }
 
 __global__ __launch_bounds__(512) void itc_head_kernel(const float* __restrict__ proj, int NQ, int P,
@@ -594,3 +652,17 @@
     }
     return check_launch("layernorm_bias_f16_kernel");
 }
+
+extern "C" int vlfm_layernorm768_f32_planes(const float* d_x, const float* d_gamma, const float* d_beta, float* d_y, void* d_hi, void* d_lo,
+                                            int rows, int dim, float eps, int* d_overflow, void* stream) {
+    if (rows == 0) return VLFM_OK;
+    if (!d_x || !d_gamma || !d_beta || !d_y || rows < 0 || dim != LNQ_D || (d_hi == nullptr) != (d_lo == nullptr) || (d_hi && !d_overflow))
+        return fail(VLFM_ERR_INVALID, "layernorm768_f32_planes: rows of 768, planes in pairs and with the overflow flag");
+    if (((uintptr_t)d_x | (uintptr_t)d_gamma | (uintptr_t)d_beta | (uintptr_t)d_y | (uintptr_t)d_hi | (uintptr_t)d_lo) & 15)
+        return fail(VLFM_ERR_INVALID, "layernorm768_f32_planes: pointers must be 16-byte aligned");
+    const dim3 grid((rows + 3) / 4), block(256);
+    VLFM_TIMED("layernorm768_f32_planes_kernel", stream);
+    VLFM_KLAUNCH(layernorm768_f32_planes_kernel, grid, block, 0, (hipStream_t)stream, d_x, d_gamma, d_beta, d_y, (_Float16*)d_hi,
+                 (_Float16*)d_lo, rows, eps, d_overflow);
+    return check_launch("layernorm768_f32_planes_kernel");
+}
diff --git a/vlfm_amd/vlm/blip2itm.py b/vlfm_amd/vlm/blip2itm.py
--- a/vlfm_amd/vlm/blip2itm.py
+++ b/vlfm_amd/vlm/blip2itm.py
@@ -190,7 +190,7 @@
 
     if (x.is_cuda and x.dtype == torch.float32 and lin_w.dtype == torch.float32 and not torch.is_grad_enabled()
             and x.numel() // x.shape[-1] >= QFORMER_SPLIT_MIN_ROWS and ops.linear_f32_supported(x, lin_w)):
-        return ops.linear_f32(x, lin_w, lin_b, act=act, residual=residual, precision="split", owner="blip2")
+        return ops.linear_f32_split(x, lin_w, lin_b, act=act, residual=residual, owner="blip2")
     y = F.linear(x, lin_w, lin_b)
     if act == "gelu":
         y = F.gelu(y)
@@ -302,6 +302,9 @@
         self._kv_all = None
         self.fused_cross_kv = True
         self._kv_pair = None
+        self.layer0_fold = True
+        self._layer0 = None
+        self.self_path_planes = True
 
     def init_random(self, seed: int = 0) -> "Blip2ITCModel":
         dev = self.query_tokens.device
@@ -322,6 +325,7 @@
         self._deferred_c = None
         self._kv_all = None
         self._kv_pair = None
+        self._layer0 = None
         for layer in self.q_layers:
             layer.attention._qkv_fused = None
             if layer.crossattention is not None:
@@ -505,6 +509,8 @@
         blocks = self._project_all_kv_blocks(enc) if fused else None
         proj = self._project_all_kv(enc) if split_ok and not fused else None
         hid, at = self.cfg.q_hidden, 0
+        if fused and self._self_path_ok(enc):
+            return self._query_features_planes(h, blocks, enc)
         for layer in self.q_layers:
             h = layer.attention(h)
             if layer.crossattention is not None:
@@ -529,6 +535,82 @@
                 and c.num_query_tokens <= ops.QFORMER_ATTENTION_MAX_QUERIES
                 and 1 <= tokens16.shape[1] <= ops.QFORMER_ATTENTION_MAX_TOKENS and c.v_hidden % 64 == 0
                 and tokens16.shape[0] * tokens16.shape[1] * c.v_hidden * 2 < (1 << 32))
+
+    def _self_path_ok(self, enc: torch.Tensor) -> bool:
+        c = self.cfg
+        return (self.self_path_planes and c.q_hidden == 768 and c.q_mlp % 32 == 0 and not self.training
+                and enc.shape[0] * c.num_query_tokens >= QFORMER_SPLIT_MIN_ROWS and self.query_tokens.dtype == torch.float32)
+
+    def _query_features_planes(self, h: torch.Tensor, blocks: torch.Tensor, enc: torch.Tensor) -> torch.Tensor:
+        from . import ops
+
+        c = self.cfg
+        B, n, d, heads, T = enc.shape[0], c.num_query_tokens, c.q_hidden, c.q_heads, enc.shape[1]
+        scale = (d // heads) ** -0.5
+
+        def gemm(x, lin, **kw):
+            return ops.linear_f32_split(x, lin.weight, lin.bias, owner="blip2", **kw)
+
+        def norm(x, ln, planes=True):
+            return ops.layernorm768_f32(x, ln.weight, ln.bias, ln.eps, planes=planes, owner="blip2")
+
+        folded = self._layer0_constant(enc)
+        h = h.contiguous()
+        h_pl = None
+        at = 0
+        for i, layer in enumerate(self.q_layers):
+            att, cross, ffn = layer.attention, layer.crossattention, layer.ffn_query
+            if i == 0 and folded is not None:
+                s, s_pl = folded[0], None
+            else:
+                if i == 0:
+                    h = h.expand(B, -1, -1).contiguous()
+                if att._qkv_fused is None or att._qkv_fused[0].device != h.device or att._qkv_fused[0].dtype != h.dtype:
+                    att._qkv_fused = (torch.cat([att.query.weight, att.key.weight, att.value.weight]).detach(),
+                                      torch.cat([att.query.bias, att.key.bias, att.value.bias]).detach())
+                qkv = ops.linear_f32_split(h, *att._qkv_fused, owner="blip2", x_planes=h_pl).view(B, n, 3, heads, d // heads) \
+                    .permute(2, 0, 3, 1, 4)
+                a = F.scaled_dot_product_attention(qkv[0], qkv[1], qkv[2]).transpose(1, 2).reshape(B, n, d)
+                s, s_pl = norm(gemm(a, att.dense, residual=h), att.LayerNorm)
+            if cross is not None:
+                kb, vb = at // 64, (at + d) // 64
+                at += 2 * d
+                if s_pl is None:
+                    a = ops.qformer_cross_attention(folded[1], blocks, T, heads, kb, vb, scale, batch=B)
+                    t = gemm(a, cross.dense, residual=s, residual_period=n)
+                else:
+                    q = gemm(s, cross.query, x_planes=s_pl)
+                    a = ops.qformer_cross_attention(q, blocks, T, heads, kb, vb, scale)
+                    t = gemm(a, cross.dense, residual=s)
+                s, s_pl = norm(t, cross.LayerNorm)
+            u, u_pl = gemm(s, ffn.up, act="gelu", x_planes=s_pl, out_planes=True)
+            last = i + 1 == len(self.q_layers)
+            out = norm(gemm(u, ffn.down, residual=s, x_planes=u_pl), ffn.LayerNorm, planes=not last)
+            h, h_pl = (out, None) if last else out
+        return h
+
+    def _layer0_constant(self, enc: torch.Tensor):
+        from . import ops
+
+        nq = self.cfg.num_query_tokens
+        l0 = self.q_layers[0]
+        if not (self.layer0_fold and l0.crossattention is not None and nq & (nq - 1) == 0):
+            return None
+        if self._layer0 is None or self._layer0[0].device != enc.device:
+            if torch.cuda.is_current_stream_capturing():
+                return None
+            att, cross = l0.attention, l0.crossattention
+            h0 = self.q_layernorm(self.query_tokens).contiguous()
+            n, d, heads = nq, self.cfg.q_hidden, att.heads
+            w_qkv = torch.cat([att.query.weight, att.key.weight, att.value.weight]).detach()
+            b_qkv = torch.cat([att.query.bias, att.key.bias, att.value.bias]).detach()
+            qkv = ops.linear_f32_split(h0, w_qkv, b_qkv, owner="blip2").view(1, n, 3, heads, d // heads).permute(2, 0, 3, 1, 4)
+            a = F.scaled_dot_product_attention(qkv[0], qkv[1], qkv[2]).transpose(1, 2).reshape(1, n, d)
+            t = ops.linear_f32_split(a, att.dense.weight, att.dense.bias, residual=h0, owner="blip2")
+            s0 = ops.layernorm768_f32(t, att.LayerNorm.weight, att.LayerNorm.bias, att.LayerNorm.eps, owner="blip2")
+            q0 = ops.linear_f32_split(s0, cross.query.weight, cross.query.bias, owner="blip2").contiguous()
+            self._layer0 = (s0, q0)
+        return self._layer0
 
     def _kv_all_pieces(self, device):
         if self._kv_all is None or self._kv_all[0].device != device:
diff --git a/vlfm_amd/vlm/ops.py b/vlfm_amd/vlm/ops.py
--- a/vlfm_amd/vlm/ops.py
+++ b/vlfm_amd/vlm/ops.py
@@ -304,18 +304,22 @@
 
 
 def qformer_cross_attention(q: torch.Tensor, kv_blocks: torch.Tensor, tokens: int, heads: int, k_block0: int, v_block0: int,
-                            scale: float, out: Optional[torch.Tensor] = None) -> torch.Tensor:
+                            scale: float, out: Optional[torch.Tensor] = None, batch: Optional[int] = None) -> torch.Tensor:
     assert q.is_cuda and q.dtype == torch.float32 and q.is_contiguous() and q.dim() == 3 and q.shape[2] == heads * 64
     assert kv_blocks.dtype == torch.float32 and kv_blocks.is_contiguous() and kv_blocks.dim() == 3 and kv_blocks.shape[2] == 64
     assert kv_blocks.device == q.device and max(k_block0, v_block0) + heads <= kv_blocks.shape[0] and min(k_block0, v_block0) >= 0
     B, Q, _ = q.shape
+    q_stride = Q * heads * 64
+    if batch is not None:
+        assert B == 1 and batch >= 1
+        B, q_stride = batch, 0
     if out is None:
-        out = torch.empty_like(q)
+        out = torch.empty((B, Q, heads * 64), dtype=torch.float32, device=q.device)
     else:
         assert out.dtype == torch.float32 and out.is_contiguous() and out.shape[1:] == q.shape[1:] and out.shape[0] >= B
-    _lib.check(_lib.lib().vlfm_qformer_cross_attention_f32(q.data_ptr(), kv_blocks.data_ptr(), out.data_ptr(), B, tokens, Q, heads,
-                                                           k_block0, v_block0, kv_blocks.shape[1], float(scale), _stream()),
-               "qformer_cross_attention_f32")
+    _lib.check(_lib.lib().vlfm_qformer_cross_attention_f32_strided(q.data_ptr(), q_stride, kv_blocks.data_ptr(), out.data_ptr(), B,
+                                                                   tokens, Q, heads, k_block0, v_block0, kv_blocks.shape[1],
+                                                                   float(scale), _stream()), "qformer_cross_attention_f32")
     return out
 
 
@@ -425,6 +429,70 @@
     return out.view(*lead, N)
 
 
+GEMM_F32_GEOMETRY = {"auto": 0, "128": 1, "m64": 2}
+
+
+def gemm_f32_split_geometry(m: int, n: int, k: int, cus: int, x_planes: bool = False) -> Tuple[str, Dict[str, Dict[str, int]]]:
+    out = (ctypes.c_longlong * 8)()
+    g = _lib.lib().vlfm_gemm_f32_split_geometry(m, n, k, cus, int(x_planes), out)
+    _lib.check(min(g, 0), "gemm_f32_split_geometry")
+    names = {v: key for key, v in GEMM_F32_GEOMETRY.items()}
+    keys = ("tiles", "slots", "rounds", "last")
+    return names[g], {name: dict(zip(keys, out[4 * i:4 * i + 4])) for i, name in enumerate(("128", "m64"))}
+
+
+def layernorm768_f32(x: torch.Tensor, weight: torch.Tensor, bias: torch.Tensor, eps: float, planes: bool = False, owner: str = ""):
+    assert x.is_cuda and x.dtype == torch.float32 and x.is_contiguous() and x.shape[-1] == 768
+    assert weight.dtype == torch.float32 and bias.dtype == torch.float32 and weight.numel() == 768 and bias.numel() == 768
+    y = torch.empty_like(x)
+    hi = lo = None
+    if planes:
+        hi = torch.empty(x.shape, dtype=torch.float16, device=x.device)
+        lo = torch.empty_like(hi)
+    _lib.check(_lib.lib().vlfm_layernorm768_f32_planes(x.data_ptr(), weight.data_ptr(), bias.data_ptr(), y.data_ptr(),
+                                                       hi.data_ptr() if planes else None, lo.data_ptr() if planes else None,
+                                                       x.numel() // 768, 768, float(eps),
+                                                       gemm_f32_overflow_flag(x.device, owner).data_ptr(), _stream()),
+               "layernorm768_f32_planes")
+    return (y, (hi, lo)) if planes else y
+
+
+def linear_f32_split(x: torch.Tensor, weight: torch.Tensor, bias=None, act=None, residual=None, residual_period: int = 0,
+                     geometry: str = "auto", out=None, owner: str = "", x_planes=None, out_planes: bool = False):
+    K = weight.shape[1]
+    N = weight.shape[0]
+    lead = x.shape[:-1]
+    x2 = x.reshape(-1, K)
+    if x_planes is not None:
+        assert all(p.dtype == torch.float16 and p.is_contiguous() and p.shape == x.shape and p.device == x.device for p in x_planes)
+    elif not x2.is_contiguous() or x2.data_ptr() % 16:
+        x2 = x2.contiguous()
+    w = weight if weight.is_contiguous() else weight.contiguous()
+    M = x2.shape[0]
+    if out is None:
+        out = torch.empty((M, N), dtype=torch.float32, device=x.device)
+    res = None
+    if residual is not None:
+        res = residual.reshape(residual_period if residual_period else M, N)
+        if not res.is_contiguous() or res.data_ptr() % 16:
+            res = res.contiguous()
+    b = None
+    if bias is not None:
+        b = bias if bias.is_contiguous() else bias.contiguous()
+    hi, lo = split_weight(w, owner)
+    c_hi = c_lo = None
+    if out_planes:
+        c_hi = torch.empty((*lead, N), dtype=torch.float16, device=x.device)
+        c_lo = torch.empty_like(c_hi)
+    _lib.check(_lib.lib().vlfm_gemm_f32_split_nt(
+        x2.data_ptr() if x_planes is None else None, x_planes[0].data_ptr() if x_planes is not None else None,
+        x_planes[1].data_ptr() if x_planes is not None else None, b.data_ptr() if b is not None else None,
+        res.data_ptr() if res is not None else None, out.data_ptr(), c_hi.data_ptr() if out_planes else None,
+        c_lo.data_ptr() if out_planes else None, M, N, K, _ACT32[act], hi.data_ptr(), lo.data_ptr(),
+        gemm_f32_overflow_flag(x.device, owner).data_ptr(), residual_period, GEMM_F32_GEOMETRY[geometry], _stream()), "gemm_f32_split_nt")
+    return (out.view(*lead, N), (c_hi, c_lo)) if out_planes else out.view(*lead, N)
+
+
 _tuned_gemms_state = None
 
 
```
